# Electron-Labs/starky_bls12_381

Hardware: AMD Instinct MI355X
Metric: starky proofs/sec (FinalExponentiateStark 73527x8192) (higher is better)
Workload: dtype u64 (Goldilocks field)

## Files before the change

bindings/rust/starkhip-sys/src/lib.rs:

```rust
#![allow(non_camel_case_types)]

use std::os::raw::{c_char, c_int, c_long, c_uint, c_void};

#[repr(C)]
#[derive(Clone, Copy, Debug, Default)]
pub struct starkhip_config_t {
    pub security_bits: u32,
    pub num_challenges: u32,
    pub rate_bits: u32,
    pub cap_height: u32,
    pub proof_of_work_bits: u32,
    pub arity_bits: u32,
    pub final_poly_bits: u32,
    pub num_query_rounds: u32,
}

#[repr(C)]
#[derive(Clone, Copy, Debug, PartialEq, Eq)]
pub enum Air {
    Fp12Mul = 0,
    PairingPrecomp = 1,
    MillerLoop = 2,
    FinalExp = 3,
    EccAggregate = 4,
// ... 231 lines not shown
    pub fn starkhip_trace_pairing_precomp(qx: *const u32, qy: *const u32, qz: *const u32, trace: *mut u64, n_rows: usize,
                                          public_inputs: *mut u64) -> c_int;
    pub fn starkhip_trace_ecc_aggregate(points: *const u32, bits: *const u8, trace: *mut u64, n_rows: usize, public_inputs: *mut u64) -> c_int;

    pub fn starkhip_init(device_ordinal: c_int, ctx: *mut *mut c_void) -> c_int;
    pub fn starkhip_shutdown(ctx: *mut c_void);
    pub fn starkhip_set_option(ctx: *mut c_void, name: *const c_char, value: c_long) -> c_int;
    pub fn starkhip_prove(ctx: *mut c_void, air: Air, cfg: *const starkhip_config_t, trace: *const u64, n_rows: usize, n_cols: usize,
                          trace_layout: c_int, trace_on_device: c_int, public_inputs: *const u64, n_pis: usize, pow_witness: u64,
                          proof: *mut *mut u64, proof_words: *mut usize) -> c_int;

    pub fn starkhip_trace_log_begin(log: *mut *mut c_void) -> c_int;
    pub fn starkhip_trace_set_threads(n: c_int) -> c_int;
    pub fn starkhip_trace_log_end(log: *mut c_void) -> c_int;
    pub fn starkhip_trace_log_free(log: *mut c_void);
    pub fn starkhip_trace_log_info(log: *const c_void, n_rows: *mut usize, n_cols: *mut usize, n_records: *mut usize, n_words: *mut usize) -> c_int;
    pub fn starkhip_prove_compact(ctx: *mut c_void, air: Air, cfg: *const starkhip_config_t, log: *const c_void, public_inputs: *const u64,
                                  n_pis: usize, pow_witness: u64, proof: *mut *mut u64, proof_words: *mut usize) -> c_int;

    pub fn starkhip_pool_create(cfg: *const starkhip_pool_config_t, pool: *mut *mut c_void) -> c_int;
    pub fn starkhip_pool_destroy(pool: *mut c_void);
    pub fn starkhip_pool_submit(pool: *mut c_void, air: Air, cfg: *const starkhip_config_t, trace: *const u64, n_rows: usize, n_cols: usize,
                                trace_layout: c_int, trace_on_device: c_int, public_inputs: *const u64, n_pis: usize, pow_witness: u64,
                                ticket: *mut u64) -> c_int;
    pub fn starkhip_prove_columns(ctx: *mut c_void, air: Air, cfg: *const starkhip_config_t, columns: *const *const u64, n_rows: usize, n_cols: usize,
                                  public_inputs: *const u64, n_pis: usize, pow_witness: u64, proof: *mut *mut u64, proof_words: *mut usize) -> c_int;
    pub fn starkhip_pool_submit_columns(pool: *mut c_void, air: Air, cfg: *const starkhip_config_t, columns: *const *const u64, n_rows: usize,
                                        n_cols: usize, public_inputs: *const u64, n_pis: usize, pow_witness: u64, ticket: *mut u64) -> c_int;
    pub fn starkhip_pool_submit_compact(pool: *mut c_void, air: Air, cfg: *const starkhip_config_t, log: *const c_void, public_inputs: *const u64,
                                        n_pis: usize, pow_witness: u64, ticket: *mut u64) -> c_int;
    pub fn starkhip_pool_submit_witness(pool: *mut c_void, air: Air, cfg: *const starkhip_config_t, operands: *const u32, n_limbs: usize,
                                        pow_witness: u64, ticket: *mut u64) -> c_int;
    pub fn starkhip_pool_wait(pool: *mut c_void, ticket: u64, proof: *mut *mut u64, proof_words: *mut usize, info: *mut starkhip_ticket_info_t) -> c_int;

    pub fn starkhip_multipool_create(devices: *const c_int, n_devices: usize, cfg: *const starkhip_pool_config_t, mpool: *mut *mut c_void) -> c_int;
    pub fn starkhip_multipool_destroy(mpool: *mut c_void);
    pub fn starkhip_multipool_size(mpool: *const c_void) -> usize;
    pub fn starkhip_multipool_submit(mpool: *mut c_void, slot: c_int, air: Air, cfg: *const starkhip_config_t, trace: *const u64, n_rows: usize,
                                     n_cols: usize, trace_layout: c_int, trace_on_device: c_int, public_inputs: *const u64, n_pis: usize,
                                     pow_witness: u64, ticket: *mut u64) -> c_int;
    pub fn starkhip_multipool_submit_columns(mpool: *mut c_void, slot: c_int, air: Air, cfg: *const starkhip_config_t, columns: *const *const u64,
                                             n_rows: usize, n_cols: usize, public_inputs: *const u64, n_pis: usize, pow_witness: u64,
                                             ticket: *mut u64) -> c_int;
    pub fn starkhip_multipool_submit_witness(mpool: *mut c_void, slot: c_int, air: Air, cfg: *const starkhip_config_t, operands: *const u32,
                                             n_limbs: usize, pow_witness: u64, ticket: *mut u64) -> c_int;
    pub fn starkhip_multipool_submit_witness_batch(mpool: *mut c_void, n_jobs: usize, airs: *const Air, operands: *const *const u32,
                                                   n_limbs: *const usize, pow_witness: u64, tickets: *mut u64, rcs: *mut c_int) -> c_int;
    pub fn starkhip_multipool_ticket_slot(mpool: *const c_void, ticket: u64) -> c_int;
    pub fn starkhip_multipool_wait(mpool: *mut c_void, ticket: u64, proof: *mut *mut u64, proof_words: *mut usize,
                                   info: *mut starkhip_ticket_info_t) -> c_int;
    pub fn starkhip_hw_queues_status() -> c_int;
    pub fn starkhip_hw_queues_in_effect() -> c_int;
    pub fn starkhip_pool_set_option(pool: *mut c_void, name: *const c_char, value: c_long) -> c_int;
    pub fn starkhip_pool_submit_verify(pool: *mut c_void, air: Air, cfg: *const starkhip_config_t, proof: *const u64, proof_words: usize,
                                       ticket: *mut u64) -> c_int;
    pub fn starkhip_pool_verify_stats(pool: *mut c_void, out: *mut starkhip_pool_verify_stats_t) -> c_int;
    pub fn starkhip_pool_check_stats(pool: *mut c_void, out: *mut u64) -> c_int;
    pub fn starkhip_multipool_set_option(mpool: *mut c_void, name: *const c_char, value: c_long) -> c_int;
    pub fn starkhip_multipool_submit_verify(mpool: *mut c_void, slot: c_int, air: Air, cfg: *const starkhip_config_t, proof: *const u64,
                                            proof_words: usize, ticket: *mut u64) -> c_int;
    pub fn starkhip_multipool_verify_batch(mpool: *mut c_void, n: usize, airs: *const Air, cfgs: *const starkhip_config_t,
                                           proofs: *const *const u64, proof_words: *const usize, results: *mut c_int) -> c_int;
    pub fn starkhip_plan_verify(n: usize, airs: *const Air, n_pools: usize, slots: *mut c_int, order: *mut usize) -> c_int;
    pub fn starkhip_air_verify_cost(air: Air) -> f64;

    pub fn starkhip_last_timings(ctx: *mut c_void, ms: *mut f32) -> c_int;
    pub fn starkhip_host_alloc(ctx: *mut c_void, bytes: usize, out: *mut *mut c_void) -> c_int;
    pub fn starkhip_host_free(p: *mut c_void);

    pub fn starkhip_verify(air: Air, cfg: *const starkhip_config_t, proof: *const u64, proof_words: usize) -> c_int;
    pub fn starkhip_verify_batch(ctx: *mut c_void, n: usize, airs: *const Air, cfgs: *const starkhip_config_t, proofs: *const *const u64,
                                 proof_words: *const usize, results: *mut c_int) -> c_int;
    pub fn starkhip_last_verify_timings(ctx: *mut c_void, out: *mut f64) -> c_int;
    pub fn starkhip_verify_batch_replay(n: usize, airs: *const Air, cfgs: *const starkhip_config_t, proofs: *const *const u64,
                                        proof_words: *const usize, results: *mut c_int) -> c_int;
    pub fn starkhip_proof_layout(proof: *const u64, proof_words: usize, out: *mut starkhip_proof_layout_t) -> c_int;
    pub fn starkhip_proof_hasher(proof: *const u64, proof_words: usize) -> c_int;
    pub fn starkhip_keccak256(bytes: *const u8, len: usize, out32: *mut u8);
    pub fn starkhip_keccak_permute_host(state12: *mut u64);
    pub fn starkhip_keccak_state_from_words(words: *const u64, n: usize, state12: *mut u64) -> c_int;
    pub fn starkhip_keccak_permute_batch(ctx: *mut c_void, states: *mut u64, n: usize) -> c_int;
    pub fn starkhip_merkle_tree_hasher(ctx: *mut c_void, hasher: c_int, lde_colmajor: *const u64, n_cols: usize, log_n: c_uint, cap_height: c_uint,
                                       digests_out: *mut u64, cap_out: *mut u64) -> c_int;
    pub fn starkhip_hash_rows_hasher(ctx: *mut c_void, hasher: c_int, rows: *const u64, width: usize, n_leaves: usize, digests_out: *mut u64) -> c_int;
    pub fn starkhip_fri_geometry(cfg: *const starkhip_config_t, log_n: c_uint, arities_out: *mut c_uint, cap: usize, n_layers: *mut usize,
                                 final_poly_len: *mut usize) -> c_int;
    pub fn starkhip_free(p: *mut c_void);
    pub fn starkhip_proof_blob_stats(out: *mut u64);
    pub fn starkhip_error_string(code: c_int) -> *const c_char;
}

#[derive(Debug, Clone, Copy, PartialEq, Eq)]
pub struct Error(pub c_int);

impl std::fmt::Display for Error {
    fn fmt(&self, f: &mut std::fmt::Formatter<'_>) -> std::fmt::Result {
        let s = unsafe { std::ffi::CStr::from_ptr(starkhip_error_string(self.0)) };
        write!(f, "starkhip: {} ({})", s.to_string_lossy(), self.0)
    }
}
impl std::error::Error for Error {}

fn check(rc: c_int) -> Result<(), Error> {
    if rc == STARKHIP_OK { Ok(()) } else { Err(Error(rc)) }
}

pub type Config = starkhip_config_t;
impl Config {
    pub fn for_air(air: Air) -> Result<Config, Error> {
        let mut cfg = Config::default();
        check(unsafe { starkhip_config_for_air(air, &mut cfg) })?;
        Ok(cfg)
    }
}

pub struct Proof(pub Vec<u64>);
impl Proof {
    pub fn layout(&self) -> Result<starkhip_proof_layout_t, Error> {
        let mut l = std::mem::MaybeUninit::<starkhip_proof_layout_t>::zeroed();
        check(unsafe { starkhip_proof_layout(self.0.as_ptr(), self.0.len(), l.as_mut_ptr()) })?;
        Ok(unsafe { l.assume_init() })
    }
    pub fn hasher(&self) -> Result<c_int, Error> {
        let h = unsafe { starkhip_proof_hasher(self.0.as_ptr(), self.0.len()) };
        if h < 0 { check(h)?; }
        Ok(h)
    }
    pub fn public_inputs(&self) -> Result<&[u64], Error> {
        let l = self.layout()?;
        Ok(&self.0[l.off_public_inputs..l.off_public_inputs + l.n_public_inputs])
    }
}

pub struct RecordedTrace {
    log: *mut c_void,
    pub public_inputs: Vec<u64>,
}
unsafe impl Send for RecordedTrace {}
impl Drop for RecordedTrace {
    fn drop(&mut self) {
        unsafe { starkhip_trace_log_free(self.log) }
    }
}

fn record(air: Air, fill: impl FnOnce(*mut u64) -> c_int) -> Result<RecordedTrace, Error> {
    let n_pis = unsafe { starkhip_air_public_inputs(air) } as usize;
    let mut pis = vec![0u64; n_pis];
    let mut log = std::ptr::null_mut();
    check(unsafe { starkhip_trace_log_begin(&mut log) })?;
    let rc = fill(pis.as_mut_ptr());
    let end = unsafe { starkhip_trace_log_end(log) };
    if rc != STARKHIP_OK || end != STARKHIP_OK {
        unsafe { starkhip_trace_log_free(log) };
        return Err(Error(if rc != STARKHIP_OK { rc } else { end }));
    }
    Ok(RecordedTrace { log, public_inputs: pis })
}

pub fn record_final_exp(x: &[u32; 144]) -> Result<RecordedTrace, Error> {
    record(Air::FinalExp, |pis| unsafe { starkhip_trace_final_exp(x.as_ptr(), std::ptr::null_mut(), 8192, pis) })
}
pub fn record_miller_loop(px: &[u32; 12], py: &[u32; 12], qx: &[u32; 24], qy: &[u32; 24], qz: &[u32; 24]) -> Result<RecordedTrace, Error> {
    record(Air::MillerLoop, |pis| unsafe {
        starkhip_trace_miller_loop(px.as_ptr(), py.as_ptr(), qx.as_ptr(), qy.as_ptr(), qz.as_ptr(), std::ptr::null_mut(), 1024, pis)
    })
}
// ... 316 lines not shown
```

include/starkhip.h:

```cpp
#ifndef STARKHIP_H
#define STARKHIP_H
#include <stddef.h>
#include <stdint.h>

#ifdef __cplusplus
extern "C" {
#endif

typedef struct {
    uint32_t security_bits;
    uint32_t num_challenges;
    uint32_t rate_bits;
    uint32_t cap_height;
    uint32_t proof_of_work_bits;
    uint32_t arity_bits;
    uint32_t final_poly_bits;
    uint32_t num_query_rounds;
} starkhip_config_t;

#define STARKHIP_AIR_CUSTOM_BASE 1024
#define STARKHIP_AIR_CUSTOM_CAPACITY 4096
#define STARKHIP_MAX_LOG_ROWS 20
#define STARKHIP_AIR_MAX_COLUMNS (1u << 20)
#define STARKHIP_AIR_MAX_PUBLIC_INPUTS 65535u
// ... 222 lines not shown
int starkhip_pool_set_option(void* pool, const char* name, long value);
int starkhip_pool_check_stats(void* pool, uint64_t out[2]);
int starkhip_pool_submit_verify(void* pool, starkhip_air_t air, const starkhip_config_t* cfg, const uint64_t* proof, size_t proof_words,
                                uint64_t* ticket);
typedef struct {
    unsigned long proofs_checked, verify_jobs, rejected, device_batches;
    double upload_ms, device_ms, prelude_ms, prelude_cpu_s;
    uint64_t arena_bytes;
} starkhip_pool_verify_stats_t;
int starkhip_pool_verify_stats(void* pool, starkhip_pool_verify_stats_t* out);

int starkhip_multipool_create(const int* devices, size_t n_devices, const starkhip_pool_config_t* cfg, void** mpool);
void starkhip_multipool_destroy(void* mpool);
size_t starkhip_multipool_size(const void* mpool);
void* starkhip_multipool_pool(void* mpool, size_t slot);
int starkhip_multipool_device(const void* mpool, size_t slot);
int starkhip_multipool_submit(void* mpool, int slot, starkhip_air_t air, const starkhip_config_t* cfg, const uint64_t* trace, size_t n_rows,
                              size_t n_cols, int trace_layout, int trace_on_device, const uint64_t* public_inputs, size_t n_pis,
                              uint64_t pow_witness, uint64_t* ticket);
int starkhip_multipool_submit_columns(void* mpool, int slot, starkhip_air_t air, const starkhip_config_t* cfg, const uint64_t* const* columns,
                                      size_t n_rows, size_t n_cols, const uint64_t* public_inputs, size_t n_pis, uint64_t pow_witness,
                                      uint64_t* ticket);
int starkhip_multipool_submit_compact(void* mpool, int slot, starkhip_air_t air, const starkhip_config_t* cfg, const void* log,
                                      const uint64_t* public_inputs, size_t n_pis, uint64_t pow_witness, uint64_t* ticket);
int starkhip_multipool_submit_witness(void* mpool, int slot, starkhip_air_t air, const starkhip_config_t* cfg, const uint32_t* operands,
                                      size_t n_limbs, uint64_t pow_witness, uint64_t* ticket);
int starkhip_multipool_submit_witness_batch(void* mpool, size_t n_jobs, const starkhip_air_t* airs, const uint32_t* const* operands,
                                            const size_t* n_limbs, uint64_t pow_witness, uint64_t* tickets, int* rcs);
int starkhip_multipool_ticket_slot(const void* mpool, uint64_t ticket);
int starkhip_multipool_wait(void* mpool, uint64_t ticket, uint64_t** proof, size_t* proof_words, starkhip_ticket_info_t* info);
int starkhip_multipool_set_option(void* mpool, const char* name, long value);
int starkhip_multipool_submit_verify(void* mpool, int slot, starkhip_air_t air, const starkhip_config_t* cfg, const uint64_t* proof,
                                     size_t proof_words, uint64_t* ticket);
int starkhip_multipool_verify_batch(void* mpool, size_t n, const starkhip_air_t* airs, const starkhip_config_t* cfgs, const uint64_t* const* proofs,
                                    const size_t* proof_words, int* results);
int starkhip_plan_verify(size_t n, const starkhip_air_t* airs, size_t n_pools, int* slots, size_t* order);
double starkhip_air_verify_cost(starkhip_air_t air);
int starkhip_plan_lpt(size_t n_jobs, const starkhip_air_t* airs, size_t n_pools, int* slots);
double starkhip_air_cost(starkhip_air_t air);

#define STARKHIP_N_PHASES 11
int starkhip_last_timings(void* ctx, float ms[STARKHIP_N_PHASES]);
int starkhip_last_kernel_timings(void* ctx, float ms[3]);
int starkhip_last_host_timings(void* ctx, float ms[2]);

int starkhip_host_alloc(void* ctx, size_t bytes, void** out);
void starkhip_host_free(void* p);

int starkhip_permutation_zs(void* ctx, starkhip_air_t air, const uint64_t* trace, size_t n_rows, size_t n_cols, int layout, int on_device,
                            const uint64_t* challenges, uint64_t* zs_out, uint64_t* closing_out);
int starkhip_permutation_zs_replay(starkhip_air_t air, const uint64_t* trace, size_t n_rows, size_t n_cols, int layout, const uint64_t* challenges,
                                   uint64_t* zs_out, uint64_t* closing_out);
int starkhip_air_eval_frame_full(starkhip_air_t air, const uint64_t* local, const uint64_t* next, const uint64_t* public_inputs,
                                 const uint64_t masks[8], const uint64_t* alphas, int n_alpha, const uint64_t* zs, const uint64_t* zs_next,
                                 const uint64_t* challenges, uint64_t* acc_out);
int starkhip_lde_batch(void* ctx, const uint64_t* values, size_t n_cols, unsigned log_n, unsigned rate_bits, uint64_t* coeffs_out,
                       uint64_t* lde_out);
int starkhip_ntt_long(void* ctx, uint64_t* data, size_t n_vecs, unsigned log_len, int inverse);
int starkhip_merkle_cap(void* ctx, const uint64_t* lde_colmajor, size_t n_cols, unsigned log_N, unsigned cap_height, uint64_t* cap_out);
int starkhip_poseidon_permute_batch(void* ctx, uint64_t* states, size_t n_states);
int starkhip_lde_bench(void* ctx, size_t n_cols, unsigned log_n, unsigned rate_bits, unsigned reps, unsigned const_per_64, const uint64_t* device_values,
                       float* ms_per_launch, float* each_ms);
int starkhip_trace_log_expand_device(void* ctx, const void* log, uint64_t* trace_colmajor);
int starkhip_field_ops_batch(void* ctx, int op, const uint64_t* a, const uint64_t* b, uint64_t* out, size_t n);
int starkhip_poseidon_permute_batch_form(void* ctx, int form, int variant, uint64_t* states, size_t n_states);
int starkhip_leaf_hash_lane_group(void* ctx, const uint64_t* mats, size_t n_segments, size_t n_cols, unsigned log_n, unsigned rate_bits, int grouped,
                                  int form, unsigned prefix_mask, uint64_t* digests_out);
int starkhip_leaf_prefix_table(void* ctx, unsigned log_n, unsigned rate_bits, uint64_t* cap_out);
int starkhip_selfcheck_hash_tables(unsigned n_states);
size_t starkhip_hash_table_image(int form, void* out, size_t cap);
size_t starkhip_lde_launch_ranges(size_t n_cols, unsigned rate_bits, uint64_t* triples, size_t cap);
int starkhip_fri_geometry(const starkhip_config_t* cfg, unsigned log_n, unsigned* arities_out, size_t cap, size_t* n_layers,
                          size_t* final_poly_len);
int starkhip_quotient_plan_check(starkhip_air_t air, unsigned want_chunks, uint64_t seed, uint64_t stats[8]);
int starkhip_quotient_classes(starkhip_air_t air, uint8_t* classes, size_t n);
int starkhip_quotient_solve_table(unsigned log_rows, unsigned quotient_degree_bits, uint64_t* out, size_t n);
int starkhip_quotient_class_plan_check(starkhip_air_t air, unsigned want_chunks, uint64_t seed, uint64_t stats[32]);
void starkhip_keccak256(const uint8_t* bytes, size_t len, uint8_t out32[32]);
void starkhip_keccak_permute_host(uint64_t state12[12]);
int starkhip_keccak_state_from_words(const uint64_t* words, size_t n, uint64_t state12[12]);
int starkhip_keccak_permute_batch(void* ctx, uint64_t* states, size_t n);
int starkhip_merkle_tree_hasher(void* ctx, int hasher, const uint64_t* lde_colmajor, size_t n_cols, unsigned log_N, unsigned cap_height,
                                uint64_t* digests_out, uint64_t* cap_out);
int starkhip_hash_rows_hasher(void* ctx, int hasher, const uint64_t* rows, size_t width, size_t n_leaves, uint64_t* digests_out);
void starkhip_poseidon_permute_host(uint64_t state[12]);
void starkhip_poseidon_permute_host_many(uint64_t state[12], size_t n, int which);

int starkhip_verify(starkhip_air_t air, const starkhip_config_t* cfg, const uint64_t* proof, size_t proof_words);

int starkhip_verify_batch(void* ctx, size_t n, const starkhip_air_t* airs, const starkhip_config_t* cfgs, const uint64_t* const* proofs,
                          const size_t* proof_words, int* results);
int starkhip_last_verify_timings(void* ctx, double out[4]);
int starkhip_verify_batch_replay(size_t n, const starkhip_air_t* airs, const starkhip_config_t* cfgs, const uint64_t* const* proofs,
                                 const size_t* proof_words, int* results);

void starkhip_free(void* p);
const char* starkhip_error_string(int code);

#define STARKHIP_PROOF_MAGIC 0x3130304652505353ULL

typedef struct {
    size_t n_columns, n_quotient_polys, degree_bits, rate_bits, cap_height, n_fri_layers, n_query_rounds, final_poly_len,
        n_public_inputs, arity_bits;
    size_t off_trace_cap, off_quotient_cap, off_local_values, off_next_values, off_quotient_openings, off_fri_caps, off_query_rounds,
        query_round_words, off_final_poly, off_pow_witness, off_public_inputs, total_words;
    size_t q_trace_leaf, q_trace_siblings, q_quotient_leaf, q_quotient_siblings, initial_sibling_count;
    size_t q_step_evals[16], q_step_siblings[16], step_sibling_count[16];
    size_t n_permutation_zs, off_permutation_zs_cap, off_permutation_zs, off_permutation_zs_next, q_permutation_zs_leaf, q_permutation_zs_siblings;
} starkhip_proof_layout_t;
int starkhip_proof_layout(const uint64_t* proof, size_t proof_words, starkhip_proof_layout_t* out);
int starkhip_proof_hasher(const uint64_t* proof, size_t proof_words);

#ifdef __cplusplus
}
#endif
#endif
```

starky_bls12_381_amd/api.py:

```python
import ctypes as C
import os
import time
import weakref

import numpy as np

_HERE = os.path.dirname(os.path.abspath(__file__))
LIB_PATH = os.environ.get("STARKHIP_LIBRARY") or os.path.join(_HERE, "libstarkhip.so")

if not os.path.exists(LIB_PATH):
    raise ImportError(
        f"{LIB_PATH} is missing: build it with `make` (or __graft_entry__.build()); "
        "starky_bls12_381_amd has no CPU fallback for the prover")

lib = C.CDLL(LIB_PATH)

P = 0xFFFFFFFF00000001
POW_SEARCH = 0xFFFFFFFFFFFFFFFF
N_PHASES = 11
PHASE_NAMES = ["upload", "ifft_lde", "trace_merkle", "quotient", "quotient_commit", "openings", "fri_combine",
               "fri_commit", "pow", "queries", "total"]

AIR_FP12_MUL, AIR_PAIRING_PRECOMP, AIR_MILLER_LOOP, AIR_FINAL_EXP, AIR_ECC_AGGREGATE, AIR_TEST_FIBONACCI = 0, 1, 2, 3, 4, 100
AIR_NAMES = {AIR_FP12_MUL: "FP12MulStark", AIR_PAIRING_PRECOMP: "PairingPrecompStark", AIR_MILLER_LOOP: "MillerLoopStark",
# ... 24 lines not shown

class StarkhipError(RuntimeError):
    def __init__(self, code):
        self.code = code
        super().__init__(f"starkhip error {code}: {lib.starkhip_error_string(code).decode()}")


def _chk(rc):
    if rc != 0:
        raise StarkhipError(rc)


_u64p = C.POINTER(C.c_uint64)
_u32p = C.POINTER(C.c_uint32)
lib.starkhip_error_string.restype = C.c_char_p
lib.starkhip_error_string.argtypes = [C.c_int]
lib.starkhip_config_standard_fast.argtypes = [C.POINTER(StarkConfig)]
lib.starkhip_config_for_air.argtypes = [C.c_int, C.POINTER(StarkConfig)]
for _f in ("columns", "public_inputs", "constraint_degree", "num_constraints", "default_rows"):
    getattr(lib, "starkhip_air_" + _f).argtypes = [C.c_int]
lib.starkhip_air_program.argtypes = [C.c_int, C.POINTER(_u64p), C.POINTER(C.c_size_t)]
lib.starkhip_init.argtypes = [C.c_int, C.POINTER(C.c_void_p)]
lib.starkhip_shutdown.argtypes = [C.c_void_p]
lib.starkhip_shutdown.restype = None
lib.starkhip_prove.argtypes = [C.c_void_p, C.c_int, C.POINTER(StarkConfig), C.c_void_p, C.c_size_t, C.c_size_t, C.c_int, C.c_int, _u64p, C.c_size_t,
                               C.c_uint64, C.POINTER(_u64p), C.POINTER(C.c_size_t)]
lib.starkhip_prove_columns.argtypes = [C.c_void_p, C.c_int, C.POINTER(StarkConfig), C.POINTER(C.c_void_p), C.c_size_t, C.c_size_t, _u64p, C.c_size_t,
                                       C.c_uint64, C.POINTER(_u64p), C.POINTER(C.c_size_t)]
lib.starkhip_last_timings.argtypes = [C.c_void_p, C.POINTER(C.c_float)]
lib.starkhip_last_kernel_timings.argtypes = [C.c_void_p, C.POINTER(C.c_float)]
lib.starkhip_last_host_timings.argtypes = [C.c_void_p, C.POINTER(C.c_float)]
lib.starkhip_ntt_long.argtypes = [C.c_void_p, _u64p, C.c_size_t, C.c_uint, C.c_int]
lib.starkhip_lde_batch.argtypes = [C.c_void_p, _u64p, C.c_size_t, C.c_uint, C.c_uint, _u64p, _u64p]
lib.starkhip_merkle_cap.argtypes = [C.c_void_p, _u64p, C.c_size_t, C.c_uint, C.c_uint, _u64p]
lib.starkhip_poseidon_permute_batch.argtypes = [C.c_void_p, _u64p, C.c_size_t]
lib.starkhip_poseidon_permute_batch_form.argtypes = [C.c_void_p, C.c_int, C.c_int, _u64p, C.c_size_t]
lib.starkhip_leaf_hash_lane_group.argtypes = [C.c_void_p, _u64p, C.c_size_t, C.c_size_t, C.c_uint, C.c_uint, C.c_int, C.c_int, C.c_uint, _u64p]
lib.starkhip_leaf_prefix_table.argtypes = [C.c_void_p, C.c_uint, C.c_uint, _u64p]
lib.starkhip_field_ops_batch.argtypes = [C.c_void_p, C.c_int, _u64p, _u64p, _u64p, C.c_size_t]
lib.starkhip_poseidon_permute_host.argtypes = [_u64p]
lib.starkhip_poseidon_permute_host.restype = None
lib.starkhip_verify.argtypes = [C.c_int, C.POINTER(StarkConfig), _u64p, C.c_size_t]
_verify_batch_args = [C.c_size_t, C.POINTER(C.c_int), C.POINTER(StarkConfig), C.POINTER(_u64p), C.POINTER(C.c_size_t), C.POINTER(C.c_int)]
lib.starkhip_verify_batch.argtypes = [C.c_void_p] + _verify_batch_args
lib.starkhip_verify_batch_replay.argtypes = _verify_batch_args
lib.starkhip_last_verify_timings.argtypes = [C.c_void_p, C.POINTER(C.c_double)]
lib.starkhip_free.argtypes = [C.c_void_p]
lib.starkhip_free.restype = None
lib.starkhip_host_alloc.argtypes = [C.c_void_p, C.c_size_t, C.POINTER(C.c_void_p)]
lib.starkhip_trace_log_begin.argtypes = [C.POINTER(C.c_void_p)]
lib.starkhip_trace_log_end.argtypes = [C.c_void_p]
lib.starkhip_trace_set_threads.argtypes = [C.c_int]
lib.starkhip_trace_log_free.argtypes = [C.c_void_p]
lib.starkhip_trace_log_free.restype = None
lib.starkhip_trace_log_info.argtypes = [C.c_void_p] + [C.POINTER(C.c_size_t)] * 4
lib.starkhip_trace_log_from_writes.argtypes = [C.c_size_t, C.c_size_t, C.POINTER(C.c_uint64), C.c_size_t, C.POINTER(C.c_void_p)]
lib.starkhip_lde_bench.argtypes = [C.c_void_p, C.c_size_t, C.c_uint, C.c_uint, C.c_uint, C.c_uint, C.c_void_p, C.POINTER(C.c_float), C.POINTER(C.c_float)]
lib.starkhip_trace_log_expand_device.argtypes = [C.c_void_p, C.c_void_p, C.POINTER(C.c_uint64)]
lib.starkhip_trace_log_overwrites.argtypes = [C.c_void_p] + [C.POINTER(C.c_size_t)] * 2
lib.starkhip_trace_log_expand_host.argtypes = [C.c_void_p, C.POINTER(C.c_uint64), C.POINTER(C.c_size_t)]
lib.starkhip_prove_compact.argtypes = [C.c_void_p, C.c_int, C.POINTER(StarkConfig), C.c_void_p, C.POINTER(C.c_uint64), C.c_size_t, C.c_uint64,
                                       C.POINTER(C.POINTER(C.c_uint64)), C.POINTER(C.c_size_t)]
lib.starkhip_host_free.argtypes = [C.c_void_p]
lib.starkhip_host_free.restype = None
lib.starkhip_trace_fibonacci.argtypes = [C.c_uint64, C.c_uint64, _u64p, C.c_size_t, _u64p]
lib.starkhip_trace_fp12_mul.argtypes = [_u32p, _u32p, _u64p, C.c_size_t, _u64p]
lib.starkhip_trace_final_exp.argtypes = [_u32p, _u64p, C.c_size_t, _u64p]
lib.starkhip_trace_miller_loop.argtypes = [_u32p, _u32p, _u32p, _u32p, _u32p, _u64p, C.c_size_t, _u64p]
lib.starkhip_trace_pairing_precomp.argtypes = [_u32p, _u32p, _u32p, _u64p, C.c_size_t, _u64p]
lib.starkhip_native_fp12_mul.argtypes = [_u32p, _u32p, _u32p]
lib.starkhip_native_final_exponentiate.argtypes = [_u32p, _u32p]
lib.starkhip_native_miller_loop.argtypes = [_u32p, _u32p, _u32p, _u32p, _u32p, _u32p]
lib.starkhip_native_pairing_precomp.argtypes = [_u32p, _u32p, _u32p, _u32p]
_u8p = C.POINTER(C.c_uint8)
HASHER_POSEIDON, HASHER_KECCAK = 0, 1
LEAF_HASH_FORM_KECCAK = 6
lib.starkhip_keccak256.argtypes = [C.c_char_p, C.c_size_t, _u8p]
lib.starkhip_keccak256.restype = None
lib.starkhip_keccak_permute_host.argtypes = [_u64p]
lib.starkhip_keccak_permute_host.restype = None
lib.starkhip_keccak_state_from_words.argtypes = [_u64p, C.c_size_t, _u64p]
lib.starkhip_keccak_permute_batch.argtypes = [C.c_void_p, _u64p, C.c_size_t]
lib.starkhip_merkle_tree_hasher.argtypes = [C.c_void_p, C.c_int, _u64p, C.c_size_t, C.c_uint, C.c_uint, _u64p, _u64p]
lib.starkhip_hash_rows_hasher.argtypes = [C.c_void_p, C.c_int, _u64p, C.c_size_t, C.c_size_t, _u64p]
lib.starkhip_proof_hasher.argtypes = [_u64p, C.c_size_t]
lib.starkhip_trace_ecc_aggregate.argtypes = [_u32p, _u8p, _u64p, C.c_size_t, _u64p]
lib.starkhip_native_g1_aggregate.argtypes = [_u32p, _u8p, _u32p]


def _p64(a):
    return a.ctypes.data_as(_u64p)


def _p32(a):
    return a.ctypes.data_as(_u32p)


def _limbs(x, n):
    a = np.ascontiguousarray(x, dtype=np.uint32).reshape(-1)
    assert a.size == n, (a.size, n)
    return a


def air_columns(air):
    r = lib.starkhip_air_columns(air)
    if r < 0:
        raise StarkhipError(r)
    return r


def air_public_inputs(air):
    r = lib.starkhip_air_public_inputs(air)
    if r < 0:
        raise StarkhipError(r)
    return r


def air_constraint_degree(air):
    r = lib.starkhip_air_constraint_degree(air)
    if r < 0:
        raise StarkhipError(r)
    return r


def air_num_constraints(air):
    r = lib.starkhip_air_num_constraints(air)
    if r < 0:
        raise StarkhipError(r)
    return r


def air_default_rows(air):
    r = lib.starkhip_air_default_rows(air)
    if r < 0:
        raise StarkhipError(r)
    return r


def air_permutation_pairs(air):
    r = lib.starkhip_air_permutation_pairs(air)
    if r < 0:
        raise StarkhipError(r)
    return r


def air_permutation_zs(air):
    r = lib.starkhip_air_permutation_zs(air)
    if r < 0:
        raise StarkhipError(r)
    return r


def air_program(air):
    blob = _u64p()
    words = C.c_size_t()
    _chk(lib.starkhip_air_program(air, C.byref(blob), C.byref(words)))
    return np.ctypeslib.as_array(blob, shape=(words.value,)).copy()


lib.starkhip_air_check_program.argtypes = [_u64p, C.c_size_t, C.c_char_p, C.c_size_t]
lib.starkhip_air_register.argtypes = [_u64p, C.c_size_t, C.c_char_p, C.c_uint32, C.POINTER(C.c_int)]
lib.starkhip_check_trace.argtypes = [C.c_void_p, C.c_int, C.c_void_p, C.c_size_t, C.c_size_t, C.c_int, C.c_int, _u64p, _u64p, _u64p]
CHECK_LIST_MAX = 1 << 20


class _CheckReportStruct(C.Structure):
# ... 900 lines not shown
    def lde_bench(self, n_cols, log_n, rate_bits, reps=5, const_per_64=0, device_ptr=None, each=False):
        ms = C.c_float()
        per = (C.c_float * 16)()
        _chk(lib.starkhip_lde_bench(self._ctx, n_cols, log_n, rate_bits, reps, const_per_64, C.c_void_p(device_ptr) if device_ptr else None, C.byref(ms), per))
        return [round(float(x), 2) for x in per[:max(1, min(reps, 16))]] if each else float(ms.value)

    def expand_trace(self, compact):
        n, c = compact.shape
        out = np.empty((c, n), dtype=np.uint64)
        _chk(lib.starkhip_trace_log_expand_device(self._ctx, compact._h, _p64(out)))
        return np.ascontiguousarray(out.T)

    def set_option(self, name, value):
        _chk(lib.starkhip_set_option(self._ctx, name.encode(), int(value)))

    def check_stats(self):
        out = np.zeros(2, dtype=np.uint64)
        _chk(lib.starkhip_check_stats(self._ctx, _p64(out)))
        return {"checked": int(out[0]), "rejected": int(out[1])}

    def prove_device(self, air, config, trace_ptr, n_rows, public_inputs, pow_witness=POW_SEARCH, layout=1, keep=True):
        pis = np.ascontiguousarray(public_inputs, dtype=np.uint64)
        out = _u64p()
        words = C.c_size_t()
        t0 = time.perf_counter()
        rc = lib.starkhip_prove(self._ctx, air, C.byref(config), C.c_void_p(trace_ptr), n_rows, air_columns(air), layout, 1, _p64(pis), pis.size, pow_witness,
                                C.byref(out), C.byref(words))
        self.last_call_s = time.perf_counter() - t0
        return _take_blob(rc, out, words, keep)

    def host_array(self, shape, dtype=np.uint64):
        shape = tuple(int(s) for s in np.atleast_1d(shape))
        nbytes = int(np.prod(shape)) * np.dtype(dtype).itemsize
        p = C.c_void_p()
        _chk(lib.starkhip_host_alloc(self._ctx, nbytes, C.byref(p)))
        raw = (C.c_ubyte * nbytes).from_address(p.value)
        weakref.finalize(raw, lib.starkhip_host_free, p.value)
        return np.frombuffer(raw, dtype=dtype).reshape(shape)

    def last_timings(self):
        ms = (C.c_float * N_PHASES)()
        _chk(lib.starkhip_last_timings(self._ctx, ms))
        return dict(zip(PHASE_NAMES, [float(x) for x in ms]))

    def last_host_timings(self):
        ms = (C.c_float * 2)()
        _chk(lib.starkhip_last_host_timings(self._ctx, ms))
        return {"fiat_shamir": float(ms[0]), "other": float(ms[1])}

    def last_kernel_timings(self):
        ms = (C.c_float * 3)()
        _chk(lib.starkhip_last_kernel_timings(self._ctx, ms))
        return {"lde_columns": float(ms[0]), "leaf_hash": float(ms[1]), "quotient_eval": float(ms[2])}

    def ntt_long(self, vectors, inverse=False):
        v = np.ascontiguousarray(vectors, dtype=np.uint64).copy()
        n_vecs, n = v.shape
        _chk(lib.starkhip_ntt_long(self._ctx, _p64(v), n_vecs, n.bit_length() - 1, 1 if inverse else 0))
        return v

    def lde_batch(self, values_colmajor, rate_bits):
        v = np.ascontiguousarray(values_colmajor, dtype=np.uint64)
        ncols, n = v.shape
        log_n = n.bit_length() - 1
        coeffs = np.zeros_like(v)
        lde = np.zeros((ncols, n << rate_bits), dtype=np.uint64)
        _chk(lib.starkhip_lde_batch(self._ctx, _p64(v), ncols, log_n, rate_bits, _p64(coeffs), _p64(lde)))
        return coeffs, lde

    def merkle_cap(self, lde_colmajor, cap_height):
        v = np.ascontiguousarray(lde_colmajor, dtype=np.uint64)
        ncols, N = v.shape
        cap = np.zeros((1 << cap_height, 4), dtype=np.uint64)
        _chk(lib.starkhip_merkle_cap(self._ctx, _p64(v), ncols, N.bit_length() - 1, cap_height, _p64(cap)))
        return cap

    def merkle_tree(self, lde_colmajor, cap_height, hasher=HASHER_POSEIDON):
        v = np.ascontiguousarray(lde_colmajor, dtype=np.uint64)
        ncols, N = v.shape
        digests = np.zeros((N, 4), dtype=np.uint64)
        cap = np.zeros((1 << cap_height, 4), dtype=np.uint64)
        _chk(lib.starkhip_merkle_tree_hasher(self._ctx, hasher, _p64(v), ncols, N.bit_length() - 1, cap_height, _p64(digests), _p64(cap)))
        return digests, cap

    def hash_rows(self, rows, hasher=HASHER_POSEIDON):
        r = np.ascontiguousarray(rows, dtype=np.uint64)
        assert r.ndim == 2
        out = np.zeros((r.shape[0], 4), dtype=np.uint64)
        _chk(lib.starkhip_hash_rows_hasher(self._ctx, hasher, _p64(r), r.shape[1], r.shape[0], _p64(out)))
        return out

    def keccak_permute_batch(self, states):
        s = np.ascontiguousarray(states, dtype=np.uint64).copy()
        assert s.ndim == 2 and s.shape[1] == 12
        _chk(lib.starkhip_keccak_permute_batch(self._ctx, _p64(s), s.shape[0]))
        return s

    def field_ops(self, op, a, b):
        a = np.ascontiguousarray(a, dtype=np.uint64)
        b = np.ascontiguousarray(b, dtype=np.uint64)
        assert a.shape == b.shape and a.ndim == 1
        out = np.zeros_like(a)
        _chk(lib.starkhip_field_ops_batch(self._ctx, op, _p64(a), _p64(b), _p64(out), a.size))
        return out

    def leaf_hash_lane_group(self, mats, log_n, rate_bits=0, grouped=True, form=3, prefix_mask=0):
        m = np.ascontiguousarray(mats, dtype=np.uint64)
        assert m.ndim == 3
        out = np.zeros((m.shape[0], m.shape[2], 4), dtype=np.uint64)
        if m.shape[2] != 1 << (log_n + rate_bits):
            raise StarkhipError(ERR_BAD_SHAPE)
        _chk(lib.starkhip_leaf_hash_lane_group(self._ctx, _p64(m), m.shape[0], m.shape[1], log_n, rate_bits, 1 if grouped else 0, form, prefix_mask, _p64(out)))
        return out

    def leaf_prefix_table(self, log_n, rate_bits):
        out = np.zeros((4, 1 << (log_n + rate_bits)), dtype=np.uint64)
        _chk(lib.starkhip_leaf_prefix_table(self._ctx, log_n, rate_bits, _p64(out)))
        return out

    def poseidon_permute_batch(self, states, form=0, variant=0):
        s = np.ascontiguousarray(states, dtype=np.uint64).copy()
        assert s.ndim == 2 and s.shape[1] == 12
        if form == 0 and variant == 0:
            _chk(lib.starkhip_poseidon_permute_batch(self._ctx, _p64(s), s.shape[0]))
        else:
            _chk(lib.starkhip_poseidon_permute_batch_form(self._ctx, form, variant, _p64(s), s.shape[0]))
        return s

    def verify_batch(self, items):
        return _verify_batch(items, self._ctx)

    def verify_stark_proof_device(self, air, config, proof):
        _chk(self.verify_batch([(air, config, proof)])[0])

    def last_verify_timings(self):
        out = (C.c_double * 4)()
        _chk(lib.starkhip_last_verify_timings(self._ctx, out))
        return dict(zip(("prelude_ms", "upload_ms", "device_ms", "cpu_s"), list(out)))


class PoolConfig(C.Structure):
    _fields_ = [("device", C.c_int), ("big_contexts", C.c_uint), ("small_contexts", C.c_uint), ("generator_threads", C.c_uint),
                ("trace_threads", C.c_uint), ("commit_policy", C.c_uint), ("stream_priority", C.c_uint), ("warm_up", C.c_uint), ("gather_ms", C.c_float)]


class TicketInfo(C.Structure):
    _fields_ = [("phase_ms", C.c_float * N_PHASES), ("kernel_ms", C.c_float * 3), ("host_ms", C.c_float * 2), ("t_submit", C.c_double), ("t_generate_start", C.c_double),
                ("t_generate_end", C.c_double), ("t_prove_start", C.c_double), ("t_done", C.c_double), ("leaf_hash_form", C.c_int),
                ("leaf_hash_group", C.c_uint)]


class PoolStats(C.Structure):
    _fields_ = [(n, C.c_ulong) for n in ("big_commit_launches", "small_commit_launches", "small_commit_requests", "max_merged_commitments", "big_commit_grids")]


lib.starkhip_pool_create.argtypes = [C.POINTER(PoolConfig), C.POINTER(C.c_void_p)]
lib.starkhip_pool_destroy.argtypes = [C.c_void_p]
lib.starkhip_pool_destroy.restype = None
lib.starkhip_pool_submit.argtypes = [C.c_void_p, C.c_int, C.POINTER(StarkConfig), C.c_void_p, C.c_size_t, C.c_size_t, C.c_int, C.c_int, _u64p,
                                     C.c_size_t, C.c_uint64, C.POINTER(C.c_uint64)]
lib.starkhip_pool_submit_compact.argtypes = [C.c_void_p, C.c_int, C.POINTER(StarkConfig), C.c_void_p, _u64p, C.c_size_t, C.c_uint64,
                                             C.POINTER(C.c_uint64)]
lib.starkhip_pool_submit_witness.argtypes = [C.c_void_p, C.c_int, C.POINTER(StarkConfig), _u32p, C.c_size_t, C.c_uint64, C.POINTER(C.c_uint64)]
lib.starkhip_pool_wait.argtypes = [C.c_void_p, C.c_uint64, C.POINTER(_u64p), C.POINTER(C.c_size_t), C.POINTER(TicketInfo)]
lib.starkhip_pool_stats.argtypes = [C.c_void_p, C.POINTER(PoolStats)]
lib.starkhip_pool_submit_columns.argtypes = [C.c_void_p, C.c_int, C.POINTER(StarkConfig), C.POINTER(C.c_void_p), C.c_size_t, C.c_size_t, _u64p, C.c_size_t,
# ... 387 lines not shown
```

starky_bls12_381_amd/csrc/capi.cpp:

```cpp
#include <dirent.h>
#include <mutex>
#include <stdio.h>
#include <stdlib.h>
#include <string.h>
#include <unistd.h>

#include <new>

#include "air_eval.h"
#include "air_validate.h"
#include "airs.h"
#include "blob_arena.h"
#include "check_report.h"
#include "free_cells.h"
#include "kernels.h"
#include "lde_ranges.h"
#include "lookup_columns.h"
#include "permutation.h"
#include "permutation_check.h"
#include "trace_log.h"

#include <atomic>
#include "poseidon.h"
#include "prover.h"
// ... 966 lines not shown
    try {
        return expand_log((Ctx*)ctx, (const TraceLog*)log, trace_colmajor);
    } catch (const std::bad_alloc&) {
        return STARKHIP_ERR_OOM;
    }
}
int starkhip_poseidon_permute_batch(void* ctx, uint64_t* states, size_t n_states) {
    if (!ctx) return STARKHIP_ERR_NO_DEVICE;
    return permute_batch((Ctx*)ctx, states, n_states);
}
int starkhip_poseidon_permute_batch_form(void* ctx, int form, int variant, uint64_t* states, size_t n_states) {
    if (!ctx) return STARKHIP_ERR_NO_DEVICE;
    return permute_batch_form((Ctx*)ctx, form, variant, states, n_states);
}
int starkhip_leaf_hash_lane_group(void* ctx, const uint64_t* mats, size_t n_segments, size_t n_cols, unsigned log_n, unsigned rate_bits, int grouped,
                                  int form, unsigned prefix_mask, uint64_t* digests_out) {
    if (!ctx) return STARKHIP_ERR_NO_DEVICE;
    return leaf_hash_lane_group((Ctx*)ctx, mats, n_segments, n_cols, log_n, rate_bits, grouped, form, prefix_mask, digests_out);
}
int starkhip_leaf_prefix_table(void* ctx, unsigned log_n, unsigned rate_bits, uint64_t* cap_out) {
    if (!ctx) return STARKHIP_ERR_NO_DEVICE;
    return leaf_prefix_table((Ctx*)ctx, log_n, rate_bits, cap_out);
}
int starkhip_field_ops_batch(void* ctx, int op, const uint64_t* a, const uint64_t* b, uint64_t* out, size_t n) {
    if (!ctx) return STARKHIP_ERR_NO_DEVICE;
    return field_ops((Ctx*)ctx, op, a, b, out, n);
}
int starkhip_selfcheck_hash_tables(unsigned n_states) {
    const int fours = merged_fours_selfcheck(n_states);
    if (fours < 0) return -1;
    return quad_merged_tables_selfcheck(n_states) + fours;
}
size_t starkhip_hash_table_image(int form, void* out, size_t cap) {
    const void* image = nullptr;
    size_t bytes = 0;
    switch (form) {
        case FORM_QUAD: image = quad_merged_tables_host(); bytes = sizeof(QuadMergedTables); break;
        case FORM_ROW: image = row_merged_tables_host(); bytes = sizeof(RowMergedTables); break;
        case FORM_LANE: image = lane_tables_host(); bytes = sizeof(LaneTables); break;
        case FORM_PAIR: image = pair_tables_host(); bytes = sizeof(PairTables); break;
    }
    if (!image) return 0;
    if (out && cap >= bytes) memcpy(out, image, bytes);
    return bytes;
}
int starkhip_fri_geometry(const starkhip_config_t* cfg, unsigned log_n, unsigned* arities_out, size_t cap, size_t* n_layers, size_t* final_poly_len) {
    if (!cfg) return STARKHIP_ERR_BAD_SHAPE;
    FriGeometry g;
    if (!FriGeometry::make(*cfg, log_n, &g)) return STARKHIP_ERR_BAD_SHAPE;
    for (size_t l = 0; l < g.arities.size() && l < cap; l++) arities_out[l] = g.arities[l];
    if (n_layers) *n_layers = g.arities.size();
    if (final_poly_len) *final_poly_len = g.final_poly_len;
    return STARKHIP_OK;
}

size_t starkhip_lde_launch_ranges(size_t n_cols, unsigned rate_bits, uint64_t* triples, size_t cap) {
    const std::vector<LdeLaunch> plan = lde_launch_plan(n_cols, rate_bits);
    for (size_t i = 0; i < plan.size() && i < cap; i++) {
        triples[3 * i] = plan[i].a;
        triples[3 * i + 1] = plan[i].b;
        triples[3 * i + 2] = plan[i].from_copy ? 1 : 0;
    }
    return plan.size();
}
void starkhip_poseidon_permute_host(uint64_t state[12]) { poseidon_permute_host(state); }

void starkhip_keccak256(const uint8_t* bytes, size_t len, uint8_t out32[32]) { keccak256_host(bytes, len, out32); }
void starkhip_keccak_permute_host(uint64_t state12[12]) { keccak_permute_host(state12); }
int starkhip_keccak_state_from_words(const uint64_t* words, size_t n, uint64_t state12[12]) {
    if (!words || !state12) return -1;
    int used = 0;
    const int have = keccak_take_words(words, (int)std::min<size_t>(n, 1u << 20), state12, 0, &used);
    return have == 12 ? used : -1;
}
int starkhip_keccak_permute_batch(void* ctx, uint64_t* states, size_t n) {
    if (!ctx) return STARKHIP_ERR_NO_DEVICE;
    return keccak_permute_batch((Ctx*)ctx, states, n);
}
int starkhip_merkle_tree_hasher(void* ctx, int hasher, const uint64_t* lde_colmajor, size_t n_cols, unsigned log_N, unsigned cap_height,
                                uint64_t* digests_out, uint64_t* cap_out) {
    if (!ctx) return STARKHIP_ERR_NO_DEVICE;
    return merkle_tree_hasher((Ctx*)ctx, hasher, lde_colmajor, n_cols, log_N, cap_height, digests_out, cap_out);
}
int starkhip_hash_rows_hasher(void* ctx, int hasher, const uint64_t* rows, size_t width, size_t n_leaves, uint64_t* digests_out) {
    if (!ctx) return STARKHIP_ERR_NO_DEVICE;
    return hash_rows_hasher((Ctx*)ctx, hasher, rows, width, n_leaves, digests_out);
}
int starkhip_proof_hasher(const uint64_t* proof, size_t proof_words) {
    ProofLayout pl;
    if (!proof || !pl.read_header(proof, proof_words)) return STARKHIP_ERR_BAD_SHAPE;
    return (int)pl.hasher;
}
void starkhip_poseidon_permute_host_many(uint64_t state[12], size_t n, int which) {
    for (size_t i = 0; i < n; i++) {
        if (which == 0) poseidon_permute_host(state);
        else poseidon_permute(state);
    }
}

int starkhip_verify(starkhip_air_t air, const starkhip_config_t* cfg, const uint64_t* proof, size_t proof_words) {
    const AirInfo* a = air_get(air);
    if (!a) return STARKHIP_ERR_BAD_AIR;
    return verify_proof(*a, *cfg, proof, proof_words);
}

int starkhip_verify_batch(void* ctx, size_t n, const starkhip_air_t* airs, const starkhip_config_t* cfgs, const uint64_t* const* proofs,
                          const size_t* proof_words, int* results) {
    if (!ctx) return STARKHIP_ERR_NO_DEVICE;
    try {
        return verify_batch_device((Ctx*)ctx, n, airs, cfgs, proofs, proof_words, results);
    } catch (const std::bad_alloc&) {
        return STARKHIP_ERR_OOM;
    }
}

int starkhip_last_verify_timings(void* ctx, double out[4]) {
    if (!ctx) return STARKHIP_ERR_NO_DEVICE;
    if (!out) return STARKHIP_ERR_BAD_SHAPE;
    memcpy(out, ctx_verify_timings((Ctx*)ctx), 4 * sizeof(double));
    return STARKHIP_OK;
}

int starkhip_verify_batch_replay(size_t n, const starkhip_air_t* airs, const starkhip_config_t* cfgs, const uint64_t* const* proofs,
                                 const size_t* proof_words, int* results) {
    try {
        return verify_batch_replay(n, airs, cfgs, proofs, proof_words, results);
    } catch (const std::bad_alloc&) {
        return STARKHIP_ERR_OOM;
    }
}

void starkhip_proof_blob_stats(uint64_t out[5]) {
    const starkhip::BlobArenaStats st = starkhip::blob_arena_stats();
    out[0] = st.blobs; out[1] = st.busy; out[2] = st.bytes; out[3] = st.taken; out[4] = st.missed;
}
void starkhip_free(void* p) { starkhip::blob_free(p); }

const char* starkhip_error_string(int code) {
    switch (code) {
        case STARKHIP_OK: return "ok";
        case STARKHIP_ERR_QUOTIENT_NOT_DIVISIBLE: return "Quotient has failed, the vanishing polynomial is not divisible by Z_H";
        case STARKHIP_ERR_ZETA_IN_SUBGROUP: return "Opening point is in the subgroup";
        case STARKHIP_ERR_BAD_SHAPE: return "bad shape (columns / public inputs / rows / config do not match the AIR)";
        case STARKHIP_ERR_HIP: return "HIP runtime error";
        case STARKHIP_ERR_OOM: return "out of device memory";
        case STARKHIP_ERR_NO_DEVICE: return "no such HIP device / context";
        case STARKHIP_ERR_VERIFY: return "proof rejected";
        case STARKHIP_ERR_BAD_AIR: return "unknown or unbuildable AIR id";
        case STARKHIP_ERR_TRACE: return "the trace violates the AIR (\"check_trace\"): a check blob is returned instead of a proof";
        default: return "unknown error";
    }
}

}
```

starky_bls12_381_amd/csrc/ctx.h:

```cpp
#pragma once
#include <hip/hip_runtime.h>

#include <stdio.h>

#include <atomic>
#include <memory>
#include <set>
#include <system_error>
#include <thread>
#include <vector>

#include "airs.h"
#include "kernels.h"
#include "prover.h"
#include "scheduler.h"
#include "trace_log.h"

namespace starkhip {

#define HIPCHK(expr)                                                                                       \
    do {                                                                                                   \
        hipError_t _e = (expr);                                                                            \
        if (_e != hipSuccess) {                                                                            \
            fprintf(stderr, "starkhip: HIP error %s at %s:%d (%s)\n", hipGetErrorString(_e), __FILE__, __LINE__, #expr); \
// ... 8 lines not shown
    ~DevBuf() { release(); }
    void release() {
        if (p) (void)hipFree(p);
        p = nullptr;
        cap = 0;
    }
    hipError_t ensure(size_t bytes) {
        if (bytes <= cap) return hipSuccess;
        release();
        hipError_t e = hipMalloc(&p, bytes);
        if (e == hipSuccess) cap = bytes;
        return e;
    }
    template <class T>
    T* as() const { return (T*)p; }
};

struct Ctx {
    int device = 0;
    hipStream_t st = nullptr;
    hipStream_t st_normal = nullptr, st_high = nullptr;
    hipEvent_t ev[STARKHIP_N_PHASES + 1] = {};
    float timings[STARKHIP_N_PHASES] = {0};
    hipEvent_t kev[6] = {};
    float ktimings[3] = {0};
    float htimings[2] = {0};
    HashService* hs = nullptr;
    hipEvent_t hash_ready = nullptr, hash_done = nullptr;
    HashService::Timing hash_timing;
    hipEvent_t wait_ev = nullptr;
    void* rb = nullptr;
    size_t rb_cap = 0, rb_used = 0;
    struct Pending { void* dst; const void* src; size_t bytes; };
    std::vector<Pending> rb_pending;
    void* host_staging = nullptr;
    size_t host_staging_cap = 0;
    hipEvent_t col_ev[2] = {nullptr, nullptr};
    std::set<int> blob_airs;
    bool hash_requested = false;
    bool urgent = false;
    long opt_quotient_impl = 0;
    long opt_quotient_cosets = 0;
    long opt_quotient_waves = 65536, opt_quotient_slots = 0, opt_quotient_chunks = 0, opt_quotient_debug = 0, opt_zeta_on_coset = 0;
    struct Tables {
        int log_n = -1, rate = -1, qdb = -1;
        DevBuf tw_fwd, tw_inv, coset_scale, qtab, qshift_inv;
        DevBuf qsolve;
        DevBuf lde2_fwd, lde2_inv, lde2_cs, lde2_oh;
        DevBuf lde_wave;
        DevBuf leaf_prefix;
        bool leaf_prefix_built = false;
        DevBuf long_cs, long_sub;
        struct LongTw { unsigned log_len; DevBuf fwd, inv; };
        std::vector<std::unique_ptr<LongTw>> long_tw;
        std::vector<DevBuf*> bufs() {
            std::vector<DevBuf*> v = {&tw_fwd, &tw_inv, &coset_scale, &qtab, &qshift_inv, &qsolve, &lde2_fwd, &lde2_inv, &lde2_cs, &lde2_oh, &lde_wave, &leaf_prefix, &long_cs, &long_sub};
            for (auto& t : long_tw) {
                v.push_back(&t->fwd);
                v.push_back(&t->inv);
            }
            return v;
        }
    };
    struct PlanDev {
        int air = -1;
        unsigned chunks = 0, want = 0;
        uint32_t recs = 0;
        bool by_class = false;
        unsigned n_work = 0, n_vecs = 0, n_classes = 0;
        DevBuf q_recs, q_streams, q_chunk_tile_off, q_tile_list, q_contrib_off, q_contribs, q_consts, q_apow, q_work, q_sum_off, q_vec_slot, q_vec_of;
        std::vector<DevBuf*> bufs() {
            return {&q_recs, &q_streams, &q_chunk_tile_off, &q_tile_list, &q_contrib_off, &q_contribs, &q_consts, &q_apow, &q_work, &q_sum_off, &q_vec_slot, &q_vec_of};
        }
    };
    std::vector<std::unique_ptr<Tables>> table_cache;
    std::vector<std::unique_ptr<PlanDev>> plan_cache;
    Tables* tab = nullptr;
    PlanDev* plan = nullptr;
    long opt_leaf_hash_form = FORM_AUTO;
    long opt_hasher = 0;
    long opt_lde_impl = 0;
    long opt_lde_closed_forms = 1;
    long opt_leaf_hash_prefix = 1;
    long opt_host_commit_leaves = 64;
    long opt_verify_chunk_mb = 1024;
    double verify_timings[4] = {0};
    long opt_check_trace = 0, opt_check_trace_list = 16;
    std::atomic<uint64_t> traces_checked{0}, traces_rejected{0};
    std::vector<gl_t> host_lde;
    struct OpProgram {
        int air = -1;
        unsigned chunks = 0, slots = 0;
        DevBuf ops, loads, chunk_off;
        std::vector<uint32_t> chunk_k_after;
        std::vector<DevBuf*> bufs() { return {&ops, &loads, &chunk_off}; }
    } prog;
    struct CheckProgram {
        int air = -1;
        unsigned want = 0, chunks = 0;
        std::vector<uint32_t> k0;
        DevBuf ops, meta, out, rep, list;
        std::vector<DevBuf*> bufs() { return {&ops, &meta, &out, &rep, &list}; }
    } chk;
    DevBuf staging, values, lde, digests, pis, apow, chunk_scale, partial, qclass, qvals, qcoef, qlde, qdigests, zpow, gzpow, open_local,
        open_next, open_q, ext_apow, comb_partial, comb_out, fri_coef, fri_vals, fri_rows[16], fri_digests[16], scale_tab, pow_state,
        pow_best, qidx, gather_t;
    std::vector<DevBuf*> dev_bufs() {
        std::vector<DevBuf*> v = {&staging, &values, &lde, &digests, &pis,
                                  &apow, &chunk_scale, &partial, &qclass, &qvals, &qcoef, &qlde, &qdigests, &zpow, &gzpow, &open_local, &open_next, &open_q,
                                  &ext_apow, &comb_partial, &comb_out, &fri_coef, &fri_vals, &scale_tab, &pow_state, &pow_best, &qidx, &gather_t};
        for (DevBuf& b : fri_rows) v.push_back(&b);
        for (DevBuf& b : fri_digests) v.push_back(&b);
        for (DevBuf* b : prog.bufs()) v.push_back(b);
        for (DevBuf* b : chk.bufs()) v.push_back(b);
        for (DevBuf* b : free_chk.bufs()) v.push_back(b);
        for (DevBuf* b : perm.bufs()) v.push_back(b);
        for (DevBuf* b : mset.bufs()) v.push_back(b);
        for (DevBuf* b : lookup.bufs()) v.push_back(b);
        for (auto& t : table_cache)
            for (DevBuf* b : t->bufs()) v.push_back(b);
        for (auto& d : plan_cache)
            for (DevBuf* b : d->bufs()) v.push_back(b);
        return v;
    }
    struct FreeCellsProgram {
        int air = -1;
        unsigned want = 0;
        DevBuf cons, pivots, planes, class_counts;
        std::vector<DevBuf*> bufs() { return {&cons, &pivots, &planes, &class_counts}; }
    } free_chk;
    struct PermBufs {
        DevBuf cols, desc, chal, zvals, zcoef, zlde, zdigests, scan, open_z, open_zn;
        std::vector<DevBuf*> bufs() { return {&cols, &desc, &chal, &zvals, &zcoef, &zlde, &zdigests, &scan, &open_z, &open_zn}; }
    } perm;
    struct MultisetBufs {
        DevBuf desc, keys, idx, table, masks;
        float ms[4] = {0, 0, 0, 0};
        std::vector<DevBuf*> bufs() { return {&desc, &keys, &idx, &table, &masks}; }
    } mset;
    struct LookupBufs {
        DevBuf desc, cols, flags, sums, slot, mask;
        float ms[4] = {0, 0, 0, 0};
        std::vector<DevBuf*> bufs() { return {&desc, &cols, &flags, &sums, &slot, &mask}; }
    } lookup;
};

hipError_t stream_wait(Ctx* c);
hipError_t read_back(Ctx* c, void* dst, const void* src, size_t bytes, hipStream_t st);
hipError_t ensure_host_staging(Ctx* c, size_t need, size_t grow_to);
int ensure_tables(Ctx* c, unsigned log_n, unsigned rate, unsigned qdb);
bool long_vector(unsigned log_len);
int ensure_long_tw(Ctx* c, unsigned log_len, LdeLongTables* out);
int ensure_plan(Ctx* c, const AirInfo& air, size_t quotient_points, bool by_class = false);
int ensure_program(Ctx* c, const AirInfo& air, size_t quotient_points);
hipError_t run_lde(Ctx* c, const gl_t* values, gl_t* coeffs, gl_t* lde, size_t cols, unsigned log_n, unsigned rate, int from_coeffs, unsigned col_base = 0,
                   unsigned* unit_count = nullptr);
bool leaf_prefix_wanted(const Ctx* c, size_t n_cols, unsigned log_n, unsigned rate);
size_t leaf_prefix_bytes(const Ctx* c, size_t n_cols, unsigned log_n, unsigned rate);
int ensure_leaf_prefix(Ctx* c, unsigned log_n, unsigned rate);
unsigned* leaf_prefix_counter(const Ctx* c);
hipError_t leaf_prefix_reset(Ctx* c);
LeafPrefix leaf_prefix(const Ctx* c);
int run_ntt(Ctx* c, gl_t* data, gl_t* mid, size_t n_vecs, size_t vec_stride, unsigned log_len, bool inverse, const gl_t* pre_scale,
            const gl_t* post_scale);
int upload_dense(Ctx* c, const TraceInput& in, gl_t* dst, const gl_t** d_values);
int check_trace_in_prove(Ctx* c, const AirInfo& air, const gl_t* d_trace, size_t n_rows, const uint64_t* pis, uint64_t** blob, size_t* words);
// ... 25 lines not shown
```

starky_bls12_381_amd/csrc/ctx.hip:

```cpp
#include <hip/hip_runtime.h>

#include <atomic>
#include <time.h>
#include <string.h>

#include <algorithm>
#include <memory>
#include <string>
#include <vector>

#include "blob_arena.h"
#include "ctx.h"
#include "quotient_ops.h"
#include "quotient_plan.h"
#include "verifier.h"

namespace starkhip {

hipError_t event_wait_sleeping(hipEvent_t ev) {
    for (int spin = 0; spin < 8; spin++) {
        const hipError_t q = hipEventQuery(ev);
        if (q != hipErrorNotReady) return q;
    }
    (void)hipGetLastError();
// ... 261 lines not shown
static void ctx_release(Ctx* c) {
    for (DevBuf* b : c->dev_bufs()) b->release();
    for (hipEvent_t e : c->ev)
        if (e) (void)hipEventDestroy(e);
    for (hipEvent_t e : c->kev)
        if (e) (void)hipEventDestroy(e);
    if (c->rb) (void)hipHostFree(c->rb);
    for (hipEvent_t e : {c->hash_ready, c->hash_done, c->wait_ev, c->hash_timing.t0, c->hash_timing.t1, c->col_ev[0], c->col_ev[1]})
        if (e) (void)hipEventDestroy(e);
    if (c->host_staging) (void)hipHostFree(c->host_staging);
    blob_arena_drop(c);
    if (c->st_normal) (void)hipStreamDestroy(c->st_normal);
    if (c->st_high) (void)hipStreamDestroy(c->st_high);
    delete c;
}

int ctx_create(int device, Ctx** out, int priority) {
    int count = 0;
    if (hipGetDeviceCount(&count) != hipSuccess || count <= 0) return STARKHIP_ERR_NO_DEVICE;
    if (device < 0 || device >= count) return STARKHIP_ERR_NO_DEVICE;
    HIPCHK(hipSetDevice(device));
    Ctx* c = new Ctx();
    c->device = device;
    bool ok;
    if (priority) {
        int least = 0, greatest = 0;
        ok = hipDeviceGetStreamPriorityRange(&least, &greatest) == hipSuccess &&
             hipStreamCreateWithPriority(&c->st_normal, hipStreamDefault, priority > 0 ? greatest : least) == hipSuccess;
    } else {
        ok = hipStreamCreate(&c->st_normal) == hipSuccess;
    }
    c->st = c->st_normal;
    for (auto& e : c->ev) ok = ok && hipEventCreate(&e) == hipSuccess;
    for (auto& e : c->kev) ok = ok && hipEventCreate(&e) == hipSuccess;
    ok = ok && hipEventCreateWithFlags(&c->hash_ready, hipEventDisableTiming) == hipSuccess;
    ok = ok && hipEventCreateWithFlags(&c->hash_done, hipEventDisableTiming | hipEventBlockingSync) == hipSuccess;
    ok = ok && hipEventCreateWithFlags(&c->wait_ev, hipEventDisableTiming | hipEventBlockingSync) == hipSuccess;
    ok = ok && hipEventCreate(&c->hash_timing.t0) == hipSuccess && hipEventCreate(&c->hash_timing.t1) == hipSuccess;
    if (ok && hipHostMalloc(&c->rb, (size_t)8 << 20, hipHostMallocDefault) == hipSuccess) c->rb_cap = (size_t)8 << 20;
    else c->rb = nullptr;
    if (!ok) {
        ctx_release(c);
        return STARKHIP_ERR_HIP;
    }
    *out = c;
    return 0;
}

void ctx_destroy(Ctx* c) {
    if (!c) return;
    (void)hipSetDevice(c->device);
    (void)hipStreamSynchronize(c->st);
    ctx_release(c);
}
void ctx_attach_hash_service(Ctx* c, HashService* hs) { c->hs = hs; }
int ctx_set_urgent(Ctx* c, bool urgent) {
    if (urgent && !c->st_high) {
        HIPCHK(hipSetDevice(c->device));
        int least = 0, greatest = 0;
        HIPCHK(hipDeviceGetStreamPriorityRange(&least, &greatest));
        HIPCHK(hipStreamCreateWithPriority(&c->st_high, hipStreamDefault, greatest));
    }
    c->st = urgent ? c->st_high : c->st_normal;
    c->urgent = urgent;
    return STARKHIP_OK;
}
bool ctx_has_hash_service(Ctx* c) { return c->hs != nullptr; }
void ctx_hash_request_reset(Ctx* c) { c->hash_requested = false; }
bool ctx_hash_requested(Ctx* c) { return c->hash_requested; }

int ctx_set_option(Ctx* c, const char* name, long value) {
    if (!c || !name) return STARKHIP_ERR_BAD_SHAPE;
    const std::string k(name);
    if (k == "quotient_impl" && (value == 0 || value == 1)) c->opt_quotient_impl = value;
    else if (k == "quotient_waves" && value >= 64) { c->opt_quotient_waves = value; c->prog.air = -1; }
    else if (k == "quotient_slots" && value >= 0 && value <= 64) { c->opt_quotient_slots = value; c->prog.air = -1; }
#ifdef STARKHIP_DEBUG
    else if (k == "quotient_debug" && value >= 0 && value <= 9) c->opt_quotient_debug = value;
#endif
    else if (k == "zeta_on_coset" && value >= 0) c->opt_zeta_on_coset = value;
    else if (k == "lde_closed_forms" && (value == 0 || value == 1)) c->opt_lde_closed_forms = value;
    else if (k == "lde_impl" && (value == 0 || value == 1)) c->opt_lde_impl = value;
    else if (k == "leaf_hash_prefix" && (value == 0 || value == 1)) c->opt_leaf_hash_prefix = value;
    else if (k == "host_commit_leaves" && value >= 0 && value <= 4096) c->opt_host_commit_leaves = value;
    else if (k == "leaf_hash_form" && value >= FORM_AUTO && value <= FORM_PAIR) c->opt_leaf_hash_form = value;
    else if (k == "quotient_cosets" && (value == 0 || value == 1)) c->opt_quotient_cosets = value;
    else if (k == "quotient_chunks" && value >= 0 && value <= 4096) c->opt_quotient_chunks = value;
    else if (k == "verify_chunk_mb" && value >= 1) c->opt_verify_chunk_mb = value;
    else if (k == "hasher" && value >= STARKHIP_HASHER_POSEIDON && value <= STARKHIP_HASHER_KECCAK) c->opt_hasher = value;
    else if (k == "check_trace" && (value == 0 || value == 1)) c->opt_check_trace = value;
    else if (k == "check_trace_list" && value >= 0 && value <= (long)STARKHIP_CHECK_LIST_MAX) c->opt_check_trace_list = value;
    else return STARKHIP_ERR_BAD_SHAPE;
    return STARKHIP_OK;
}
void ctx_set_check_trace(Ctx* c, bool on, size_t list_cap) {
    c->opt_check_trace = on;
    c->opt_check_trace_list = (long)std::min<size_t>(list_cap, STARKHIP_CHECK_LIST_MAX);
}
void ctx_set_hasher(Ctx* c, int hasher) { c->opt_hasher = hasher; }
void ctx_check_stats(Ctx* c, uint64_t out[2]) {
    out[0] = c->traces_checked.load();
    out[1] = c->traces_rejected.load();
}
size_t ctx_device_bytes(Ctx* c) {
    size_t total = 0;
    for (DevBuf* b : c->dev_bufs()) total += b->cap;
    return total;
}
size_t ctx_pinned_bytes(Ctx* c) { return c->host_staging_cap + c->rb_cap; }
const float* ctx_timings(Ctx* c) { return c->timings; }
long ctx_verify_chunk_mb(Ctx* c) { return c->opt_verify_chunk_mb; }
double* ctx_verify_timings(Ctx* c) { return c->verify_timings; }
int ctx_device(Ctx* c) { return c->device; }
const float* ctx_kernel_timings(Ctx* c) { return c->ktimings; }
const float* ctx_host_timings(Ctx* c) { return c->htimings; }
void ctx_commit_info(Ctx* c, int* form, unsigned* group) {
    *form = c->hash_timing.form;
    *group = c->hash_timing.group;
}

hipError_t ensure_host_staging(Ctx* c, size_t need, size_t grow_to) {
    if (c->host_staging_cap >= need) return hipSuccess;
    if (c->host_staging) (void)hipHostFree(c->host_staging);
    c->host_staging = nullptr;
    c->host_staging_cap = 0;
    const hipError_t e = hipHostMalloc(&c->host_staging, grow_to, hipHostMallocDefault);
    if (e == hipSuccess) c->host_staging_cap = grow_to;
    return e;
}

std::vector<LogPiece> recording_pieces(const TraceLog& log) {
    const size_t nw = log.total_words(), nr = log.total_records();
    std::vector<LogPiece> pieces;
    size_t at_r = 0, at_z = 0;
    log.for_each_part([&](const TraceLog& part) {
        if (!part.words.empty()) pieces.push_back({part.base, part.words.data(), part.words.size()});
        if (!part.offsets.empty()) pieces.push_back({nw + at_r, part.offsets.data(), part.offsets.size()});
        if (!part.late_zeros.empty()) pieces.push_back({nw + nr + at_z, part.late_zeros.data(), part.late_zeros.size()});
        at_r += part.offsets.size();
        at_z += part.late_zeros.size();
    });
    return pieces;
}

int upload_dense(Ctx* c, const TraceInput& in, gl_t* dst, const gl_t** d_values) {
    const size_t n = in.n_rows, C = in.n_cols;
    *d_values = dst;
    if (in.callers_columns()) *d_values = in.words;
    else if (in.on_device) HIPCHK(launch_transpose(in.words, dst, n, C, c->st));
    else if (in.form == TraceForm::ColMajor) HIPCHK(hipMemcpyAsync(dst, in.words, C * n * 8, hipMemcpyHostToDevice, c->st));
    else {
        HIPCHK(hipMemcpyAsync(c->lde.p, in.words, C * n * 8, hipMemcpyHostToDevice, c->st));
        HIPCHK(launch_transpose(c->lde.as<gl_t>(), dst, n, C, c->st));
    }
    return 0;
}

hipError_t launch_leaf_hash_lone(const Ctx* c, const gl_t* lde, size_t n_cols, unsigned log_n, unsigned rate, gl_t* digests, hipStream_t st, int* form,
                                 LeafPrefix prefix) {
    const LeafHashForm f = c->opt_leaf_hash_form == FORM_LANE ? FORM_LANE : use_pair_form(c, n_cols, log_n + rate) ? FORM_PAIR : use_row_form(c, n_cols, log_n + rate) ? FORM_ROW : FORM_QUAD;
    *form = leaf_hash_sent(f);
    return launch_leaf_hash_form(f, lde, n_cols, log_n, rate, digests, st, prefix);
}

int run_ntt(Ctx* c, gl_t* data, gl_t* mid, size_t n_vecs, size_t vec_stride, unsigned log_len, bool inverse, const gl_t* pre_scale,
                   const gl_t* post_scale) {
// ... 13 lines not shown
```

starky_bls12_381_amd/csrc/host_only_stubs.cc:

```cpp
#include <hip/hip_runtime.h>
#include <stdlib.h>
#include <string.h>

#include <atomic>
#include <chrono>
#include <set>
#include <thread>

#include "blob_arena.h"
#include "kernels.h"
#include "prover.h"
#include "scheduler.h"
#include "verifier.h"
#include "verify_chunk.h"
#include "verify_query.h"

namespace starkhip {
std::atomic<uint64_t> g_wait_cpu_ns(0);

static bool fake_device() {
    const char* e = getenv("STARKHIP_FAKE_DEVICE");
    return e && *e == '1';
}

// ... 5 lines not shown
    float timings[STARKHIP_N_PHASES] = {0}, ktimings[3] = {0}, htimings[2] = {0};
    double verify_timings[4] = {0};
    std::set<int> blob_airs;
    HashService::Timing hash_timing;
    char done_tag = 0;
};
static char g_failing_ready_tag = 0;
static hipEvent_t failing_ready() { return (hipEvent_t)&g_failing_ready_tag; }
int ctx_create(int device, Ctx** out, int) {
    if (!fake_device() || device < 0 || device >= 8) {
        *out = nullptr;
        return STARKHIP_ERR_NO_DEVICE;
    }
    *out = new Ctx();
    (*out)->device = device;
    return STARKHIP_OK;
}
void ctx_destroy(Ctx* c) {
    if (c) blob_arena_drop(c);
    delete c;
}
size_t ctx_device_bytes(Ctx*) { return 0; }
size_t ctx_pinned_bytes(Ctx*) { return 0; }
const float* ctx_timings(Ctx* c) { return c->timings; }
long ctx_verify_chunk_mb(Ctx*) { return 1024; }
double* ctx_verify_timings(Ctx* c) { return c->verify_timings; }
int ctx_device(Ctx* c) { return c->device; }
const float* ctx_kernel_timings(Ctx* c) { return c->ktimings; }
const float* ctx_host_timings(Ctx* c) { return c->htimings; }
void ctx_commit_info(Ctx* c, int* form, unsigned* group) { *form = c->hash_timing.form; *group = c->hash_timing.group; }
int ctx_set_option(Ctx*, const char*, long) { return STARKHIP_ERR_NO_DEVICE; }
void ctx_attach_hash_service(Ctx* c, HashService* hs) { c->hs = hs; }
bool ctx_has_hash_service(Ctx* c) { return c->hs != nullptr; }
void ctx_hash_request_reset(Ctx* c) { c->hash_requested = false; }
bool ctx_hash_requested(Ctx* c) { return c->hash_requested; }
int ctx_set_urgent(Ctx* c, bool urgent) { c->urgent = urgent; return STARKHIP_OK; }
void ctx_set_check_trace(Ctx* c, bool on, size_t) { c->check_trace = on; }
void ctx_set_hasher(Ctx*, int) {}
void ctx_check_stats(Ctx* c, uint64_t out[2]) { out[0] = c->traces_checked.load(); out[1] = 0; }
int ctx_reserve(Ctx* c, const AirInfo& air, const starkhip_config_t&, size_t, unsigned proof_blobs, bool) {
    if (proof_blobs && !c->blob_airs.count(air.id)) {
        if (blob_arena_add(c, 64 + air.prog.n_pis * 8, proof_blobs) != 0) return STARKHIP_ERR_OOM;
        c->blob_airs.insert(air.id);
    }
    return STARKHIP_OK;
}

int prove(Ctx* c, const AirInfo& air, const starkhip_config_t& cfg, const TraceInput& in, const uint64_t* pis, size_t n_pis, uint64_t pow_witness,
          uint64_t** proof_out, size_t* proof_words) {
    if (!fake_device()) return STARKHIP_ERR_NO_DEVICE;
    if (n_pis != air.prog.n_pis) return STARKHIP_ERR_BAD_SHAPE;
    if (pow_witness == 0xBAD) return STARKHIP_ERR_BAD_SHAPE;
    const size_t n_rows = in.n_rows;
    std::this_thread::sleep_for(std::chrono::milliseconds(air.cols > 50000 ? 3 : 1));
    if (c->check_trace) c->traces_checked++;
    unsigned log_n = 0;
    while (((size_t)1 << log_n) < n_rows) log_n++;
    if (c->hs) {
        c->hash_requested = true;
        static gl_t dummy[8];
        c->hash_timing = HashService::Timing();
        if (c->hs->hash(dummy, air.cols, log_n, cfg.rate_bits, dummy, nullptr, pow_witness == 0xBAD3 ? failing_ready() : nullptr, (hipEvent_t)&c->done_tag,
                        !HashService::is_big(log_n, cfg.rate_bits), c->urgent, &c->hash_timing) != hipSuccess)
            return STARKHIP_ERR_HIP;
    }
    std::this_thread::sleep_for(std::chrono::milliseconds(2));
    if (pow_witness == 0xBAD2) return STARKHIP_ERR_QUOTIENT_NOT_DIVISIBLE;
    uint64_t* out = blob_alloc((4 + n_pis) * 8);
    if (!out) return STARKHIP_ERR_OOM;
    out[0] = 0xFA4EULL; out[1] = (uint64_t)air.id; out[2] = n_rows; out[3] = (uint64_t)c->urgent | ((uint64_t)c->device << 8);
    if (n_pis) memcpy(out + 4, pis, n_pis * 8);
    *proof_out = out;
    *proof_words = 4 + n_pis;
    c->timings[STARKHIP_N_PHASES - 1] = 3.0f;
    return STARKHIP_OK;
}
int lde_batch(Ctx*, const uint64_t*, size_t, unsigned, unsigned, uint64_t*, uint64_t*) { return STARKHIP_ERR_NO_DEVICE; }
int ntt_long(Ctx*, uint64_t*, size_t, unsigned, int) { return STARKHIP_ERR_NO_DEVICE; }
int merkle_cap(Ctx*, const uint64_t*, size_t, unsigned, unsigned, uint64_t*) { return STARKHIP_ERR_NO_DEVICE; }
int permute_batch(Ctx*, uint64_t*, size_t) { return STARKHIP_ERR_NO_DEVICE; }
int permute_batch_form(Ctx*, int, int, uint64_t*, size_t) { return STARKHIP_ERR_NO_DEVICE; }
int keccak_permute_batch(Ctx*, uint64_t*, size_t) { return STARKHIP_ERR_NO_DEVICE; }
int merkle_tree_hasher(Ctx*, int, const uint64_t*, size_t, unsigned, unsigned, uint64_t*, uint64_t*) { return STARKHIP_ERR_NO_DEVICE; }
int hash_rows_hasher(Ctx*, int, const uint64_t*, size_t, size_t, uint64_t*) { return STARKHIP_ERR_NO_DEVICE; }
int leaf_hash_lane_group(Ctx*, const uint64_t*, size_t, size_t, unsigned, unsigned, int, int, unsigned, uint64_t*) { return STARKHIP_ERR_NO_DEVICE; }
int leaf_prefix_table(Ctx*, unsigned, unsigned, uint64_t*) { return STARKHIP_ERR_NO_DEVICE; }
int expand_log(Ctx*, const TraceLog*, uint64_t*) { return STARKHIP_ERR_NO_DEVICE; }
int check_trace(Ctx*, const AirInfo&, const TraceInput&, const uint64_t*, uint64_t*, uint64_t*) { return STARKHIP_ERR_NO_DEVICE; }
int check_trace_report(Ctx*, const AirInfo&, const TraceInput&, const uint64_t*, uint32_t*, uint64_t*, uint64_t*, size_t, starkhip_check_report_t*) {
    return STARKHIP_ERR_NO_DEVICE;
}
int check_trace_free_cells(Ctx*, const AirInfo&, const TraceInput&, const uint64_t*, uint64_t, uint32_t*, uint64_t*, starkhip_free_cells_t*) {
    return STARKHIP_ERR_NO_DEVICE;
}
int check_trace_free_cell_classes(Ctx*, const AirInfo&, const TraceInput&, const uint64_t*, uint64_t, uint32_t*, uint64_t*, uint32_t*,
                                  starkhip_free_cell_classes_t*) {
    return STARKHIP_ERR_NO_DEVICE;
}
int check_trace_permutations(Ctx*, const AirInfo&, const TraceInput&, uint64_t, uint32_t*, uint64_t*, uint64_t*, size_t, starkhip_perm_check_t*) {
    return STARKHIP_ERR_NO_DEVICE;
}
void perm_check_timings(Ctx*, float ms[4]) { ms[0] = ms[1] = ms[2] = ms[3] = 0; }
int lookup_columns(Ctx*, const LookupTrace&, const starkhip_lookup_t*, size_t, uint32_t*, uint64_t*, uint64_t*, size_t, starkhip_lookup_report_t*) {
    return STARKHIP_ERR_NO_DEVICE;
}
void lookup_timings(Ctx*, float ms[4]) { ms[0] = ms[1] = ms[2] = ms[3] = 0; }
int lde_bench(Ctx*, size_t, unsigned, unsigned, unsigned, unsigned, const uint64_t*, float*, float*) { return STARKHIP_ERR_NO_DEVICE; }
int field_ops(Ctx*, int, const uint64_t*, const uint64_t*, uint64_t*, size_t) { return STARKHIP_ERR_NO_DEVICE; }
int permutation_zs(Ctx*, const AirInfo&, const TraceInput&, const uint64_t*, uint64_t*, uint64_t*) { return STARKHIP_ERR_NO_DEVICE; }
int host_alloc(Ctx*, size_t, void**) { return STARKHIP_ERR_NO_DEVICE; }
void host_free(void*) {}

hipError_t event_wait_sleeping(hipEvent_t ev) { return ev == failing_ready() ? hipErrorUnknown : hipSuccess; }

static std::atomic<unsigned long> g_fake_launches(0), g_fake_merged(0), g_fake_lane_grids(0), g_fake_lane_members(0), g_service_records(0);
hipError_t launch_leaf_hash_form(LeafHashForm, const gl_t*, size_t, unsigned, unsigned, gl_t*, hipStream_t, LeafPrefix) { g_fake_launches++; return hipSuccess; }
hipError_t launch_leaf_hash_multi(const LeafHashBatch&, unsigned count, size_t, unsigned, unsigned, hipStream_t) {
    g_fake_launches++;
    g_fake_merged += count;
    return hipSuccess;
}
hipError_t launch_leaf_hash_lane_group(const LeafHashBatch& B, unsigned count, size_t, unsigned, unsigned, hipStream_t) {
    if (count == 0 || count > LEAF_HASH_MAX_BATCH) return hipErrorInvalidValue;
    for (unsigned i = 0; i < count; i++)
        if (!B.mat[i] || !B.digests[i]) return hipErrorInvalidValue;
    g_fake_launches++;
    g_fake_lane_grids++;
    g_fake_lane_members += count;
    return hipSuccess;
}
hipError_t launch_leaf_hash_keccak(const gl_t*, size_t, unsigned, unsigned, gl_t*, hipStream_t) { return hipErrorNoDevice; }
hipError_t launch_leaf_hash_rows_keccak(const gl_t*, size_t, size_t, gl_t*, hipStream_t) { return hipErrorNoDevice; }
hipError_t launch_merkle_levels_keccak(gl_t*, unsigned, unsigned, hipStream_t) { return hipErrorNoDevice; }
hipError_t launch_permute_batch_keccak(gl_t*, size_t, hipStream_t) { return hipErrorNoDevice; }
hipError_t launch_pow_grind_keccak(const gl_t*, int, unsigned, uint64_t, uint64_t, unsigned long long*, hipStream_t) { return hipErrorNoDevice; }
hipError_t launch_verify_leaf_digests_keccak(const gl_t* words, const VQLeaf* leaves, size_t n, gl_t* digests, hipStream_t) {
    if (!fake_device()) return hipErrorNoDevice;
    verify_host_leaf_digests(words, leaves, n, digests);
    return hipSuccess;
}
hipError_t launch_ext_powers(gl2_t* out, gl2_t alpha, size_t n, hipStream_t) {
    if (!fake_device()) return hipErrorNoDevice;
    verify_host_ext_powers(out, alpha, n);
    return hipSuccess;
}
hipError_t launch_verify_leaf_digests(const gl_t* words, const VQLeaf* leaves, size_t n, gl_t* digests, unsigned, hipStream_t) {
    if (!fake_device()) return hipErrorNoDevice;
    verify_host_leaf_digests(words, leaves, n, digests);
    return hipSuccess;
}
hipError_t launch_verify_range(const gl_t* words, const VQProof* proofs, size_t n, uint32_t* bad, hipStream_t) {
    if (!fake_device()) return hipErrorNoDevice;
    verify_host_range(words, proofs, n, bad);
    return hipSuccess;
}
hipError_t launch_verify_combine(const gl_t* words, const VQProof* proofs, const uint32_t* qp, size_t nq, const gl2_t* apow, gl2_t* sums, hipStream_t) {
    if (!fake_device()) return hipErrorNoDevice;
    verify_host_combine(words, proofs, qp, nq, apow, sums);
    return hipSuccess;
}
hipError_t launch_verify_queries(const gl_t* words, const VQProof* proofs, const uint32_t* qp, const uint64_t* xi, size_t nq, const gl_t* dig,
                                 const gl2_t* sums, uint32_t* status, hipStream_t) {
    if (!fake_device()) return hipErrorNoDevice;
    verify_host_queries(words, proofs, qp, xi, nq, dig, sums, status);
    return hipSuccess;
}
}

static std::atomic<unsigned long> g_stub_allocs(0);
extern "C" unsigned long starkhip_stub_allocations(void) { return g_stub_allocs.load(); }
extern "C" void starkhip_stub_commit_counters(unsigned long out[4]) {
    out[0] = starkhip::g_fake_launches.load(); out[1] = starkhip::g_fake_lane_grids.load(); out[2] = starkhip::g_fake_lane_members.load();
    out[3] = starkhip::g_service_records.load();
}
extern "C" {
hipError_t hipSetDevice(int) { return hipSuccess; }
hipError_t hipGetDevice(int* d) { *d = 0; return hipSuccess; }
hipError_t hipGetLastError(void) { return hipSuccess; }
hipError_t hipStreamCreateWithFlags(hipStream_t* s, unsigned) { g_stub_allocs++; *s = (hipStream_t)malloc(1); return hipSuccess; }
hipError_t hipStreamCreateWithPriority(hipStream_t* s, unsigned, int) { g_stub_allocs++; *s = (hipStream_t)malloc(1); return hipSuccess; }
hipError_t hipDeviceGetStreamPriorityRange(int* least, int* greatest) { *least = 1; *greatest = -1; return hipSuccess; }
hipError_t hipStreamDestroy(hipStream_t s) { free((void*)s); return hipSuccess; }
hipError_t hipStreamSynchronize(hipStream_t) { return hipSuccess; }
hipError_t hipStreamQuery(hipStream_t) { return hipSuccess; }
hipError_t hipStreamWaitEvent(hipStream_t, hipEvent_t, unsigned) { return hipSuccess; }
hipError_t hipEventRecord(hipEvent_t, hipStream_t s) { if (s) starkhip::g_service_records++; return hipSuccess; }
hipError_t hipEventSynchronize(hipEvent_t) { return hipSuccess; }
hipError_t hipEventQuery(hipEvent_t) { return hipSuccess; }
hipError_t hipHostMalloc(void** p, size_t bytes, unsigned) { g_stub_allocs++; *p = malloc(bytes ? bytes : 1); return *p ? hipSuccess : hipErrorOutOfMemory; }
hipError_t hipHostFree(void* p) { free(p); return hipSuccess; }
hipError_t hipMalloc(void** p, size_t bytes) { g_stub_allocs++; *p = malloc(bytes ? bytes : 1); return *p ? hipSuccess : hipErrorOutOfMemory; }
hipError_t hipFree(void* p) { free(p); return hipSuccess; }
hipError_t hipMemcpy(void* d, const void* s, size_t n, hipMemcpyKind) { if (n) memcpy(d, s, n); return hipSuccess; }
hipError_t hipMemcpyAsync(void* d, const void* s, size_t n, hipMemcpyKind, hipStream_t) { if (n) memcpy(d, s, n); return hipSuccess; }
hipError_t hipMemsetAsync(void* d, int v, size_t n, hipStream_t) { if (n) memset(d, v, n); return hipSuccess; }
hipError_t hipEventCreate(hipEvent_t* e) { g_stub_allocs++; *e = (hipEvent_t)malloc(1); return hipSuccess; }
hipError_t hipEventCreateWithFlags(hipEvent_t* e, unsigned) { g_stub_allocs++; *e = (hipEvent_t)malloc(1); return hipSuccess; }
hipError_t hipEventDestroy(hipEvent_t e) { free((void*)e); return hipSuccess; }
hipError_t hipEventElapsedTime(float* ms, hipEvent_t, hipEvent_t) { *ms = 0; return hipSuccess; }
}
```

starky_bls12_381_amd/csrc/kernel_entries.hip:

```cpp
#include <hip/hip_runtime.h>

#include <algorithm>
#include <vector>

#include "ctx.h"
#include "kernels_permutation.h"
#include "permutation.h"

namespace starkhip {

int permutation_zs(Ctx* c, const AirInfo& air, const TraceInput& in, const uint64_t* challenges, uint64_t* zs_out, uint64_t* closing_out) {
    const AirProgram& P = air.prog;
    const size_t n = in.n_rows, C = in.n_cols, nZ = P.perm_zs(), B = P.perm_batch_size();
    HIPCHK(hipSetDevice(c->device));
    const std::vector<uint32_t> cols = perm_columns(P), desc = perm_descriptor(P, true);
    Ctx::PermBufs& pb = c->perm;
    HIPCHK(c->values.ensure(C * n * 8));
    HIPCHK(c->lde.ensure(C * n * 8));
    HIPCHK(pb.cols.ensure(cols.size() * n * 8));
    HIPCHK(pb.desc.ensure(desc.size() * 4));
    HIPCHK(pb.chal.ensure(B * 4 * 8));
    HIPCHK(pb.zvals.ensure(nZ * n * 8));
    HIPCHK(pb.scan.ensure((perm_scratch_words(n, (unsigned)nZ) + nZ) * 8));
    const gl_t* d_values = nullptr;
// ... 60 lines not shown
    HIPCHK(c->values.ensure(words * 8));
    HIPCHK(c->lde.ensure(words * 8));
    HIPCHK(hipMemcpyAsync(c->values.p, data, words * 8, hipMemcpyHostToDevice, c->st));
    if (int rc = run_ntt(c, c->values.as<gl_t>(), c->lde.as<gl_t>(), n_vecs, (size_t)1 << log_len, log_len, inverse != 0, nullptr, nullptr)) return rc;
    HIPCHK(hipMemcpyAsync(data, c->values.p, words * 8, hipMemcpyDeviceToHost, c->st));
    HIPCHK(stream_wait(c));
    return STARKHIP_OK;
}

int lde_bench(Ctx* c, size_t n_cols, unsigned log_n, unsigned rate_bits, unsigned reps, unsigned const_per_64, const uint64_t* device_values, float* ms_out, float* each_ms) {
    if (log_n < 1 || log_n > STARKHIP_MAX_LOG_ROWS || rate_bits > 8 || !n_cols) return STARKHIP_ERR_BAD_SHAPE;
    HIPCHK(hipSetDevice(c->device));
    int rc;
    if ((rc = ensure_tables(c, log_n, rate_bits, 0))) return rc;
    const size_t n = (size_t)1 << log_n, N = n << rate_bits;
    const bool long_cols = lde_long_supported(log_n);
    HIPCHK(c->values.ensure(n_cols * n * 8 * (long_cols ? 2 : 1)));
    HIPCHK(c->lde.ensure(n_cols * N * 8));
    const gl_t* in = device_values ? (const gl_t*)device_values : c->values.as<gl_t>();
    gl_t* const cf = long_cols ? c->values.as<gl_t>() + n_cols * n : nullptr;
    if (device_values) const_per_64 = 0;
    else HIPCHK(launch_fill_powers(c->values.as<gl_t>(), 3, GL_GENERATOR, n_cols * n, c->st));
    const bool unit = (const_per_64 & 256u) != 0, prewarm = (const_per_64 & 1024u) != 0, touch = (const_per_64 & 2048u) != 0;
    const_per_64 &= 255u;
    for (size_t c0 = 0; const_per_64 && c0 < n_cols; c0 += 64) {
        const size_t cnt = std::min<size_t>(const_per_64, n_cols - c0);
        HIPCHK(hipMemsetAsync(c->values.as<gl_t>() + c0 * n, unit ? 0 : 1, cnt * n * 8, c->st));
        for (size_t k = 0; unit && k < cnt; k++) HIPCHK(hipMemsetAsync(c->values.as<gl_t>() + (c0 + k) * n + ((c0 + k) * 37) % n, 1, 1, c->st));
    }
    const bool cold = reps == 0;
    if (cold) reps = 1;
    reps = std::min(reps, 16u);
    std::vector<hipEvent_t> ev(reps + 1, nullptr);
    hipError_t err = hipSuccess;
    for (hipEvent_t& e : ev)
        if (err == hipSuccess) err = hipEventCreate(&e);
    if (err == hipSuccess && cold && touch) err = hipMemsetAsync(c->lde.p, 0, n_cols * N * 8, c->st);
    if (err == hipSuccess && cold && prewarm)
        for (int k = 0; k < 4 && err == hipSuccess; k++) err = run_lde(c, in, cf, c->lde.as<gl_t>(), std::min<size_t>(n_cols, 4096), log_n, rate_bits, 0);
    if (err == hipSuccess) err = cold ? hipStreamSynchronize(c->st) : run_lde(c, in, cf, c->lde.as<gl_t>(), n_cols, log_n, rate_bits, 0);
    if (err == hipSuccess) err = hipEventRecord(ev[0], c->st);
    for (unsigned r = 0; r < reps && err == hipSuccess; r++) {
        err = run_lde(c, in, cf, c->lde.as<gl_t>(), n_cols, log_n, rate_bits, 0);
        if (err == hipSuccess) err = hipEventRecord(ev[r + 1], c->st);
    }
    if (err == hipSuccess) err = hipEventSynchronize(ev[reps]);
    float ms = 0;
    if (err == hipSuccess) err = hipEventElapsedTime(&ms, ev[0], ev[reps]);
    for (unsigned r = 0; r < reps && err == hipSuccess && each_ms; r++) err = hipEventElapsedTime(&each_ms[r], ev[r], ev[r + 1]);
    for (hipEvent_t e : ev)
        if (e) (void)hipEventDestroy(e);
    HIPCHK(err);
    *ms_out = ms / reps;
    return STARKHIP_OK;
}

int expand_log(Ctx* c, const TraceLog* log, uint64_t* out_colmajor) {
    HIPCHK(hipSetDevice(c->device));
    const size_t nw = log->total_words(), nr = log->total_records(), nz = log->total_late_zeros();
    std::vector<uint32_t> h(nw + nr + nz);
    for (const LogPiece& pc : recording_pieces(*log)) std::copy(pc.src, pc.src + pc.words, h.begin() + pc.at);
    const size_t cells = log->rows * log->cols;
    HIPCHK(c->values.ensure(cells * 8));
    HIPCHK(c->staging.ensure(std::max<size_t>(h.size(), 1) * 4));
    uint32_t* d = c->staging.as<uint32_t>();
    if (!h.empty()) HIPCHK(hipMemcpyAsync(d, h.data(), h.size() * 4, hipMemcpyHostToDevice, c->st));
    HIPCHK(hipMemsetAsync(c->values.p, 0, cells * 8, c->st));
    if (nr) HIPCHK(launch_expand_trace(d, d + nw, nr, c->values.as<gl_t>(), log->rows, c->st));
    if (nz) HIPCHK(launch_zero_cells(d + nw + nr, nz / 2, c->values.as<gl_t>(), log->rows, c->st));
    HIPCHK(hipMemcpyAsync(out_colmajor, c->values.p, cells * 8, hipMemcpyDeviceToHost, c->st));
    HIPCHK(stream_wait(c));
    return STARKHIP_OK;
}

int merkle_cap(Ctx* c, const uint64_t* lde_natural, size_t n_cols, unsigned log_N, unsigned cap_h, uint64_t* cap_out) {
    if (log_N < cap_h) return STARKHIP_ERR_BAD_SHAPE;
    HIPCHK(hipSetDevice(c->device));
    const size_t N = (size_t)1 << log_N;
    HIPCHK(c->lde.ensure(n_cols * N * 8));
    HIPCHK(c->digests.ensure(digest_words(N) * 8));
    HIPCHK(hipMemcpyAsync(c->lde.p, lde_natural, n_cols * N * 8, hipMemcpyHostToDevice, c->st));
    int form;
    HIPCHK(launch_leaf_hash_lone(c, c->lde.as<gl_t>(), n_cols, log_N, 0, c->digests.as<gl_t>(), c->st, &form));
    HIPCHK(launch_merkle_levels(c->digests.as<gl_t>(), log_N, cap_h, c->st));
    HIPCHK(hipMemcpyAsync(cap_out, c->digests.as<gl_t>() + 4 * level_off(N, log_N - cap_h), ((size_t)4 << cap_h) * 8, hipMemcpyDeviceToHost, c->st));
    HIPCHK(stream_wait(c));
    return STARKHIP_OK;
}

int permute_batch(Ctx* c, uint64_t* states, size_t n) {
    HIPCHK(hipSetDevice(c->device));
    HIPCHK(c->staging.ensure(n * 12 * 8));
    HIPCHK(hipMemcpyAsync(c->staging.p, states, n * 96, hipMemcpyHostToDevice, c->st));
    HIPCHK(launch_permute_batch(c->staging.as<gl_t>(), n, c->st));
    HIPCHK(hipMemcpyAsync(states, c->staging.p, n * 96, hipMemcpyDeviceToHost, c->st));
    HIPCHK(stream_wait(c));
    return STARKHIP_OK;
}

int keccak_permute_batch(Ctx* c, uint64_t* states, size_t n) {
    if (n == 0) return STARKHIP_OK;
    if (!states) return STARKHIP_ERR_BAD_SHAPE;
    HIPCHK(hipSetDevice(c->device));
    HIPCHK(c->staging.ensure(n * 96));
    HIPCHK(hipMemcpyAsync(c->staging.p, states, n * 96, hipMemcpyHostToDevice, c->st));
    HIPCHK(launch_permute_batch_keccak(c->staging.as<gl_t>(), n, c->st));
    HIPCHK(hipMemcpyAsync(states, c->staging.p, n * 96, hipMemcpyDeviceToHost, c->st));
    HIPCHK(stream_wait(c));
    return STARKHIP_OK;
}

int merkle_tree_hasher(Ctx* c, int hasher, const uint64_t* lde_natural, size_t n_cols, unsigned log_N, unsigned cap_h, uint64_t* digests_out, uint64_t* cap_out) {
    if (hasher < STARKHIP_HASHER_POSEIDON || hasher > STARKHIP_HASHER_KECCAK || !lde_natural || !cap_out || !n_cols || log_N < cap_h || log_N > 28)
        return STARKHIP_ERR_BAD_SHAPE;
    HIPCHK(hipSetDevice(c->device));
    const size_t N = (size_t)1 << log_N;
    HIPCHK(c->lde.ensure(n_cols * N * 8));
    HIPCHK(c->digests.ensure(digest_words(N) * 8));
    HIPCHK(hipMemcpyAsync(c->lde.p, lde_natural, n_cols * N * 8, hipMemcpyHostToDevice, c->st));
    int form;
    if (hasher == STARKHIP_HASHER_KECCAK) HIPCHK(launch_leaf_hash_keccak(c->lde.as<gl_t>(), n_cols, log_N, 0, c->digests.as<gl_t>(), c->st));
    else HIPCHK(launch_leaf_hash_lone(c, c->lde.as<gl_t>(), n_cols, log_N, 0, c->digests.as<gl_t>(), c->st, &form));
    HIPCHK(launch_merkle_levels_by(hasher, c->digests.as<gl_t>(), log_N, cap_h, c->st));
    if (digests_out) HIPCHK(hipMemcpyAsync(digests_out, c->digests.p, 4 * N * 8, hipMemcpyDeviceToHost, c->st));
    HIPCHK(hipMemcpyAsync(cap_out, c->digests.as<gl_t>() + 4 * level_off(N, log_N - cap_h), ((size_t)4 << cap_h) * 8, hipMemcpyDeviceToHost, c->st));
    HIPCHK(stream_wait(c));
    return STARKHIP_OK;
}

int hash_rows_hasher(Ctx* c, int hasher, const uint64_t* rows, size_t width, size_t n_leaves, uint64_t* digests_out) {
    if (hasher < STARKHIP_HASHER_POSEIDON || hasher > STARKHIP_HASHER_KECCAK || !rows || !digests_out || !width || !n_leaves || width > ((size_t)1 << 24) ||
        n_leaves > ((size_t)1 << 28))
        return STARKHIP_ERR_BAD_SHAPE;
    HIPCHK(hipSetDevice(c->device));
    HIPCHK(c->staging.ensure((width + 4) * n_leaves * 8));
    gl_t* d_rows = c->staging.as<gl_t>();
    gl_t* d_dig = d_rows + width * n_leaves;
    HIPCHK(hipMemcpyAsync(d_rows, rows, width * n_leaves * 8, hipMemcpyHostToDevice, c->st));
    HIPCHK(launch_leaf_hash_rows_by(hasher, d_rows, width, n_leaves, d_dig, c->st));
    HIPCHK(hipMemcpyAsync(digests_out, d_dig, 4 * n_leaves * 8, hipMemcpyDeviceToHost, c->st));
    HIPCHK(stream_wait(c));
    return STARKHIP_OK;
}

int permute_batch_form(Ctx* c, int form, int variant, uint64_t* states, size_t n) {
    if (variant < 0 || (unsigned)variant >= permute_form_variants(form)) return STARKHIP_ERR_BAD_SHAPE;
    if (n == 0) return STARKHIP_OK;
    if (!states) return STARKHIP_ERR_BAD_SHAPE;
    HIPCHK(hipSetDevice(c->device));
    HIPCHK(c->staging.ensure(2 * n * 96));
    gl_t* in = c->staging.as<gl_t>();
    HIPCHK(hipMemcpyAsync(in, states, n * 96, hipMemcpyHostToDevice, c->st));
    HIPCHK(launch_permute_batch_form(form, variant, in, in + 12 * n, n, c->st));
    HIPCHK(hipMemcpyAsync(states, in + 12 * n, n * 96, hipMemcpyDeviceToHost, c->st));
    HIPCHK(stream_wait(c));
    return STARKHIP_OK;
}

int leaf_hash_lane_group(Ctx* c, const uint64_t* mats, size_t n_segments, size_t n_cols, unsigned log_n, unsigned rate_bits, int grouped, int form,
                         unsigned prefix_mask, uint64_t* digests_out) {
    if (!mats || !digests_out || n_segments == 0 || n_segments > 4 || n_cols == 0 || log_n + rate_bits > 20 || n_cols > ((size_t)1 << 20)) return STARKHIP_ERR_BAD_SHAPE;
    if ((form != FORM_LANE && form != FORM_PAIR) || (grouped && form != FORM_LANE) || (prefix_mask >> n_segments) != 0) return STARKHIP_ERR_BAD_SHAPE;
    HIPCHK(hipSetDevice(c->device));
    LeafPrefix pf;
    if (prefix_mask && leaf_prefix_wanted(c, ((size_t)1 << log_n) + 8, log_n, rate_bits)) {
        if (int rc = ensure_tables(c, log_n, rate_bits, 0)) return rc;
        if (int rc = ensure_leaf_prefix(c, log_n, rate_bits)) return rc;
        pf = leaf_prefix(c);
    }
    const size_t N = (size_t)1 << (log_n + rate_bits), mat_words = n_cols * N, dig_words = 4 * N;
    HIPCHK(c->staging.ensure(n_segments * (mat_words + dig_words) * 8));
    gl_t* d_mats = c->staging.as<gl_t>();
    gl_t* d_dig = d_mats + n_segments * mat_words;
    HIPCHK(hipMemcpyAsync(d_mats, mats, n_segments * mat_words * 8, hipMemcpyHostToDevice, c->st));
    HIPCHK(hipMemsetAsync(d_dig, 0xEE, n_segments * dig_words * 8, c->st));
    LeafHashBatch B = {};
    for (size_t s = 0; s < n_segments; s++) {
        B.mat[s] = d_mats + s * mat_words;
        B.digests[s] = d_dig + s * dig_words;
        if (prefix_mask >> s & 1u) {
            B.prefix_count[s] = pf.count;
            B.prefix_cap[s] = pf.cap;
        }
    }
    if (grouped) {
        HIPCHK(launch_leaf_hash_lane_group(B, (unsigned)n_segments, n_cols, log_n, rate_bits, c->st));
    } else {
        for (size_t s = 0; s < n_segments; s++) HIPCHK(launch_leaf_hash_form((LeafHashForm)form, B.mat[s], n_cols, log_n, rate_bits, B.digests[s], c->st, LeafPrefix{B.prefix_count[s], B.prefix_cap[s]}));
    }
    HIPCHK(hipMemcpyAsync(digests_out, d_dig, n_segments * dig_words * 8, hipMemcpyDeviceToHost, c->st));
    HIPCHK(stream_wait(c));
    return STARKHIP_OK;
}

int leaf_prefix_table(Ctx* c, unsigned log_n, unsigned rate_bits, uint64_t* cap_out) {
    if (!cap_out || log_n > STARKHIP_MAX_LOG_ROWS || rate_bits > 8 || !leaf_prefix_wanted(c, ((size_t)1 << log_n) + 8, log_n, rate_bits)) return STARKHIP_ERR_BAD_SHAPE;
    HIPCHK(hipSetDevice(c->device));
    if (int rc = ensure_tables(c, log_n, rate_bits, 0)) return rc;
    if (int rc = ensure_leaf_prefix(c, log_n, rate_bits)) return rc;
    HIPCHK(hipMemcpyAsync(cap_out, c->tab->leaf_prefix.p, leaf_prefix_words(log_n, rate_bits) * 8, hipMemcpyDeviceToHost, c->st));
    HIPCHK(stream_wait(c));
    return STARKHIP_OK;
}

int field_ops(Ctx* c, int op, const uint64_t* a, const uint64_t* b, uint64_t* out, size_t n) {
    HIPCHK(hipSetDevice(c->device));
    HIPCHK(c->staging.ensure(3 * n * 8));
    gl_t* d = c->staging.as<gl_t>();
// ... 28 lines not shown
```

starky_bls12_381_amd/csrc/kernels.h:

```cpp
#pragma once
#include <hip/hip_runtime.h>
#include <stdint.h>

#include "gl.h"
#include "poseidon_tables.h"

#ifndef STARKHIP_NO_PRIO
#define STARKHIP_PRIO_ENTRY __builtin_amdgcn_s_setprio(2);
#else
#define STARKHIP_PRIO_ENTRY
#endif

namespace starkhip {
struct QOp;
struct QTRec;
struct QTStream;
struct QTContrib;
struct VQProof;
struct VQLeaf;
}

namespace starkhip {

hipError_t launch_fill_powers(gl_t* out, gl_t base, gl_t mult, size_t count, hipStream_t st);
hipError_t launch_fill_coset_scale(gl_t* out, unsigned log_n, unsigned rate_bits, hipStream_t st);
hipError_t launch_transpose(const gl_t* in, gl_t* out, size_t rows, size_t cols, hipStream_t st);
hipError_t launch_expand_trace(const uint32_t* words, const uint32_t* offsets, size_t n_records, gl_t* values, size_t n_rows, hipStream_t st);
hipError_t launch_zero_cells(const uint32_t* col_row, size_t n_cells, gl_t* values, size_t n_rows, hipStream_t st);
hipError_t launch_lde_columns(const gl_t* values, gl_t* coeffs, gl_t* lde, size_t n_cols, unsigned log_n, unsigned rate_bits,
                              const gl_t* tw_fwd, const gl_t* tw_inv, unsigned tw_log, const gl_t* coset_scale, int from_coeffs,
                              hipStream_t st);
bool lde_v2_supported(unsigned log_n);
size_t lde_v2_tw_words(unsigned log_n);
size_t lde_v2_oh_words(unsigned log_n, unsigned rate_bits);
hipError_t lde_v2_upload_tables(unsigned log_n, unsigned rate_bits, gl_t* d_tw_fwd, gl_t* d_tw_inv, gl_t* d_cs, gl_t* d_oh, hipStream_t st);
hipError_t launch_lde_columns_v2(const gl_t* values, gl_t* coeffs, gl_t* lde, size_t n_cols, unsigned log_n, unsigned rate_bits,
                                 const gl_t* tw_fwd, const gl_t* tw_inv, const gl_t* cs, const gl_t* oh, int from_coeffs, hipStream_t st,
                                 unsigned col_base = 0, unsigned* unit_count = nullptr);
bool lde_wave_supported(unsigned log_n);
size_t lde_wave_table_words(unsigned rate_bits);
hipError_t lde_wave_upload_tables(unsigned rate_bits, gl_t* d_tab, hipStream_t st);
hipError_t launch_lde_columns_wave(const gl_t* values, gl_t* lde, size_t n_cols, unsigned rate_bits, const gl_t* d_tab, const gl_t* oh, unsigned* next,
                                   hipStream_t st, unsigned col_base = 0, unsigned* unit_count = nullptr);
bool lde_long_supported(unsigned log_n);
size_t lde_long_sub_words();
hipError_t lde_long_upload_sub_tables(gl_t* d_sub, hipStream_t st);
hipError_t lde_long_fill_twiddles(gl_t* d_fwd, gl_t* d_inv, unsigned log_n, hipStream_t st);
struct LdeLongTables {
    const gl_t *sub, *tw_fwd, *tw_inv;
};
hipError_t launch_lde_columns_long(const gl_t* values, gl_t* coeffs, gl_t* lde, size_t n_cols, unsigned log_n, unsigned rate_bits, const LdeLongTables& tb,
                                   const gl_t* cs, int from_coeffs, hipStream_t st);
hipError_t launch_ntt_long(const gl_t* src, gl_t* mid, gl_t* dst, size_t n_vecs, size_t vec_stride, unsigned log_n, bool inverse, const gl_t* pre_scale,
                           const gl_t* post_scale, const LdeLongTables& tb, hipStream_t st);
hipError_t launch_ntt_global(gl_t* data, size_t n_vecs, size_t vec_stride, unsigned log_n, const gl_t* tw, unsigned tw_log,
                             const gl_t* pre_scale, const gl_t* post_scale, gl_t final_mul, hipStream_t st);

static const unsigned LEAF_HASH_MAX_BATCH = 64;
struct LeafPrefix {
    const unsigned* count = nullptr;
    const gl_t* cap = nullptr;
};
size_t leaf_prefix_words(unsigned log_n, unsigned rate_bits);
hipError_t launch_leaf_prefix_build(const gl_t* oh, unsigned log_n, unsigned rate_bits, gl_t* cap, hipStream_t st);
struct LeafHashBatch {
    const gl_t* mat[LEAF_HASH_MAX_BATCH];
    gl_t* digests[LEAF_HASH_MAX_BATCH];
    const unsigned* prefix_count[LEAF_HASH_MAX_BATCH];
    const gl_t* prefix_cap[LEAF_HASH_MAX_BATCH];
};
hipError_t launch_leaf_hash_multi(const LeafHashBatch& B, unsigned count, size_t n_cols, unsigned log_n, unsigned rate_bits, hipStream_t st);
hipError_t launch_leaf_hash_lane_group(const LeafHashBatch& B, unsigned count, size_t n_cols, unsigned log_n, unsigned rate_bits, hipStream_t st);
enum LeafHashForm : int {
    FORM_AUTO = 0,
    FORM_QUAD = 1,
    FORM_ROW = 2,
    FORM_LANE = 3,
    FORM_PAIR = 4,
};
enum LeafHashSent : int {
    SENT_QUAD = 0,
    SENT_ROW = 1,
    SENT_MERGED = 2,
    SENT_LANE = 3,
    SENT_HOST = 4,
    SENT_PAIR = 5,
    SENT_KECCAK = 6,
};
inline LeafHashSent leaf_hash_sent(LeafHashForm form) {
    return form == FORM_ROW ? SENT_ROW : form == FORM_LANE ? SENT_LANE : form == FORM_PAIR ? SENT_PAIR : SENT_QUAD;
}
hipError_t launch_leaf_hash_form(LeafHashForm form, const gl_t* mat, size_t n_cols, unsigned log_n, unsigned rate_bits, gl_t* digests, hipStream_t st,
                                 LeafPrefix prefix = LeafPrefix());
hipError_t upload_table_once(const void* symbol, const void* image, size_t bytes, bool (&done)[64]);
hipError_t launch_leaf_hash_rows(const gl_t* rows, size_t width, size_t n_leaves, gl_t* digests, hipStream_t st);
hipError_t launch_merkle_levels(gl_t* digests, unsigned log_leaves, unsigned cap_h, hipStream_t st);
hipError_t launch_permute_batch(gl_t* states, size_t n, hipStream_t st);
inline unsigned permute_form_variants(int form) {
    switch (form) {
        case FORM_AUTO: case FORM_ROW: return 1u;
        case FORM_QUAD: case FORM_LANE: case FORM_PAIR: return 2u;
    }
    return 0u;
}
hipError_t launch_permute_quad_form(bool cap_only, const gl_t* in, gl_t* out, size_t n, hipStream_t st);
hipError_t launch_permute_batch_form(int form, int variant, const gl_t* in, gl_t* out, size_t n, hipStream_t st);
hipError_t launch_pow_grind(const gl_t* base_state, int pos, unsigned pow_bits, uint64_t start, uint64_t count, unsigned long long* best,
                            hipStream_t st);
hipError_t launch_leaf_hash_keccak(const gl_t* mat, size_t n_cols, unsigned log_n, unsigned rate_bits, gl_t* digests, hipStream_t st);
hipError_t launch_leaf_hash_rows_keccak(const gl_t* rows, size_t width, size_t n_leaves, gl_t* digests, hipStream_t st);
hipError_t launch_merkle_levels_keccak(gl_t* digests, unsigned log_leaves, unsigned cap_h, hipStream_t st);
hipError_t launch_permute_batch_keccak(gl_t* states, size_t n, hipStream_t st);
hipError_t launch_pow_grind_keccak(const gl_t* base_state, int pos, unsigned pow_bits, uint64_t start, uint64_t count, unsigned long long* best,
                                   hipStream_t st);
inline hipError_t launch_leaf_hash_rows_by(int hasher, const gl_t* rows, size_t width, size_t n_leaves, gl_t* digests, hipStream_t st) {
    return hasher ? launch_leaf_hash_rows_keccak(rows, width, n_leaves, digests, st) : launch_leaf_hash_rows(rows, width, n_leaves, digests, st);
}
inline hipError_t launch_merkle_levels_by(int hasher, gl_t* digests, unsigned log_leaves, unsigned cap_h, hipStream_t st) {
    return hasher ? launch_merkle_levels_keccak(digests, log_leaves, cap_h, st) : launch_merkle_levels(digests, log_leaves, cap_h, st);
}
hipError_t launch_field_ops(int op, const gl_t* a, const gl_t* b, gl_t* out, size_t n, hipStream_t st);

hipError_t launch_quotient_tables(gl_t* tab, unsigned log_n, unsigned qdb, hipStream_t st);
hipError_t launch_quotient_eval(const QOp* ops, const uint32_t* loads, unsigned n_slots, const uint32_t* chunk_batch, unsigned n_chunks,
                                const gl_t* pis, const gl_t* lde, const gl_t* tab, const gl_t* apow, gl_t alpha0, gl_t alpha1, gl_t* partial,
                                unsigned log_n, unsigned rate_bits, unsigned qdb, hipStream_t st);
hipError_t launch_quotient_combine(const gl_t* partial, const gl_t* chunk_scale, unsigned n_chunks, const gl_t* tab, unsigned log_n,
                                   unsigned qdb, gl_t* out, hipStream_t st);

hipError_t launch_quotient_weights(QTRec* recs, const uint32_t* contrib_off, const QTContrib* contribs, uint32_t n_recs, gl_t* apow, uint32_t K,
                                   const gl_t* consts, const gl_t* pis, gl_t alpha0, gl_t alpha1, hipStream_t st);
hipError_t launch_quotient_tiles(const QTRec* recs, const QTStream* streams, const uint32_t* chunk_tile_off,
                                 const uint32_t* tile_list, unsigned n_chunks, const gl_t* lde, const gl_t* tab, gl_t* partial, unsigned log_n,
                                 unsigned rate_bits, unsigned qdb, unsigned n_cols, unsigned dbg, hipStream_t st, const uint32_t* work = nullptr,
                                 unsigned n_work = 0, unsigned n_accs = 1);
hipError_t launch_quotient_class_sums(const gl_t* partial, const uint32_t* sum_off, const uint32_t* vec_slot, unsigned n_vecs, unsigned n_slots,
                                      const gl_t* tab, unsigned log_n, unsigned qdb, gl_t* out, hipStream_t st);
hipError_t launch_quotient_class_solve(const gl_t* a, const uint32_t* vec_of, unsigned n_classes, const gl_t* solve, unsigned log_n, unsigned qdb,
                                       gl_t* out, hipStream_t st);
hipError_t launch_quotient_tiles_combine(const gl_t* partial, unsigned n_chunks, const gl_t* tab, unsigned log_n, unsigned qdb, gl_t* out,
                                         hipStream_t st);

struct CheckView {
    const QOp* ops;
    const uint32_t* chunk_op;
    const gl_t* trace;
    const gl_t* pis;
    const uint32_t* chunk_k0;
    unsigned n_chunks, log_n;
};
hipError_t launch_check_trace(const CheckView& v, unsigned long long* out, hipStream_t st);
hipError_t launch_check_report_count(const CheckView& v, uint32_t* counts, unsigned long long* row_mask, hipStream_t st);
hipError_t launch_check_report_list(const CheckView& v, const uint32_t* chunks, unsigned n_launched, uint32_t* cursors, const unsigned long long* row_mask,
                                    const uint32_t* base, unsigned long long* list, uint32_t list_len, hipStream_t st);

struct FreeCon;
hipError_t launch_free_cell_classes(const CheckView& v, const FreeCon* cons, const uint32_t* pivots, uint32_t n_constraints, gl_t delta,
                                    unsigned long long* planes, size_t plane_words, uint32_t* open_rows, hipStream_t st);
hipError_t launch_free_cell_classes_count(const unsigned long long* planes, size_t plane_words, uint32_t n_cols, unsigned log_n,
                                          uint32_t* per_column, hipStream_t st);

hipError_t launch_ext_powers(gl2_t* out, gl2_t base, size_t count, hipStream_t st);
hipError_t launch_coset_weights(gl2_t* wz, gl2_t* wgz, gl2_t z, gl2_t scale, unsigned log_n, hipStream_t st);
hipError_t launch_openings(const gl_t* coeffs, size_t stride, size_t n_polys, size_t n, const gl2_t* zpow, const gl2_t* gzpow, gl2_t* out_z,
                           gl2_t* out_gz, hipStream_t st);
hipError_t launch_fri_combine(const gl_t* coeffs, size_t stride, size_t n_polys, size_t n, const gl2_t* apow, size_t polys_per_chunk,
                              size_t n_chunks, gl2_t* partial, hipStream_t st);
hipError_t launch_ext_reduce(const gl2_t* partial, size_t n_chunks, size_t n, gl_t* out, hipStream_t st);
hipError_t launch_fri_leaves(const gl_t* vals, unsigned log_len, unsigned arity_bits, gl_t* rows, hipStream_t st);
hipError_t launch_fri_fold(const gl_t* in, size_t len, unsigned arity_bits, gl2_t beta, gl_t* out, hipStream_t st);

hipError_t launch_query_leaf_colmajor(const gl_t* mat, size_t n_cols, unsigned log_n, unsigned rate_bits, const uint32_t* xs, size_t n_queries,
                                      gl_t* out, size_t stride, size_t off, hipStream_t st);
hipError_t launch_query_leaf_rows(const gl_t* rows, size_t width, const uint32_t* xs, unsigned shift, size_t n_queries, gl_t* out, size_t stride,
                                  size_t off, hipStream_t st);
hipError_t launch_query_path(const gl_t* digests, size_t n_leaves, unsigned depth, const uint32_t* xs, unsigned shift, size_t n_queries, gl_t* out,
                             size_t stride, size_t off, hipStream_t st);

hipError_t launch_verify_leaf_digests(const gl_t* words, const VQLeaf* leaves, size_t n_leaves, gl_t* digests, unsigned hashers, hipStream_t st);
hipError_t launch_verify_leaf_digests_keccak(const gl_t* words, const VQLeaf* leaves, size_t n_leaves, gl_t* digests, hipStream_t st);
hipError_t launch_verify_range(const gl_t* words, const VQProof* proofs, size_t n_proofs, uint32_t* bad, hipStream_t st);
hipError_t launch_verify_combine(const gl_t* words, const VQProof* proofs, const uint32_t* query_proof, size_t n_queries, const gl2_t* apow,
                                 gl2_t* sums, hipStream_t st);
hipError_t launch_verify_queries(const gl_t* words, const VQProof* proofs, const uint32_t* query_proof, const uint64_t* x_index, size_t n_queries,
                                 const gl_t* digests, const gl2_t* sums, uint32_t* status, hipStream_t st);

}
```

starky_bls12_381_amd/csrc/kernels_hash.hip:

```cpp
#include <hip/hip_runtime.h>

#include <mutex>

#include "kernels.h"
#include "poseidon_dev.h"
#include "verify_query.h"

namespace starkhip {

__constant__ QuadMergedTables QUAD_MERGED;
__constant__ RowMergedTables ROW_MERGED;
static bool quad_uploaded[64], row_uploaded[64], lane_uploaded[64], pair_uploaded[64];

__device__ __forceinline__ void leaf_hash_body(const gl_t* __restrict__ mat, size_t n_cols, unsigned log_n, unsigned rate_bits,
                                               gl_t* __restrict__ digests) {
    __shared__ RcPair rcs[4][96];
    for (unsigned idx = threadIdx.x; idx < 4 * 96; idx += blockDim.x) {
        const unsigned ll = idx / 96, w = idx % 96;
        const gl_t c = w < 90 ? POSEIDON_RC_DEV[12 * (w / 3) + ll + 4 * (w % 3)] : 0;
        rcs[ll][w].lo = c & 0xFFFFFFFFull;
        rcs[ll][w].hi = c >> 32;
    }
    __shared__ RcPair tks[2 * QUAD_MERGED_TRIPLES];
    __shared__ RcPair tk3s[4][3 * QUAD_MERGED_TRIPLES];
    for (unsigned idx = threadIdx.x; idx < 2 * QUAD_MERGED_TRIPLES; idx += blockDim.x) tks[idx] = QUAD_MERGED.tk[idx];
    for (unsigned idx = threadIdx.x; idx < 4 * 3 * QUAD_MERGED_TRIPLES; idx += blockDim.x)
        tk3s[idx / (3 * QUAD_MERGED_TRIPLES)][idx % (3 * QUAD_MERGED_TRIPLES)] = QUAD_MERGED.tk3[idx / (3 * QUAD_MERGED_TRIPLES)][idx % (3 * QUAD_MERGED_TRIPLES)];
    __syncthreads();
    const unsigned log_N = log_n + rate_bits;
    const size_t N = (size_t)1 << log_N;
    const size_t tid = blockIdx.x * (size_t)blockDim.x + threadIdx.x;
    const unsigned l = (unsigned)tid & 3u;
    const size_t q = tid >> 2;
    if (q >= N) return;
    const size_t s = q >> log_n, k = q & (((size_t)1 << log_n) - 1);
    const size_t i = (k << rate_bits) + s;
    const size_t j = gl_bitrev((uint32_t)i, log_N);
    const gl_t* col = mat + q;
    if (n_cols <= 4) {
        digests[4 * j + l] = l < n_cols ? col[(size_t)l * N] : 0;
        return;
    }
    const uint32_t diag0 = l == 0 ? 8u : 0u;
    const RcPair* rc = rcs[l];
    QuadMergedCoef mc;
    {
        const uint32_t* c = QUAD_MERGED.coef[l];
#pragma unroll
        for (int e = 0; e < 36; e++) mc.n3[e / 12][e % 12] = c[e];
#pragma unroll
        for (int e = 0; e < 3; e++) {
            mc.n1[e] = c[36 + e];
            mc.n2[e] = c[39 + e];
            mc.b2[e] = c[43 + e];
            mc.b3[e] = c[46 + e];
        }
        mc.m00 = c[42];
#pragma unroll
        for (int e = 0; e < 12; e++) mc.cf[e] = c[50 + e];
    }
    const RcPair* tk3 = tk3s[l];
    const bool even_lane = (l & 1u) == 0;
    gl_t s0 = 0, s1 = 0, s2 = 0;
    const gl_t* mine = col + (size_t)l * N;
    const size_t n_full = n_cols / 8, rem = n_cols % 8;
    gl_t n0 = 0, n1 = 0;
    if (n_full) {
        n0 = mine[0];
        n1 = mine[4 * N];
    }
    for (size_t b = 0; b < n_full; b++) {
        s0 = n0;
        s1 = n1;
        if (b + 1 < n_full) {
            n0 = mine[(8 * (b + 1)) * N];
            n1 = mine[(8 * (b + 1) + 4) * N];
            poseidon_permute_quad_merged<true>(s0, s1, s2, diag0, rc, mc, tks, tk3, l == 0, even_lane);
        } else {
            poseidon_permute_quad_merged<false>(s0, s1, s2, diag0, rc, mc, tks, tk3, l == 0, even_lane);
        }
    }
    if (rem) {
        const size_t off = 8 * n_full;
        if (l < rem) s0 = mine[off * N];
        if (l + 4 < rem) s1 = mine[(off + 4) * N];
        poseidon_permute_quad_merged<false>(s0, s1, s2, diag0, rc, mc, tks, tk3, l == 0, even_lane);
    }
// ... 448 lines not shown
    const size_t N = (size_t)1 << (log_n + rate_bits);
    hipLaunchKernelGGL(leaf_prefix_build_kernel, dim3(nblocks(N, 64)), dim3(64), 0, st, oh, log_n, rate_bits, cap);
    return hipGetLastError();
}

hipError_t upload_table_once(const void* symbol, const void* image, size_t bytes, bool (&done)[64]) {
    static std::mutex mu;
    int dev = 0;
    hipError_t e = hipGetDevice(&dev);
    if (e != hipSuccess) return e;
    std::lock_guard<std::mutex> g(mu);
    if (dev < 0 || dev >= 64) return hipErrorInvalidDevice;
    if (done[dev]) return hipSuccess;
    if (!image) return hipErrorInvalidValue;
    e = hipMemcpyToSymbol(symbol, image, bytes);
    if (e == hipSuccess) done[dev] = true;
    return e;
}
static hipError_t ensure_quad_merged_tables() { return upload_table_once(&QUAD_MERGED, quad_merged_tables_host(), sizeof QUAD_MERGED, quad_uploaded); }
static hipError_t ensure_row_merged_tables() { return upload_table_once(&ROW_MERGED, row_merged_tables_host(), sizeof ROW_MERGED, row_uploaded); }
static hipError_t ensure_lane_tables() { return upload_table_once(&LANE_TABLES, lane_tables_host(), sizeof LANE_TABLES, lane_uploaded); }
static hipError_t ensure_pair_tables() { return upload_table_once(&PAIR_TABLES, pair_tables_host(), sizeof PAIR_TABLES, pair_uploaded); }

hipError_t launch_leaf_hash_form(LeafHashForm form, const gl_t* mat, size_t n_cols, unsigned log_n, unsigned rate_bits, gl_t* digests, hipStream_t st,
                                 LeafPrefix prefix) {
    const size_t N = (size_t)1 << (log_n + rate_bits);
    switch (form) {
        case FORM_QUAD:
            if (hipError_t e = ensure_quad_merged_tables(); e != hipSuccess) return e;
            hipLaunchKernelGGL(leaf_hash_kernel, dim3(nblocks(4 * N, 256)), dim3(256), 0, st, mat, n_cols, log_n, rate_bits, digests);
            break;
        case FORM_ROW:
            if (hipError_t e = ensure_row_merged_tables(); e != hipSuccess) return e;
            hipLaunchKernelGGL(leaf_hash_row_kernel, dim3(nblocks(16 * N, 256)), dim3(256), 0, st, mat, n_cols, log_n, rate_bits, digests);
            break;
        case FORM_LANE:
            if (hipError_t e = ensure_lane_tables(); e != hipSuccess) return e;
            {
                LeafHashBatch B = {};
                B.mat[0] = mat;
                B.digests[0] = digests;
                B.prefix_count[0] = prefix.count;
                B.prefix_cap[0] = prefix.cap;
                hipLaunchKernelGGL(leaf_hash_lane_kernel, dim3(nblocks(N, 256)), dim3(256), 0, st, B, n_cols, log_n, rate_bits);
            }
            break;
        case FORM_PAIR:
            if (hipError_t e = ensure_pair_tables(); e != hipSuccess) return e;
            hipLaunchKernelGGL(leaf_hash_pair_kernel, dim3(nblocks(N, 128)), dim3(256), 0, st, mat, n_cols, log_n, rate_bits, digests, prefix.count, prefix.cap);
            break;
        default: return hipErrorInvalidValue;
    }
    return hipGetLastError();
}
hipError_t launch_verify_leaf_digests(const gl_t* words, const VQLeaf* leaves, size_t n_leaves, gl_t* digests, unsigned hashers, hipStream_t st) {
    if (!n_leaves) return hipSuccess;
    if (hashers & (1u << STARKHIP_HASHER_POSEIDON)) {
        if (hipError_t e = ensure_row_merged_tables(); e != hipSuccess) return e;
        hipLaunchKernelGGL(verify_leaf_digest_kernel, dim3(nblocks(16 * n_leaves, 256)), dim3(256), 0, st, words, leaves, n_leaves, digests);
        if (hipError_t e = hipGetLastError(); e != hipSuccess) return e;
    }
    if (hashers & (1u << STARKHIP_HASHER_KECCAK)) return launch_verify_leaf_digests_keccak(words, leaves, n_leaves, digests, st);
    return hipSuccess;
}
hipError_t launch_leaf_hash_multi(const LeafHashBatch& B, unsigned count, size_t n_cols, unsigned log_n, unsigned rate_bits, hipStream_t st) {
    if (count == 0 || count > LEAF_HASH_MAX_BATCH) return hipErrorInvalidValue;
    size_t N = (size_t)1 << (log_n + rate_bits);
    if (hipError_t e = ensure_quad_merged_tables(); e != hipSuccess) return e;
    if (count == 1) hipLaunchKernelGGL(leaf_hash_kernel, dim3(nblocks(4 * N, 256)), dim3(256), 0, st, B.mat[0], n_cols, log_n, rate_bits, B.digests[0]);
    else hipLaunchKernelGGL(leaf_hash_multi_kernel, dim3(nblocks(4 * N, 256), count), dim3(256), 0, st, B, n_cols, log_n, rate_bits);
    return hipGetLastError();
}
hipError_t launch_leaf_hash_lane_group(const LeafHashBatch& B, unsigned count, size_t n_cols, unsigned log_n, unsigned rate_bits, hipStream_t st) {
    if (count == 0 || count > LEAF_HASH_MAX_BATCH) return hipErrorInvalidValue;
    const size_t N = (size_t)1 << (log_n + rate_bits);
    if (hipError_t e = ensure_lane_tables(); e != hipSuccess) return e;
    hipLaunchKernelGGL(leaf_hash_lane_kernel, dim3(nblocks(N, 256), count), dim3(256), 0, st, B, n_cols, log_n, rate_bits);
    return hipGetLastError();
}
hipError_t launch_leaf_hash_rows(const gl_t* rows, size_t width, size_t n_leaves, gl_t* digests, hipStream_t st) {
    hipLaunchKernelGGL(leaf_hash_rows_kernel, dim3(nblocks(n_leaves, 64)), dim3(64), 0, st, rows, width, n_leaves, digests);
    return hipGetLastError();
}
hipError_t launch_merkle_levels(gl_t* digests, unsigned log_leaves, unsigned cap_h, hipStream_t st) {
    gl_t* child = digests;
    for (unsigned lv = log_leaves; lv > cap_h; lv--) {
        size_t n_parent = (size_t)1 << (lv - 1);
        gl_t* parent = child + ((size_t)4 << lv);
        hipLaunchKernelGGL(merkle_level_kernel, dim3(nblocks(n_parent, 64)), dim3(64), 0, st, child, parent, n_parent);
        hipError_t e = hipGetLastError();
        if (e != hipSuccess) return e;
        child = parent;
    }
    return hipSuccess;
}
hipError_t launch_permute_batch(gl_t* states, size_t n, hipStream_t st) {
    hipLaunchKernelGGL(permute_batch_kernel, dim3(nblocks(n, 64)), dim3(64), 0, st, states, n);
    return hipGetLastError();
}
hipError_t launch_permute_batch_form(int form, int variant, const gl_t* in, gl_t* out, size_t n, hipStream_t st) {
    if (variant < 0 || (unsigned)variant >= permute_form_variants(form) || n == 0) return hipErrorInvalidValue;
    switch (form) {
        case FORM_AUTO:
            if (hipError_t e = hipMemcpyAsync(out, in, n * 96, hipMemcpyDeviceToDevice, st); e != hipSuccess) return e;
            return launch_permute_batch(out, n, st);
        case FORM_QUAD: return launch_permute_quad_form(variant != 0, in, out, n, st);
        case FORM_ROW:
            if (hipError_t e = ensure_row_merged_tables(); e != hipSuccess) return e;
            hipLaunchKernelGGL(permute_row_form_kernel, dim3(nblocks(16 * n, 256)), dim3(256), 0, st, in, out, n);
            break;
        case FORM_LANE:
            if (hipError_t e = ensure_lane_tables(); e != hipSuccess) return e;
            if (variant) hipLaunchKernelGGL(permute_lane_form_kernel<true>, dim3(nblocks(n, 256)), dim3(256), 0, st, in, out, n);
            else hipLaunchKernelGGL(permute_lane_form_kernel<false>, dim3(nblocks(n, 256)), dim3(256), 0, st, in, out, n);
            break;
        default:
            if (hipError_t e = ensure_pair_tables(); e != hipSuccess) return e;
            if (variant) hipLaunchKernelGGL(permute_pair_form_kernel<true>, dim3(nblocks(n, 128)), dim3(256), 0, st, in, out, n);
            else hipLaunchKernelGGL(permute_pair_form_kernel<false>, dim3(nblocks(n, 128)), dim3(256), 0, st, in, out, n);
    }
    return hipGetLastError();
}
hipError_t launch_pow_grind(const gl_t* base_state, int pos, unsigned pow_bits, uint64_t start, uint64_t count, unsigned long long* best,
                            hipStream_t st) {
    hipLaunchKernelGGL(pow_grind_kernel, dim3(nblocks(count, 256)), dim3(256), 0, st, base_state, pos, pow_bits, start, count, best);
    return hipGetLastError();
}

}
```

starky_bls12_381_amd/csrc/kernels_keccak.hip:

```cpp
#include <hip/hip_runtime.h>

#include "keccak.h"
#include "kernels.h"
#include "verify_query.h"

namespace starkhip {

__global__ __launch_bounds__(64) void leaf_hash_keccak_kernel(const gl_t* __restrict__ mat, size_t n_cols, unsigned log_n, unsigned rate_bits,
                                                              gl_t* __restrict__ digests) { STARKHIP_PRIO_ENTRY
    const unsigned log_N = log_n + rate_bits;
    const size_t N = (size_t)1 << log_N;
    const size_t q = blockIdx.x * (size_t)blockDim.x + threadIdx.x;
    if (q >= N) return;
    const size_t s = q >> log_n, k = q & (((size_t)1 << log_n) - 1);
    const size_t i = (k << rate_bits) + s;
    const size_t j = gl_bitrev((uint32_t)i, log_N);
    const gl_t* col = mat + q;
    gl_t w[4];
    if (n_cols <= 3) {
        keccak_digest_words(col[0], n_cols > 1 ? col[N] : 0, n_cols > 2 ? col[2 * N] : 0, 0, w);
    } else {
        uint64_t a[25], nx[KECCAK_RATE_WORDS];
#pragma unroll
        for (int e = 0; e < 25; e++) a[e] = 0;
        const size_t n_blocks = n_cols / KECCAK_RATE_WORDS + 1;
        size_t rem = n_cols < KECCAK_RATE_WORDS ? n_cols : KECCAK_RATE_WORDS;
#pragma unroll
        for (int e = 0; e < KECCAK_RATE_WORDS; e++) nx[e] = (size_t)e < rem ? col[(size_t)e * N] : 0;
        for (size_t b = 0; b < n_blocks; b++) {
#pragma unroll
            for (int e = 0; e < KECCAK_RATE_WORDS; e++) a[e] ^= nx[e];
            if (b + 1 == n_blocks) {
#pragma unroll
                for (int e = 0; e < KECCAK_RATE_WORDS; e++) {
                    if ((size_t)e == rem) a[e] ^= 0x01ULL;
                }
                a[16] ^= KECCAK_PAD_LAST;
            } else {
                const size_t off = (b + 1) * KECCAK_RATE_WORDS;
                rem = n_cols - off < KECCAK_RATE_WORDS ? n_cols - off : KECCAK_RATE_WORDS;
#pragma unroll
                for (int e = 0; e < KECCAK_RATE_WORDS; e++) nx[e] = (size_t)e < rem ? col[(off + e) * N] : 0;
            }
            keccak_f1600(a);
        }
        keccak_digest_words(a[0], a[1], a[2], a[3], w);
    }
#pragma unroll
    for (int e = 0; e < 4; e++) digests[4 * j + e] = w[e];
}

__global__ __launch_bounds__(64) void leaf_hash_rows_keccak_kernel(const gl_t* __restrict__ rows, size_t width, size_t n_leaves,
                                                                   gl_t* __restrict__ digests) { STARKHIP_PRIO_ENTRY
    const size_t j = blockIdx.x * (size_t)blockDim.x + threadIdx.x;
    if (j >= n_leaves) return;
    gl_t w[4];
    keccak_hash_or_noop(rows + j * width, width, 1, w);
#pragma unroll
    for (int e = 0; e < 4; e++) digests[4 * j + e] = w[e];
}

__global__ __launch_bounds__(64) void merkle_level_keccak_kernel(const gl_t* __restrict__ child, gl_t* __restrict__ parent, size_t n_parent) { STARKHIP_PRIO_ENTRY
    const size_t j = blockIdx.x * (size_t)blockDim.x + threadIdx.x;
    if (j >= n_parent) return;
    gl_t w[4];
    keccak_two_to_one(child + 8 * j, child + 8 * j + 4, w);
#pragma unroll
    for (int e = 0; e < 4; e++) parent[4 * j + e] = w[e];
}

__global__ __launch_bounds__(64) void keccak_permute_batch_kernel(gl_t* states, size_t n) { STARKHIP_PRIO_ENTRY
    const size_t i = blockIdx.x * (size_t)blockDim.x + threadIdx.x;
    if (i >= n) return;
    gl_t s[12];
#pragma unroll
    for (int e = 0; e < 12; e++) s[e] = states[12 * i + e];
    keccak_permute(s);
#pragma unroll
    for (int e = 0; e < 12; e++) states[12 * i + e] = s[e];
}

__global__ __launch_bounds__(256) void pow_grind_keccak_kernel(const gl_t* __restrict__ base_state, int pos, unsigned pow_bits, uint64_t start,
                                                               uint64_t count, unsigned long long* best) { STARKHIP_PRIO_ENTRY
    const uint64_t t = blockIdx.x * (uint64_t)blockDim.x + threadIdx.x;
    if (t >= count) return;
    const uint64_t w = start + t;
    gl_t s[12];
#pragma unroll
    for (int e = 0; e < 12; e++) s[e] = e == pos ? w : base_state[e];
    keccak_permute(s);
    if ((s[7] >> (64 - pow_bits)) == 0) atomicMin(best, (unsigned long long)w);
}

__global__ __launch_bounds__(64) void verify_leaf_digest_keccak_kernel(const gl_t* __restrict__ words, const VQLeaf* __restrict__ leaves,
                                                                       size_t n_leaves, gl_t* __restrict__ digests) { STARKHIP_PRIO_ENTRY
    const size_t q = blockIdx.x * (size_t)blockDim.x + threadIdx.x;
    if (q >= n_leaves) return;
    const VQLeaf lf = leaves[q];
    if (lf.hasher != STARKHIP_HASHER_KECCAK) return;
    gl_t w[4];
    keccak_hash_or_noop(words + lf.off, lf.len, 1, w);
    gl_t* out = digests + 4 * (size_t)lf.slot;
#pragma unroll
    for (int e = 0; e < 4; e++) out[e] = w[e];
}

static inline unsigned nblocks(size_t n, unsigned bs) { return (unsigned)((n + bs - 1) / bs); }

hipError_t launch_leaf_hash_keccak(const gl_t* mat, size_t n_cols, unsigned log_n, unsigned rate_bits, gl_t* digests, hipStream_t st) {
    const size_t N = (size_t)1 << (log_n + rate_bits);
    hipLaunchKernelGGL(leaf_hash_keccak_kernel, dim3(nblocks(N, 64)), dim3(64), 0, st, mat, n_cols, log_n, rate_bits, digests);
    return hipGetLastError();
}
hipError_t launch_leaf_hash_rows_keccak(const gl_t* rows, size_t width, size_t n_leaves, gl_t* digests, hipStream_t st) {
    hipLaunchKernelGGL(leaf_hash_rows_keccak_kernel, dim3(nblocks(n_leaves, 64)), dim3(64), 0, st, rows, width, n_leaves, digests);
    return hipGetLastError();
}
hipError_t launch_merkle_levels_keccak(gl_t* digests, unsigned log_leaves, unsigned cap_h, hipStream_t st) {
    gl_t* child = digests;
    for (unsigned lv = log_leaves; lv > cap_h; lv--) {
        const size_t n_parent = (size_t)1 << (lv - 1);
        gl_t* parent = child + ((size_t)4 << lv);
        hipLaunchKernelGGL(merkle_level_keccak_kernel, dim3(nblocks(n_parent, 64)), dim3(64), 0, st, child, parent, n_parent);
        if (hipError_t e = hipGetLastError(); e != hipSuccess) return e;
        child = parent;
    }
    return hipSuccess;
}
hipError_t launch_permute_batch_keccak(gl_t* states, size_t n, hipStream_t st) {
    if (!n) return hipSuccess;
    hipLaunchKernelGGL(keccak_permute_batch_kernel, dim3(nblocks(n, 64)), dim3(64), 0, st, states, n);
    return hipGetLastError();
}
hipError_t launch_pow_grind_keccak(const gl_t* base_state, int pos, unsigned pow_bits, uint64_t start, uint64_t count, unsigned long long* best,
                                   hipStream_t st) {
    hipLaunchKernelGGL(pow_grind_keccak_kernel, dim3(nblocks(count, 256)), dim3(256), 0, st, base_state, pos, pow_bits, start, count, best);
    return hipGetLastError();
}
hipError_t launch_verify_leaf_digests_keccak(const gl_t* words, const VQLeaf* leaves, size_t n_leaves, gl_t* digests, hipStream_t st) {
    if (!n_leaves) return hipSuccess;
    hipLaunchKernelGGL(verify_leaf_digest_keccak_kernel, dim3(nblocks(n_leaves, 64)), dim3(64), 0, st, words, leaves, n_leaves, digests);
    return hipGetLastError();
}

}
```

starky_bls12_381_amd/csrc/prover.h:

```cpp
#pragma once
#include <stddef.h>
#include <stdint.h>

#include "airs.h"
#include "lookup_columns.h"
#include "trace_input.h"

namespace starkhip {

struct Ctx;
int ctx_create(int device, Ctx** out, int priority = 0);
void ctx_destroy(Ctx* c);
const float* ctx_timings(Ctx* c);
const float* ctx_kernel_timings(Ctx* c);
const float* ctx_host_timings(Ctx* c);
void ctx_commit_info(Ctx* c, int* form, unsigned* group);
int ctx_set_option(Ctx* c, const char* name, long value);
class HashService;
void ctx_attach_hash_service(Ctx* c, HashService* hs);
bool ctx_has_hash_service(Ctx* c);
int ctx_set_urgent(Ctx* c, bool urgent);
void ctx_set_check_trace(Ctx* c, bool on, size_t list_cap);
void ctx_set_hasher(Ctx* c, int hasher);
void ctx_check_stats(Ctx* c, uint64_t out[2]);
int ctx_reserve(Ctx* c, const AirInfo& air, const starkhip_config_t& cfg, size_t log_bytes, unsigned proof_blobs = 0, bool device_traces = false);
void ctx_hash_request_reset(Ctx* c);
bool ctx_hash_requested(Ctx* c);

struct Pool;
int pool_create(const starkhip_pool_config_t& cfg, Pool** out, unsigned cpu_share = 1);
void pool_destroy(Pool* p);
int pool_submit(Pool* p, int air, const starkhip_config_t* cfg, const TraceInput& in, const uint64_t* pis, size_t n_pis, uint64_t pow, uint64_t* ticket);
int pool_submit_witness(Pool* p, int air, const starkhip_config_t* cfg, const uint32_t* operands, size_t n_limbs, uint64_t pow, uint64_t* ticket);
int pool_wait(Pool* p, uint64_t ticket, uint64_t** proof, size_t* words, starkhip_ticket_info_t* info);
int pool_stats(Pool* p, starkhip_pool_stats_t* out);
int pool_reservation(Pool* p, starkhip_pool_reservation_t* out);
int pool_host_info(Pool* p, starkhip_pool_host_info_t* out);
int pool_set_option(Pool* p, const char* name, long value);
int pool_submit_verify(Pool* p, int air, const starkhip_config_t* cfg, const uint64_t* proof, size_t words, uint64_t* ticket);
int pool_verify_stats(Pool* p, starkhip_pool_verify_stats_t* out);
int pool_check_stats(Pool* p, uint64_t out[2]);
double air_verify_cost(int air);
unsigned cpu_budget();
void host_cpu_seconds(double out[3]);
struct MultiPool;
double air_cost(int air);
int multipool_create(const int* devices, size_t n, const starkhip_pool_config_t& cfg, MultiPool** out);
void multipool_destroy(MultiPool* mp);
size_t multipool_size(const MultiPool* mp);
Pool* multipool_pool(MultiPool* mp, size_t slot);
int multipool_device(const MultiPool* mp, size_t slot);
int multipool_submit(MultiPool* mp, int slot, int air, const starkhip_config_t* cfg, const TraceInput& in, const uint64_t* pis, size_t n_pis, uint64_t pow,
                     uint64_t* ticket);
int multipool_submit_witness(MultiPool* mp, int slot, int air, const starkhip_config_t* cfg, const uint32_t* operands, size_t n_limbs, uint64_t pow,
                             uint64_t* ticket);
int multipool_submit_witness_batch(MultiPool* mp, size_t n, const int* airs, const uint32_t* const* operands, const size_t* n_limbs, uint64_t pow,
                                   uint64_t* tickets, int* rcs);
int multipool_ticket_slot(const MultiPool* mp, uint64_t ticket);
int multipool_wait(MultiPool* mp, uint64_t ticket, uint64_t** proof, size_t* words, starkhip_ticket_info_t* info);
int multipool_set_option(MultiPool* mp, const char* name, long value);
int multipool_submit_verify(MultiPool* mp, int slot, int air, const starkhip_config_t* cfg, const uint64_t* proof, size_t words, uint64_t* ticket);
int multipool_verify_batch(MultiPool* mp, size_t n, const int* airs, const starkhip_config_t* cfgs, const uint64_t* const* proofs, const size_t* words,
                           int* results);
void plan_verify(size_t n, const int* airs, size_t n_pools, int* slots, size_t* order);
void plan_lpt(size_t n, const int* airs, size_t n_pools, int* slots);
size_t ctx_device_bytes(Ctx* c);
size_t ctx_pinned_bytes(Ctx* c);

int prove(Ctx* c, const AirInfo& air, const starkhip_config_t& cfg, const TraceInput& in, const uint64_t* pis, size_t n_pis, uint64_t pow_witness,
          uint64_t** proof_out, size_t* proof_words);
int check_trace(Ctx* c, const AirInfo& air, const TraceInput& in, const uint64_t* pis, uint64_t* violations, uint64_t first[3]);
int check_trace_report(Ctx* c, const AirInfo& air, const TraceInput& in, const uint64_t* pis, uint32_t* per_constraint, uint64_t* row_mask,
                       uint64_t* list, size_t cap, starkhip_check_report_t* out);
int check_trace_free_cells(Ctx* c, const AirInfo& air, const TraceInput& in, const uint64_t* pis, uint64_t delta, uint32_t* per_column,
                           uint64_t* free_mask, starkhip_free_cells_t* out);
int check_trace_free_cell_classes(Ctx* c, const AirInfo& air, const TraceInput& in, const uint64_t* pis, uint64_t delta, uint32_t* per_column,
                                  uint64_t* planes, uint32_t* open_rows, starkhip_free_cell_classes_t* out);
int check_trace_permutations(Ctx* c, const AirInfo& air, const TraceInput& in, uint64_t seed, uint32_t* per_pair, uint64_t* masks, uint64_t* list,
                             size_t cap, starkhip_perm_check_t* out);
void perm_check_timings(Ctx* c, float ms[4]);
int lookup_columns(Ctx* c, const LookupTrace& tr, const starkhip_lookup_t* lookups, size_t n_lookups, uint32_t* per_lookup, uint64_t* masks,
                   uint64_t* list, size_t cap, starkhip_lookup_report_t* out);
void lookup_timings(Ctx* c, float ms[4]);
int ntt_long(Ctx* c, uint64_t* data, size_t n_vecs, unsigned log_len, int inverse);
int lde_batch(Ctx* c, const uint64_t* values, size_t n_cols, unsigned log_n, unsigned rate_bits, uint64_t* coeffs_out, uint64_t* lde_out);
int merkle_cap(Ctx* c, const uint64_t* lde_natural, size_t n_cols, unsigned log_N, unsigned cap_h, uint64_t* cap_out);
int permute_batch(Ctx* c, uint64_t* states, size_t n);
int keccak_permute_batch(Ctx* c, uint64_t* states, size_t n);
int merkle_tree_hasher(Ctx* c, int hasher, const uint64_t* lde_natural, size_t n_cols, unsigned log_N, unsigned cap_h, uint64_t* digests_out, uint64_t* cap_out);
int hash_rows_hasher(Ctx* c, int hasher, const uint64_t* rows, size_t width, size_t n_leaves, uint64_t* digests_out);
int permute_batch_form(Ctx* c, int form, int variant, uint64_t* states, size_t n);
int leaf_hash_lane_group(Ctx* c, const uint64_t* mats, size_t n_segments, size_t n_cols, unsigned log_n, unsigned rate_bits, int grouped, int form,
                         unsigned prefix_mask, uint64_t* digests_out);
int leaf_prefix_table(Ctx* c, unsigned log_n, unsigned rate_bits, uint64_t* cap_out);
int expand_log(Ctx* c, const TraceLog* log, uint64_t* out_colmajor);
int lde_bench(Ctx* c, size_t n_cols, unsigned log_n, unsigned rate_bits, unsigned reps, unsigned const_per_64, const uint64_t* device_values, float* ms_out, float* each_ms = nullptr);
int field_ops(Ctx* c, int op, const uint64_t* a, const uint64_t* b, uint64_t* out, size_t n);
int permutation_zs(Ctx* c, const AirInfo& air, const TraceInput& in, const uint64_t* challenges, uint64_t* zs_out, uint64_t* closing_out);
int host_alloc(Ctx* c, size_t bytes, void** out);
void host_free(void* p);

int verify_proof(const AirInfo& air, const starkhip_config_t& cfg, const uint64_t* proof, size_t words);

}
```

starky_bls12_381_amd/csrc/prover.hip:

```cpp
#include <hip/hip_runtime.h>

#include <stdio.h>
#include <stdlib.h>
#include <string.h>

#include <algorithm>
#include <chrono>
#include <vector>

#include "airs.h"
#include "blob_arena.h"
#include "check_report.h"
#include "ctx.h"
#include "kernels.h"
#include "kernels_permutation.h"
#include "lde_ranges.h"
#include "permutation.h"
#include "trace_log.h"
#include "poseidon.h"
#include "proof.h"
#include "quotient_ops.h"
#include "quotient_plan.h"
#include "prover.h"
#include "scheduler.h"
// ... 208 lines not shown
    return 0;
}

int ProveCall::upload() {
    int rc;
    switch (in.form) {
        case TraceForm::Recording: rc = upload_recording(in.log); break;
        case TraceForm::ColumnTable: rc = upload_column_table(in.columns); break;
        default: rc = upload_dense(c, in, d_trace, &d_values);
    }
    if (rc == 0 && c->opt_check_trace) rc = check_trace_in_prove(c, air, d_values, s.n, pis_host, &out, &check_words);
    if (rc == 0 && s.nZ) {
        const std::vector<uint32_t> cols = perm_columns(air.prog);
        for (size_t k = 0; k < cols.size(); k++)
            HIPCHK(hipMemcpyAsync(c->perm.cols.as<gl_t>() + k * s.n, d_values + (size_t)cols[k] * s.n, s.n * 8, hipMemcpyDeviceToDevice, st));
    }
    return rc;
}

int ProveCall::ifft_lde() {
    HIPCHK(hipEventRecord(c->kev[4], st));
    if (lde_long_supported(s.log_n)) HIPCHK(run_lde(c, d_values, c->values.as<gl_t>(), c->lde.as<gl_t>(), s.C, s.log_n, s.r, 0));
    else {
        HIPCHK(leaf_prefix_reset(c));
        HIPCHK(run_lde_trace(c, d_values, c->lde.as<gl_t>(), c->values.as<gl_t>(), s.C, s.log_n, s.r, trace_in_lde, prefix ? leaf_prefix_counter(c) : nullptr));
    }
    HIPCHK(hipEventRecord(c->kev[5], st));
    return 0;
}

int ProveCall::leaf_hash_on_host() {
    const size_t n = s.n, N = s.N, C = s.C;
    const unsigned r = s.r, log_N = s.log_N;
    if (c->hs && !HashService::is_big(s.log_n, r)) {
        c->hs->abandon_small();
        c->hash_requested = true;
    }
    c->hash_timing.form = SENT_HOST;
    c->hash_timing.group = 1;
    c->host_lde.resize(C * N);
    HIPCHK(hipMemcpyAsync(c->host_lde.data(), c->lde.p, C * N * 8, hipMemcpyDeviceToHost, st));
    HIPCHK(stream_wait(c));
    std::vector<gl_t> leaf_digests(4 * N);
    const gl_t* lde_h = c->host_lde.data();
    const unsigned n_thr = (unsigned)std::min<size_t>(N, std::max(1u, cpu_budget()));
    run_on_helpers(n_thr, [&](unsigned w) {
        for (size_t j = w; j < N; j += n_thr) {
            size_t i = 0;
            for (unsigned b = 0; b < log_N; b++) i |= ((j >> b) & 1) << (log_N - 1 - b);
            const size_t s_ = i & (((size_t)1 << r) - 1), k_ = i >> r;
            gl_t state[12] = {0};
            const gl_t* col = lde_h + s_ * n + k_;
            for (size_t off = 0; off < C; off += 8) {
                const size_t cnt = std::min<size_t>(8, C - off);
                for (size_t e = 0; e < cnt; e++) state[e] = col[(off + e) * N];
                poseidon_permute_host(state);
            }
            for (int e = 0; e < 4; e++) leaf_digests[4 * j + e] = state[e];
        }
    });
    HIPCHK(hipMemcpyAsync(c->digests.p, leaf_digests.data(), 4 * N * 8, hipMemcpyHostToDevice, st));
    HIPCHK(stream_wait(c));
    return 0;
}

int ProveCall::trace_merkle() {
    const LeafPrefix pf = prefix ? leaf_prefix(c) : LeafPrefix();
    HIPCHK(hipEventRecord(c->kev[0], st));
    if (c->opt_hasher == STARKHIP_HASHER_KECCAK) {
        c->hash_timing.form = SENT_KECCAK;
        c->hash_timing.group = 1;
        HIPCHK(launch_leaf_hash_keccak(c->lde.as<gl_t>(), s.C, s.log_n, s.r, c->digests.as<gl_t>(), st));
    } else if (s.N <= (size_t)c->opt_host_commit_leaves && s.C >= 64 && c->opt_leaf_hash_form == FORM_AUTO) {
        if (int rc = leaf_hash_on_host()) return rc;
    } else if (c->hs) {
        c->hash_requested = true;
        HIPCHK(c->hs->hash(c->lde.as<gl_t>(), s.C, s.log_n, s.r, c->digests.as<gl_t>(), st, c->hash_ready, c->hash_done, !HashService::is_big(s.log_n, s.r), c->urgent,
                           &c->hash_timing, pf));
    } else {
        c->hash_timing.group = 1;
        HIPCHK(launch_leaf_hash_lone(c, c->lde.as<gl_t>(), s.C, s.log_n, s.r, c->digests.as<gl_t>(), st, &c->hash_timing.form, pf));
    }
    HIPCHK(hipEventRecord(c->kev[1], st));
    HIPCHK(launch_merkle_levels_by((int)c->opt_hasher, c->digests.as<gl_t>(), s.log_N, s.cap_h, st));
    trace_cap.resize(4 * s.ncap);
    HIPCHK(read_back(c, trace_cap.data(), c->digests.as<gl_t>() + 4 * level_off(s.N, s.log_N - s.cap_h), 4 * s.ncap * 8, st));
    return 0;
}

int ProveCall::run_quotient_tiles(unsigned debug_mode, gl_t* qvals_out, bool timed) {
    const Ctx::PlanDev& D = *c->plan;
    HIPCHK(launch_quotient_weights(D.q_recs.as<QTRec>(), D.q_contrib_off.as<uint32_t>(), D.q_contribs.as<QTContrib>(), D.recs, D.q_apow.as<gl_t>(),
                                   air.prog.n_constraints, D.q_consts.as<gl_t>(), c->pis.as<gl_t>(), alphas[0], alphas[1], st));
    if (timed) HIPCHK(hipEventRecord(c->kev[2], st));
    HIPCHK(launch_quotient_tiles(D.q_recs.as<QTRec>(), D.q_streams.as<QTStream>(), D.q_chunk_tile_off.as<uint32_t>(), D.q_tile_list.as<uint32_t>(), D.chunks,
                                 c->lde.as<gl_t>(), c->tab->qtab.as<gl_t>(), c->partial.as<gl_t>(), s.log_n, s.r, s.qdb, (unsigned)s.C, debug_mode, st));
    if (timed) HIPCHK(hipEventRecord(c->kev[3], st));
    HIPCHK(launch_quotient_tiles_combine(c->partial.as<gl_t>(), D.chunks, c->tab->qtab.as<gl_t>(), s.log_n, s.qdb, qvals_out, st));
    return 0;
}

int ProveCall::run_quotient_classes() {
    const Ctx::PlanDev& D = *c->plan;
    HIPCHK(launch_quotient_weights(D.q_recs.as<QTRec>(), D.q_contrib_off.as<uint32_t>(), D.q_contribs.as<QTContrib>(), D.recs, D.q_apow.as<gl_t>(),
                                   air.prog.n_constraints, D.q_consts.as<gl_t>(), c->pis.as<gl_t>(), alphas[0], alphas[1], st));
    HIPCHK(hipEventRecord(c->kev[2], st));
    HIPCHK(launch_quotient_tiles(D.q_recs.as<QTRec>(), D.q_streams.as<QTStream>(), D.q_chunk_tile_off.as<uint32_t>(), D.q_tile_list.as<uint32_t>(), D.chunks,
                                 c->lde.as<gl_t>(), c->tab->qtab.as<gl_t>(), c->partial.as<gl_t>(), s.log_n, s.r, s.qdb, (unsigned)s.C, 0, st,
                                 D.q_work.as<uint32_t>(), D.n_work, D.n_classes));
    HIPCHK(hipEventRecord(c->kev[3], st));
    gl_t* const vecs = c->qclass.as<gl_t>();
    HIPCHK(launch_quotient_class_sums(c->partial.as<gl_t>(), D.q_sum_off.as<uint32_t>(), D.q_vec_slot.as<uint32_t>(), D.n_vecs, D.n_classes + 1,
                                      c->tab->qtab.as<gl_t>(), s.log_n, s.qdb, vecs, st));
    if (int rc = run_ntt(c, vecs, vecs + (size_t)2 * D.n_vecs * s.n, 2 * D.n_vecs, s.n, s.log_n, true, nullptr, nullptr)) return rc;
    HIPCHK(launch_quotient_class_solve(vecs, D.q_vec_of.as<uint32_t>(), D.n_classes, c->tab->qsolve.as<gl_t>(), s.log_n, s.qdb, c->qvals.as<gl_t>(), st));
    return 0;
}

int ProveCall::run_quotient_ops() {
    std::vector<gl_t> apow(2 * (AIR_MAX_GROUP + 1)), cscale(2 * n_chunks);
    for (int j = 0; j < 2; j++) {
        apow[j * (AIR_MAX_GROUP + 1)] = 1;
        for (unsigned m = 1; m <= AIR_MAX_GROUP; m++) apow[j * (AIR_MAX_GROUP + 1) + m] = gl_mul(apow[j * (AIR_MAX_GROUP + 1) + m - 1], alphas[j]);
        for (unsigned k = 0; k < n_chunks; k++) cscale[k * 2 + j] = gl_pow(alphas[j], c->prog.chunk_k_after[k]);
    }
    HIPCHK(hipMemcpyAsync(c->apow.p, apow.data(), apow.size() * 8, hipMemcpyHostToDevice, st));
    HIPCHK(hipMemcpyAsync(c->chunk_scale.p, cscale.data(), cscale.size() * 8, hipMemcpyHostToDevice, st));
    HIPCHK(hipEventRecord(c->kev[2], st));
    HIPCHK(launch_quotient_eval(c->prog.ops.as<QOp>(), c->prog.loads.as<uint32_t>(), c->prog.slots, c->prog.chunk_off.as<uint32_t>(), n_chunks,
                                c->pis.as<gl_t>(), c->lde.as<gl_t>(), c->tab->qtab.as<gl_t>(), c->apow.as<gl_t>(), alphas[0], alphas[1],
                                c->partial.as<gl_t>(), s.log_n, s.r, s.qdb, st));
    HIPCHK(hipEventRecord(c->kev[3], st));
    HIPCHK(launch_quotient_combine(c->partial.as<gl_t>(), c->chunk_scale.as<gl_t>(), n_chunks, c->tab->qtab.as<gl_t>(), s.log_n, s.qdb,
                                   c->qvals.as<gl_t>(), st));
    HIPCHK(stream_wait(c));
    return 0;
}

int ProveCall::compare_quotient_evaluators() {
    const size_t n = s.n, size = s.size, qdb = s.qdb;
    if (int rc = ensure_plan(c, air, size)) return rc;
    std::vector<gl_t> ref(2 * size), got(2 * size);
    HIPCHK(read_back(c, ref.data(), c->qvals.p, 2 * size * 8, st));
    HIPCHK(c->partial.ensure((size_t)std::max(n_chunks, c->plan->chunks) * 2 * size * 8));
    if (int rc = run_quotient_tiles(0, c->comb_partial.as<gl_t>(), false)) return rc;
    HIPCHK(read_back(c, got.data(), c->comb_partial.p, 2 * size * 8, st));
    HIPCHK(stream_wait(c));
    size_t bad = 0, last_blk = (size_t)-1;
    for (size_t i = 0; i < 2 * size; i++)
        if (ref[i] != got[i]) {
            const size_t ii = i % size, k = ii >> qdb, spp = ii & (((size_t)1 << qdb) - 1), tt = spp * n + k, blk = tt / 64;
            if (blk != last_blk && bad < 4096) fprintf(stderr, "quotient mismatch alpha %zu point-block %zu (sp %zu, k %zu..)\n", i / size, blk, spp, k & ~(size_t)63);
            last_blk = blk;
            bad++;
        }
    fprintf(stderr, "quotient compare: %zu of %zu values differ\n", bad, 2 * size);
    return 0;
}

int ProveCall::permutation() {
    const AirProgram& P = air.prog;
    const size_t n = s.n, nZ = s.nZ;
    fs.start();
    perm_chal.resize((size_t)P.perm_batch_size() * 4);
    for (gl_t& x : perm_chal) x = ch.get();
    fs.stop();
    perm_desc = perm_descriptor(P, true);
    const std::vector<uint32_t> by_col = perm_descriptor(P, false);
    perm_desc.insert(perm_desc.end(), by_col.begin(), by_col.end());
    Ctx::PermBufs& pb = c->perm;
    HIPCHK(hipMemcpyAsync(pb.desc.p, perm_desc.data(), perm_desc.size() * 4, hipMemcpyHostToDevice, st));
    HIPCHK(hipMemcpyAsync(pb.chal.p, perm_chal.data(), perm_chal.size() * 8, hipMemcpyHostToDevice, st));
    gl_t* const d_closing = pb.scan.as<gl_t>() + perm_scratch_words(n, (unsigned)nZ);
    HIPCHK(launch_perm_zs(pb.desc.as<uint32_t>(), pb.cols.as<gl_t>(), n, pb.chal.as<gl_t>(), n, (unsigned)nZ, pb.zvals.as<gl_t>(), pb.scan.as<gl_t>(), d_closing, st));
    std::vector<gl_t> closing(nZ);
    HIPCHK(read_back(c, closing.data(), d_closing, nZ * 8, st));
    HIPCHK(stream_wait(c));
    for (gl_t v : closing)
        if (v != 1) return STARKHIP_ERR_QUOTIENT_NOT_DIVISIBLE;
    HIPCHK(run_lde(c, pb.zvals.as<gl_t>(), lde_long_supported(s.log_n) ? pb.zcoef.as<gl_t>() : nullptr, pb.zlde.as<gl_t>(), nZ, s.log_n, s.r, 0));
    if (c->opt_hasher == STARKHIP_HASHER_KECCAK) HIPCHK(launch_leaf_hash_keccak(pb.zlde.as<gl_t>(), nZ, s.log_n, s.r, pb.zdigests.as<gl_t>(), st));
    else HIPCHK(launch_leaf_hash_form(FORM_QUAD, pb.zlde.as<gl_t>(), nZ, s.log_n, s.r, pb.zdigests.as<gl_t>(), st));
    HIPCHK(launch_merkle_levels_by((int)c->opt_hasher, pb.zdigests.as<gl_t>(), s.log_N, s.cap_h, st));
    zs_cap.resize(4 * s.ncap);
    HIPCHK(read_back(c, zs_cap.data(), pb.zdigests.as<gl_t>() + 4 * level_off(s.N, s.log_N - s.cap_h), 4 * s.ncap * 8, st));
    HIPCHK(stream_wait(c));
    fs.start();
    ch.observe_many(zs_cap.data(), zs_cap.size());
    fs.stop();
    return 0;
}

int ProveCall::quotient() {
    const size_t n = s.n, size = s.size, factor = s.factor;
    HIPCHK(stream_wait(c));
    fs.start();
    ch.observe_many(trace_cap.data(), trace_cap.size());
    fs.stop();
    if (s.nZ)
        if (int rc = permutation()) return rc;
    fs.start();
    alphas[0] = ch.get();
    alphas[1] = ch.get();
    fs.stop();
    if (s.pl.n_pis) HIPCHK(hipMemcpyAsync(c->pis.p, pis_host, s.pl.n_pis * 8, hipMemcpyHostToDevice, st));
    const unsigned debug = (unsigned)((c->opt_quotient_debug <= 4 || c->opt_quotient_debug == 8) ? c->opt_quotient_debug : 0);
    if (tiled && c->plan->by_class) {
        if (int rc = run_quotient_classes()) return rc;
    } else {
        if (int rc = tiled ? run_quotient_tiles(debug, c->qvals.as<gl_t>(), true) : run_quotient_ops()) return rc;
        if (c->opt_quotient_debug == 9 && !tiled)
            if (int rc = compare_quotient_evaluators()) return rc;
        if (s.nZ)
            HIPCHK(launch_perm_quotient(c->perm.desc.as<uint32_t>() + s.perm_desc_words, c->lde.as<gl_t>(), c->perm.zlde.as<gl_t>(), c->perm.chal.as<gl_t>(),
                                        c->tab->qtab.as<gl_t>(), c->qvals.as<gl_t>(), alphas[0], alphas[1], gl_pow(alphas[0], 2 * s.nZ), gl_pow(alphas[1], 2 * s.nZ),
                                        s.log_n, s.r, s.qdb, st));
        if (int rc = run_ntt(c, c->qvals.as<gl_t>(), c->partial.as<gl_t>(), 2, size, s.log_n + s.qdb, true, nullptr, c->tab->qshift_inv.as<gl_t>()))
            return rc;
    }
    if (size > factor * n) {
        quot_tail.resize(2 * (size - factor * n));
        for (int j = 0; j < 2; j++)
            HIPCHK(read_back(c, quot_tail.data() + j * (size - factor * n), c->qvals.as<gl_t>() + j * size + factor * n, (size - factor * n) * 8, st));
    }
    for (int j = 0; j < 2; j++)
        HIPCHK(hipMemcpyAsync(c->qcoef.as<gl_t>() + (size_t)j * factor * n, c->qvals.as<gl_t>() + j * size, factor * n * 8, hipMemcpyDeviceToDevice, st));
    return 0;
}

int ProveCall::quotient_commit() {
    HIPCHK(stream_wait(c));
    for (gl_t v : quot_tail)
        if (v != 0) return STARKHIP_ERR_QUOTIENT_NOT_DIVISIBLE;
    HIPCHK(run_lde(c, c->qcoef.as<gl_t>(), nullptr, c->qlde.as<gl_t>(), s.Q, s.log_n, s.r, 1));
    if (c->opt_hasher == STARKHIP_HASHER_KECCAK) HIPCHK(launch_leaf_hash_keccak(c->qlde.as<gl_t>(), s.Q, s.log_n, s.r, c->qdigests.as<gl_t>(), st));
    else HIPCHK(launch_leaf_hash_form(FORM_QUAD, c->qlde.as<gl_t>(), s.Q, s.log_n, s.r, c->qdigests.as<gl_t>(), st));
    HIPCHK(launch_merkle_levels_by((int)c->opt_hasher, c->qdigests.as<gl_t>(), s.log_N, s.cap_h, st));
    quot_cap.resize(4 * s.ncap);
    HIPCHK(read_back(c, quot_cap.data(), c->qdigests.as<gl_t>() + 4 * level_off(s.N, s.log_N - s.cap_h), 4 * s.ncap * 8, st));
    return 0;
}

int ProveCall::openings() {
    const size_t n = s.n, C = s.C, Q = s.Q, nZ = s.nZ;
    HIPCHK(stream_wait(c));
    fs.start();
    ch.observe_many(quot_cap.data(), quot_cap.size());
    zeta = ch.get_ext();
    fs.stop();
    if (c->opt_zeta_on_coset > 0)
        zeta = gl2_make(gl_mul(GL_GENERATOR, gl_pow(gl_root_of_unity(s.log_n), (uint64_t)(c->opt_zeta_on_coset - 1) & (n - 1))), 0);
    if (gl2_eq(gl2_pow(zeta, n), gl2_one())) return STARKHIP_ERR_ZETA_IN_SUBGROUP;
    const gl_t shift_n = gl_pow(GL_GENERATOR, n);
    const gl2_t zh = gl2_sub(gl2_pow(zeta, n), gl2_make(shift_n, 0));
    const gl2_t w_scale = gl2_mul_base(zh, gl_inv(gl_mul((gl_t)n, shift_n)));
    HIPCHK(launch_ext_powers(c->zpow.as<gl2_t>(), zeta, n, st));
    HIPCHK(launch_coset_weights(c->zpow.as<gl2_t>() + n, c->gzpow.as<gl2_t>(), zeta, w_scale, s.log_n, st));
    HIPCHK(launch_openings(c->lde.as<gl_t>(), s.N, C, n, c->zpow.as<gl2_t>() + n, c->gzpow.as<gl2_t>(), c->open_local.as<gl2_t>(),
                           c->open_next.as<gl2_t>(), st));
    HIPCHK(launch_openings(c->qcoef.as<gl_t>(), n, Q, n, c->zpow.as<gl2_t>(), nullptr, c->open_q.as<gl2_t>(), nullptr, st));
    if (nZ) {
        HIPCHK(launch_openings(c->perm.zlde.as<gl_t>(), s.N, nZ, n, c->zpow.as<gl2_t>() + n, c->gzpow.as<gl2_t>(), c->perm.open_z.as<gl2_t>(),
                               c->perm.open_zn.as<gl2_t>(), st));
        op_z.resize(nZ);
        op_zn.resize(nZ);
        HIPCHK(read_back(c, op_z.data(), c->perm.open_z.p, nZ * 16, st));
        HIPCHK(read_back(c, op_zn.data(), c->perm.open_zn.p, nZ * 16, st));
    }
    op_local.resize(C);
    op_next.resize(C);
    op_q.resize(Q);
    HIPCHK(read_back(c, op_local.data(), c->open_local.p, C * 16, st));
    HIPCHK(read_back(c, op_next.data(), c->open_next.p, C * 16, st));
    HIPCHK(read_back(c, op_q.data(), c->open_q.p, Q * 16, st));
    return 0;
}

int ProveCall::fri_combine() {
    const size_t n = s.n, N = s.N, C = s.C, Q = s.Q, nZ = s.nZ;
    HIPCHK(stream_wait(c));
    fs.start();
    for (size_t i = 0; i < C; i++) ch.observe_ext(op_local[i]);
    for (size_t i = 0; i < nZ; i++) ch.observe_ext(op_z[i]);
    for (size_t i = 0; i < Q; i++) ch.observe_ext(op_q[i]);
    for (size_t i = 0; i < C; i++) ch.observe_ext(op_next[i]);
    for (size_t i = 0; i < nZ; i++) ch.observe_ext(op_zn[i]);
    const gl2_t fri_alpha = ch.get_ext();
    fs.stop();
    const gl2_t gzeta = gl2_mul_base(zeta, gl_root_of_unity(s.log_n));
    HIPCHK(launch_ext_powers(c->ext_apow.as<gl2_t>(), fri_alpha, C + nZ + Q, st));
    gl_t* comb_t = c->comb_out.as<gl_t>();
    gl2_t* comb_q = c->comb_out.as<gl2_t>() + n;
    HIPCHK(launch_fri_combine(c->lde.as<gl_t>(), N, C, n, c->ext_apow.as<gl2_t>(), COMB_PPC, comb_chunks(C), c->comb_partial.as<gl2_t>(), st));
    if (nZ)
        HIPCHK(launch_fri_combine(c->perm.zlde.as<gl_t>(), N, nZ, n, c->ext_apow.as<gl2_t>() + C, nZ, 1, c->comb_partial.as<gl2_t>() + comb_chunks(C) * n, st));
    HIPCHK(launch_ext_reduce(c->comb_partial.as<gl2_t>(), comb_chunks(C) + (nZ ? 1 : 0), n, comb_t, st));
    if (int rc = run_ntt(c, comb_t, c->fri_vals.as<gl_t>(), 2, n, s.log_n, true, nullptr, c->tab->qshift_inv.as<gl_t>())) return rc;
    HIPCHK(launch_fri_combine(c->qcoef.as<gl_t>(), n, Q, n, c->ext_apow.as<gl2_t>() + C + nZ, Q, 1, comb_q, st));
    std::vector<gl_t> F1w(2 * n);
    std::vector<gl2_t> F1(n), tailq(n), F0(n), q0(n), q1(n), fin(n);
    HIPCHK(read_back(c, F1w.data(), comb_t, n * 16, st));
    HIPCHK(read_back(c, tailq.data(), comb_q, n * 16, st));
    HIPCHK(stream_wait(c));
    host_other.start();
    for (size_t k = 0; k < n; k++) F1[k] = gl2_make(F1w[k], F1w[n + k]);
    for (size_t k = 0; k < n; k++) F0[k] = gl2_add(F1[k], tailq[k]);
    divide_by_linear(F0.data(), n, zeta, q0.data());
    divide_by_linear(F1.data(), n, gzeta, q1.data());
    const gl2_t shift = gl2_pow(fri_alpha, C + nZ);
    for (size_t k = 0; k < n; k++) fin[k] = gl2_add(gl2_mul(q0[k], shift), q1[k]);
    std::vector<gl_t> soa(2 * N, 0);
    for (size_t k = 0; k < n; k++) {
        soa[k] = fin[k].a0;
        soa[N + k] = fin[k].a1;
    }
    host_other.stop();
    HIPCHK(hipMemcpyAsync(c->fri_coef.p, soa.data(), 2 * N * 8, hipMemcpyHostToDevice, st));
    HIPCHK(stream_wait(c));
    return 0;
}

int ProveCall::fri_commit() {
    const size_t ncap = s.ncap;
    fri_caps.resize(s.L * 4 * ncap);
    final_poly.resize(s.geo.final_poly_len);
    size_t len = s.N;
    unsigned log_len = s.log_N;
    gl_t shift = GL_GENERATOR;
    gl_t* coef = c->fri_coef.as<gl_t>();
    gl_t* vals = c->fri_vals.as<gl_t>();
    for (size_t l = 0; l < s.L; l++) {
        HIPCHK(launch_fill_powers(c->scale_tab.as<gl_t>(), 1, shift, len, st));
        if (long_vector(log_len)) {
            LdeLongTables tb;
            if (int rc = ensure_long_tw(c, log_len, &tb)) return rc;
            HIPCHK(launch_ntt_long(coef, vals, vals, 2, len, log_len, false, c->scale_tab.as<gl_t>(), nullptr, tb, st));
        } else {
            HIPCHK(hipMemcpyAsync(vals, coef, len * 8, hipMemcpyDeviceToDevice, st));
            HIPCHK(hipMemcpyAsync(vals + len, coef + len, len * 8, hipMemcpyDeviceToDevice, st));
            HIPCHK(launch_ntt_global(vals, 2, len, log_len, c->tab->tw_fwd.as<gl_t>(), s.log_N, c->scale_tab.as<gl_t>(), nullptr, 1, st));
        }
        const unsigned ab = s.geo.arities[l];
        const size_t n_leaves = len >> ab, width = 2 << ab;
        HIPCHK(launch_fri_leaves(vals, log_len, ab, c->fri_rows[l].as<gl_t>(), st));
        HIPCHK(launch_leaf_hash_rows_by((int)c->opt_hasher, c->fri_rows[l].as<gl_t>(), width, n_leaves, c->fri_digests[l].as<gl_t>(), st));
        HIPCHK(launch_merkle_levels_by((int)c->opt_hasher, c->fri_digests[l].as<gl_t>(), log_len - ab, s.cap_h, st));
        gl_t* cap = fri_caps.data() + l * 4 * ncap;
        HIPCHK(read_back(c, cap, c->fri_digests[l].as<gl_t>() + 4 * level_off(n_leaves, log_len - ab - s.cap_h), 4 * ncap * 8, st));
        HIPCHK(stream_wait(c));
        fs.start();
        ch.observe_many(cap, 4 * ncap);
        const gl2_t beta = ch.get_ext();
        fs.stop();
        HIPCHK(launch_fri_fold(coef, len, ab, beta, vals, st));
        std::swap(coef, vals);
        len >>= ab;
        log_len -= ab;
        for (unsigned b = 0; b < ab; b++) shift = gl_sqr(shift);
    }
    std::vector<gl_t> fc(2 * len);
    HIPCHK(read_back(c, fc.data(), coef, len * 8, st));
    HIPCHK(read_back(c, fc.data() + len, coef + len, len * 8, st));
    HIPCHK(stream_wait(c));
    if ((len >> s.r) != s.geo.final_poly_len) return STARKHIP_ERR_BAD_SHAPE;
    for (size_t k = 0; k < len; k++) {
        if (k < s.geo.final_poly_len) final_poly[k] = gl2_make(fc[k], fc[len + k]);
        else if (fc[k] || fc[len + k]) return STARKHIP_ERR_QUOTIENT_NOT_DIVISIBLE;
    }
    fs.start();
    for (auto& e : final_poly) ch.observe_ext(e);
    fs.stop();
    return 0;
}

int ProveCall::pow() {
    if (pow_witness == STARKHIP_POW_SEARCH) {
        if (cfg.proof_of_work_bits == 0) {
            pow_witness = 0;
        } else {
            gl_t base[12];
            memcpy(base, ch.state, sizeof base);
            for (int i = 0; i < ch.n_in; i++) base[i] = ch.in[i];
            HIPCHK(hipMemcpyAsync(c->pow_state.p, base, sizeof base, hipMemcpyHostToDevice, st));
            unsigned long long best = ~0ULL;
            const uint64_t batch = 1ULL << 20;
            for (uint64_t start = 0; best == ~0ULL; start += batch) {
                if (start >= GL_P - batch) return STARKHIP_ERR_HIP;
                HIPCHK(hipMemcpyAsync(c->pow_best.p, &best, 8, hipMemcpyHostToDevice, st));
                if (c->opt_hasher == STARKHIP_HASHER_KECCAK)
                    HIPCHK(launch_pow_grind_keccak(c->pow_state.as<gl_t>(), ch.n_in, cfg.proof_of_work_bits, start, batch, c->pow_best.as<unsigned long long>(), st));
                else
                    HIPCHK(launch_pow_grind(c->pow_state.as<gl_t>(), ch.n_in, cfg.proof_of_work_bits, start, batch, c->pow_best.as<unsigned long long>(), st));
                HIPCHK(read_back(c, &best, c->pow_best.p, 8, st));
                HIPCHK(stream_wait(c));
            }
            pow_witness = best;
        }
    }
    ch.observe(pow_witness);
    (void)ch.get();
    return 0;
}

int ProveCall::queries() {
    const ProofLayout& pl = s.pl;
    const size_t N = s.N, C = s.C, Q = s.Q, L = s.L, ncap = s.ncap;
    if (!c->hs && !c->blob_airs.count(air.id)) {
        static const bool pinned = [] { const char* e = getenv("STARKHIP_PINNED_PROOFS"); return !(e && *e == '0'); }();
        if (pinned) (void)blob_arena_add(c, pl.total * 8, 2);
        c->blob_airs.insert(air.id);
    }
    out = blob_alloc(pl.total * 8);
    if (!out) return STARKHIP_ERR_OOM;
    const size_t nq = pl.n_queries;
    std::vector<uint32_t> xs(nq);
    for (size_t q = 0; q < nq; q++) xs[q] = (uint32_t)(ch.get() % N);
    const size_t stride = pl.query_words;
    const unsigned d0 = s.log_N - s.cap_h;
    int err = 0;
#define HIPCHK_FREE(expr) do { hipError_t _e = (expr); if (_e != hipSuccess) { fprintf(stderr, "starkhip: HIP error %s (%s)\n", hipGetErrorString(_e), #expr); err = 1; } } while (0)
    gl_t* dq = c->gather_t.as<gl_t>();
    if (nq) HIPCHK_FREE(hipMemcpyAsync(c->qidx.p, xs.data(), nq * 4, hipMemcpyHostToDevice, st));
    const uint32_t* dxs = c->qidx.as<uint32_t>();
    size_t off = 0;
    if (!err) {
        HIPCHK_FREE(launch_query_leaf_colmajor(c->lde.as<gl_t>(), C, s.log_n, s.r, dxs, nq, dq, stride, off, st)); off += C;
        HIPCHK_FREE(launch_query_path(c->digests.as<gl_t>(), N, d0, dxs, 0, nq, dq, stride, off, st)); off += 4 * d0;
        if (s.nZ) {
            HIPCHK_FREE(launch_query_leaf_colmajor(c->perm.zlde.as<gl_t>(), s.nZ, s.log_n, s.r, dxs, nq, dq, stride, off, st)); off += s.nZ;
// ... 141 lines not shown
```

Before: 9.032.

## Fuse Merkle tree levels into subtree kernels that keep nodes in LDS

Replaces the per-level Merkle hashing loop, which issued one kernel per tree level, with a subtree kernel that hashes up to seven levels per launch. Intermediate nodes stay in shared memory. For Poseidon, the narrow upper levels switch to a row form where 16 lanes cooperate on one permutation, keeping more threads busy when few parents remain. The aim is to cut launch overhead and the global re-reads of child digests, at the cost of shrinking per-block parallelism on upper levels and extra shared memory. The feature is on by default, can be toggled with a context option, and a test API exposes it.

```diff
diff --git a/bindings/rust/starkhip-sys/src/lib.rs b/bindings/rust/starkhip-sys/src/lib.rs
--- a/bindings/rust/starkhip-sys/src/lib.rs
+++ b/bindings/rust/starkhip-sys/src/lib.rs
@@ -337,6 +337,8 @@
     pub fn starkhip_keccak_permute_batch(ctx: *mut c_void, states: *mut u64, n: usize) -> c_int;
     pub fn starkhip_merkle_tree_hasher(ctx: *mut c_void, hasher: c_int, lde_colmajor: *const u64, n_cols: usize, log_n: c_uint, cap_height: c_uint,
                                        digests_out: *mut u64, cap_out: *mut u64) -> c_int;
+    pub fn starkhip_merkle_levels(ctx: *mut c_void, hasher: c_int, leaf_digests: *const u64, log_leaves: c_uint, cap_height: c_uint, fused: c_int,
+                                  out: *mut u64) -> c_int;
     pub fn starkhip_hash_rows_hasher(ctx: *mut c_void, hasher: c_int, rows: *const u64, width: usize, n_leaves: usize, digests_out: *mut u64) -> c_int;
     pub fn starkhip_fri_geometry(cfg: *const starkhip_config_t, log_n: c_uint, arities_out: *mut c_uint, cap: usize, n_layers: *mut usize,
                                  final_poly_len: *mut usize) -> c_int;
diff --git a/include/starkhip.h b/include/starkhip.h
--- a/include/starkhip.h
+++ b/include/starkhip.h
@@ -328,6 +328,7 @@
 int starkhip_keccak_permute_batch(void* ctx, uint64_t* states, size_t n);
 int starkhip_merkle_tree_hasher(void* ctx, int hasher, const uint64_t* lde_colmajor, size_t n_cols, unsigned log_N, unsigned cap_height,
                                 uint64_t* digests_out, uint64_t* cap_out);
+int starkhip_merkle_levels(void* ctx, int hasher, const uint64_t* leaf_digests, unsigned log_leaves, unsigned cap_height, int fused, uint64_t* out);
 int starkhip_hash_rows_hasher(void* ctx, int hasher, const uint64_t* rows, size_t width, size_t n_leaves, uint64_t* digests_out);
 void starkhip_poseidon_permute_host(uint64_t state[12]);
 void starkhip_poseidon_permute_host_many(uint64_t state[12], size_t n, int which);
diff --git a/starky_bls12_381_amd/api.py b/starky_bls12_381_amd/api.py
--- a/starky_bls12_381_amd/api.py
+++ b/starky_bls12_381_amd/api.py
@@ -130,6 +130,7 @@
 lib.starkhip_keccak_state_from_words.argtypes = [_u64p, C.c_size_t, _u64p]
 lib.starkhip_keccak_permute_batch.argtypes = [C.c_void_p, _u64p, C.c_size_t]
 lib.starkhip_merkle_tree_hasher.argtypes = [C.c_void_p, C.c_int, _u64p, C.c_size_t, C.c_uint, C.c_uint, _u64p, _u64p]
+lib.starkhip_merkle_levels.argtypes = [C.c_void_p, C.c_int, _u64p, C.c_uint, C.c_uint, C.c_int, _u64p]
 lib.starkhip_hash_rows_hasher.argtypes = [C.c_void_p, C.c_int, _u64p, C.c_size_t, C.c_size_t, _u64p]
 lib.starkhip_proof_hasher.argtypes = [_u64p, C.c_size_t]
 lib.starkhip_trace_ecc_aggregate.argtypes = [_u32p, _u8p, _u64p, C.c_size_t, _u64p]
@@ -1196,6 +1197,19 @@
         cap = np.zeros((1 << cap_height, 4), dtype=np.uint64)
         _chk(lib.starkhip_merkle_tree_hasher(self._ctx, hasher, _p64(v), ncols, N.bit_length() - 1, cap_height, _p64(digests), _p64(cap)))
         return digests, cap
+
+    def merkle_levels(self, leaf_digests, cap_height, hasher=HASHER_POSEIDON, fused=True):
+        d = np.ascontiguousarray(leaf_digests, dtype=np.uint64)
+        assert d.ndim == 2 and d.shape[1] == 4
+        log_leaves = d.shape[0].bit_length() - 1
+        assert d.shape[0] == 1 << log_leaves and log_leaves >= cap_height
+        out = np.zeros((2 * d.shape[0] - (1 << cap_height), 4), dtype=np.uint64)
+        _chk(lib.starkhip_merkle_levels(self._ctx, hasher, _p64(d), log_leaves, cap_height, 1 if fused else 0, _p64(out)))
+        levels, at = [], 0
+        for l in range(log_leaves, cap_height - 1, -1):
+            levels.append(out[at:at + (1 << l)])
+            at += 1 << l
+        return levels
 
     def hash_rows(self, rows, hasher=HASHER_POSEIDON):
         r = np.ascontiguousarray(rows, dtype=np.uint64)
diff --git a/starky_bls12_381_amd/csrc/capi.cpp b/starky_bls12_381_amd/csrc/capi.cpp
--- a/starky_bls12_381_amd/csrc/capi.cpp
+++ b/starky_bls12_381_amd/csrc/capi.cpp
@@ -1072,6 +1072,10 @@
     if (!ctx) return STARKHIP_ERR_NO_DEVICE;
     return merkle_tree_hasher((Ctx*)ctx, hasher, lde_colmajor, n_cols, log_N, cap_height, digests_out, cap_out);
 }
+int starkhip_merkle_levels(void* ctx, int hasher, const uint64_t* leaf_digests, unsigned log_leaves, unsigned cap_height, int fused, uint64_t* out) {
+    if (!ctx) return STARKHIP_ERR_NO_DEVICE;
+    return merkle_levels((Ctx*)ctx, hasher, leaf_digests, log_leaves, cap_height, fused, out);
+}
 int starkhip_hash_rows_hasher(void* ctx, int hasher, const uint64_t* rows, size_t width, size_t n_leaves, uint64_t* digests_out) {
     if (!ctx) return STARKHIP_ERR_NO_DEVICE;
     return hash_rows_hasher((Ctx*)ctx, hasher, rows, width, n_leaves, digests_out);
diff --git a/starky_bls12_381_amd/csrc/ctx.h b/starky_bls12_381_amd/csrc/ctx.h
--- a/starky_bls12_381_amd/csrc/ctx.h
+++ b/starky_bls12_381_amd/csrc/ctx.h
@@ -114,6 +114,7 @@
     long opt_lde_impl = 0;
     long opt_lde_closed_forms = 1;
     long opt_leaf_hash_prefix = 1;
+    long opt_merkle_fused = 1;
     long opt_host_commit_leaves = 64;
     long opt_verify_chunk_mb = 1024;
     double verify_timings[4] = {0};
diff --git a/starky_bls12_381_amd/csrc/ctx.hip b/starky_bls12_381_amd/csrc/ctx.hip
--- a/starky_bls12_381_amd/csrc/ctx.hip
+++ b/starky_bls12_381_amd/csrc/ctx.hip
@@ -367,6 +367,7 @@
     else if (k == "lde_closed_forms" && (value == 0 || value == 1)) c->opt_lde_closed_forms = value;
     else if (k == "lde_impl" && (value == 0 || value == 1)) c->opt_lde_impl = value;
     else if (k == "leaf_hash_prefix" && (value == 0 || value == 1)) c->opt_leaf_hash_prefix = value;
+    else if (k == "merkle_fused" && (value == 0 || value == 1)) c->opt_merkle_fused = value;
     else if (k == "host_commit_leaves" && value >= 0 && value <= 4096) c->opt_host_commit_leaves = value;
     else if (k == "leaf_hash_form" && value >= FORM_AUTO && value <= FORM_PAIR) c->opt_leaf_hash_form = value;
     else if (k == "quotient_cosets" && (value == 0 || value == 1)) c->opt_quotient_cosets = value;
diff --git a/starky_bls12_381_amd/csrc/host_only_stubs.cc b/starky_bls12_381_amd/csrc/host_only_stubs.cc
--- a/starky_bls12_381_amd/csrc/host_only_stubs.cc
+++ b/starky_bls12_381_amd/csrc/host_only_stubs.cc
@@ -111,6 +111,7 @@
 int permute_batch_form(Ctx*, int, int, uint64_t*, size_t) { return STARKHIP_ERR_NO_DEVICE; }
 int keccak_permute_batch(Ctx*, uint64_t*, size_t) { return STARKHIP_ERR_NO_DEVICE; }
 int merkle_tree_hasher(Ctx*, int, const uint64_t*, size_t, unsigned, unsigned, uint64_t*, uint64_t*) { return STARKHIP_ERR_NO_DEVICE; }
+int merkle_levels(Ctx*, int, const uint64_t*, unsigned, unsigned, int, uint64_t*) { return STARKHIP_ERR_NO_DEVICE; }
 int hash_rows_hasher(Ctx*, int, const uint64_t*, size_t, size_t, uint64_t*) { return STARKHIP_ERR_NO_DEVICE; }
 int leaf_hash_lane_group(Ctx*, const uint64_t*, size_t, size_t, unsigned, unsigned, int, int, unsigned, uint64_t*) { return STARKHIP_ERR_NO_DEVICE; }
 int leaf_prefix_table(Ctx*, unsigned, unsigned, uint64_t*) { return STARKHIP_ERR_NO_DEVICE; }
@@ -160,7 +161,8 @@
 }
 hipError_t launch_leaf_hash_keccak(const gl_t*, size_t, unsigned, unsigned, gl_t*, hipStream_t) { return hipErrorNoDevice; }
 hipError_t launch_leaf_hash_rows_keccak(const gl_t*, size_t, size_t, gl_t*, hipStream_t) { return hipErrorNoDevice; }
-hipError_t launch_merkle_levels_keccak(gl_t*, unsigned, unsigned, hipStream_t) { return hipErrorNoDevice; }
+hipError_t launch_merkle_levels(gl_t*, unsigned, unsigned, hipStream_t, bool) { return hipErrorNoDevice; }
+hipError_t launch_merkle_levels_keccak(gl_t*, unsigned, unsigned, hipStream_t, bool) { return hipErrorNoDevice; }
 hipError_t launch_permute_batch_keccak(gl_t*, size_t, hipStream_t) { return hipErrorNoDevice; }
 hipError_t launch_pow_grind_keccak(const gl_t*, int, unsigned, uint64_t, uint64_t, unsigned long long*, hipStream_t) { return hipErrorNoDevice; }
 hipError_t launch_verify_leaf_digests_keccak(const gl_t* words, const VQLeaf* leaves, size_t n, gl_t* digests, hipStream_t) {
diff --git a/starky_bls12_381_amd/csrc/kernel_entries.hip b/starky_bls12_381_amd/csrc/kernel_entries.hip
--- a/starky_bls12_381_amd/csrc/kernel_entries.hip
+++ b/starky_bls12_381_amd/csrc/kernel_entries.hip
@@ -166,7 +166,7 @@
     HIPCHK(hipMemcpyAsync(c->lde.p, lde_natural, n_cols * N * 8, hipMemcpyHostToDevice, c->st));
     int form;
     HIPCHK(launch_leaf_hash_lone(c, c->lde.as<gl_t>(), n_cols, log_N, 0, c->digests.as<gl_t>(), c->st, &form));
-    HIPCHK(launch_merkle_levels(c->digests.as<gl_t>(), log_N, cap_h, c->st));
+    HIPCHK(launch_merkle_levels(c->digests.as<gl_t>(), log_N, cap_h, c->st, c->opt_merkle_fused != 0));
     HIPCHK(hipMemcpyAsync(cap_out, c->digests.as<gl_t>() + 4 * level_off(N, log_N - cap_h), ((size_t)4 << cap_h) * 8, hipMemcpyDeviceToHost, c->st));
     HIPCHK(stream_wait(c));
     return STARKHIP_OK;
@@ -205,9 +205,26 @@
     int form;
     if (hasher == STARKHIP_HASHER_KECCAK) HIPCHK(launch_leaf_hash_keccak(c->lde.as<gl_t>(), n_cols, log_N, 0, c->digests.as<gl_t>(), c->st));
     else HIPCHK(launch_leaf_hash_lone(c, c->lde.as<gl_t>(), n_cols, log_N, 0, c->digests.as<gl_t>(), c->st, &form));
-    HIPCHK(launch_merkle_levels_by(hasher, c->digests.as<gl_t>(), log_N, cap_h, c->st));
+    HIPCHK(launch_merkle_levels_by(hasher, c->digests.as<gl_t>(), log_N, cap_h, c->st, c->opt_merkle_fused != 0));
     if (digests_out) HIPCHK(hipMemcpyAsync(digests_out, c->digests.p, 4 * N * 8, hipMemcpyDeviceToHost, c->st));
     HIPCHK(hipMemcpyAsync(cap_out, c->digests.as<gl_t>() + 4 * level_off(N, log_N - cap_h), ((size_t)4 << cap_h) * 8, hipMemcpyDeviceToHost, c->st));
+    HIPCHK(stream_wait(c));
+    return STARKHIP_OK;
+}
+
+int merkle_levels(Ctx* c, int hasher, const uint64_t* leaf_digests, unsigned log_leaves, unsigned cap_h, int fused, uint64_t* out) {
+    if (hasher < STARKHIP_HASHER_POSEIDON || hasher > STARKHIP_HASHER_KECCAK || !leaf_digests || !out || log_leaves < cap_h || log_leaves > 24 ||
+        (fused != 0 && fused != 1))
+        return STARKHIP_ERR_BAD_SHAPE;
+    HIPCHK(hipSetDevice(c->device));
+    const size_t N = (size_t)1 << log_leaves;
+    const size_t words = 4 * (2 * N - ((size_t)1 << cap_h));
+    HIPCHK(c->digests.ensure(digest_words(N) * 8));
+    gl_t* d = c->digests.as<gl_t>();
+    HIPCHK(hipMemcpyAsync(d, leaf_digests, 4 * N * 8, hipMemcpyHostToDevice, c->st));
+    if (words > 4 * N) HIPCHK(hipMemsetAsync(d + 4 * N, 0xEE, (words - 4 * N) * 8, c->st));
+    HIPCHK(launch_merkle_levels_by(hasher, d, log_leaves, cap_h, c->st, fused != 0));
+    HIPCHK(hipMemcpyAsync(out, d, words * 8, hipMemcpyDeviceToHost, c->st));
     HIPCHK(stream_wait(c));
     return STARKHIP_OK;
 }
diff --git a/starky_bls12_381_amd/csrc/kernels.h b/starky_bls12_381_amd/csrc/kernels.h
--- a/starky_bls12_381_amd/csrc/kernels.h
+++ b/starky_bls12_381_amd/csrc/kernels.h
@@ -94,7 +94,7 @@
                                  LeafPrefix prefix = LeafPrefix());
 hipError_t upload_table_once(const void* symbol, const void* image, size_t bytes, bool (&done)[64]);
 hipError_t launch_leaf_hash_rows(const gl_t* rows, size_t width, size_t n_leaves, gl_t* digests, hipStream_t st);
-hipError_t launch_merkle_levels(gl_t* digests, unsigned log_leaves, unsigned cap_h, hipStream_t st);
+hipError_t launch_merkle_levels(gl_t* digests, unsigned log_leaves, unsigned cap_h, hipStream_t st, bool fused);
 hipError_t launch_permute_batch(gl_t* states, size_t n, hipStream_t st);
 inline unsigned permute_form_variants(int form) {
     switch (form) {
@@ -109,15 +109,15 @@
                             hipStream_t st);
 hipError_t launch_leaf_hash_keccak(const gl_t* mat, size_t n_cols, unsigned log_n, unsigned rate_bits, gl_t* digests, hipStream_t st);
 hipError_t launch_leaf_hash_rows_keccak(const gl_t* rows, size_t width, size_t n_leaves, gl_t* digests, hipStream_t st);
-hipError_t launch_merkle_levels_keccak(gl_t* digests, unsigned log_leaves, unsigned cap_h, hipStream_t st);
+hipError_t launch_merkle_levels_keccak(gl_t* digests, unsigned log_leaves, unsigned cap_h, hipStream_t st, bool fused);
 hipError_t launch_permute_batch_keccak(gl_t* states, size_t n, hipStream_t st);
 hipError_t launch_pow_grind_keccak(const gl_t* base_state, int pos, unsigned pow_bits, uint64_t start, uint64_t count, unsigned long long* best,
                                    hipStream_t st);
 inline hipError_t launch_leaf_hash_rows_by(int hasher, const gl_t* rows, size_t width, size_t n_leaves, gl_t* digests, hipStream_t st) {
     return hasher ? launch_leaf_hash_rows_keccak(rows, width, n_leaves, digests, st) : launch_leaf_hash_rows(rows, width, n_leaves, digests, st);
 }
-inline hipError_t launch_merkle_levels_by(int hasher, gl_t* digests, unsigned log_leaves, unsigned cap_h, hipStream_t st) {
-    return hasher ? launch_merkle_levels_keccak(digests, log_leaves, cap_h, st) : launch_merkle_levels(digests, log_leaves, cap_h, st);
+inline hipError_t launch_merkle_levels_by(int hasher, gl_t* digests, unsigned log_leaves, unsigned cap_h, hipStream_t st, bool fused) {
+    return hasher ? launch_merkle_levels_keccak(digests, log_leaves, cap_h, st, fused) : launch_merkle_levels(digests, log_leaves, cap_h, st, fused);
 }
 hipError_t launch_field_ops(int op, const gl_t* a, const gl_t* b, gl_t* out, size_t n, hipStream_t st);
 
diff --git a/starky_bls12_381_amd/csrc/kernels_hash.hip b/starky_bls12_381_amd/csrc/kernels_hash.hip
--- a/starky_bls12_381_amd/csrc/kernels_hash.hip
+++ b/starky_bls12_381_amd/csrc/kernels_hash.hip
@@ -3,6 +3,7 @@
 #include <mutex>
 
 #include "kernels.h"
+#include "merkle_fused.h"
 #include "poseidon_dev.h"
 #include "verify_query.h"
 
@@ -617,7 +618,30 @@
     hipLaunchKernelGGL(leaf_hash_rows_kernel, dim3(nblocks(n_leaves, 64)), dim3(64), 0, st, rows, width, n_leaves, digests);
     return hipGetLastError();
 }
-hipError_t launch_merkle_levels(gl_t* digests, unsigned log_leaves, unsigned cap_h, hipStream_t st) {
+struct PoseidonTwoToOne {
+    static constexpr bool ROW_FORM = true;
+    static constexpr unsigned ROW_MAX_WIDTH = 64;
+    struct RowShared {
+        RcPair rcs[16][64];
+    };
+    struct RowLane {
+        RowConsts K;
+        const RcPair* rc;
+    };
+    static __device__ __forceinline__ void two_to_one(const gl_t* a, const gl_t* b, gl_t* out) { poseidon_two_to_one_dev(a, b, out); }
+    static __device__ __forceinline__ void row_init(RowShared& sh, RowLane& ln) {
+        row_rcs_fill(sh.rcs);
+        const unsigned e = threadIdx.x & 15u;
+        row_consts_init(ln.K, e, ROW_MERGED.coef[e]);
+        ln.rc = sh.rcs[e];
+    }
+    static __device__ __forceinline__ gl_t row_permute(gl_t s, const RowShared&, const RowLane& ln) {
+        return gl_canon(poseidon_permute_row_merged_asm(s, ln.rc, ln.K));
+    }
+    static hipError_t prepare() { return ensure_row_merged_tables(); }
+};
+hipError_t launch_merkle_levels(gl_t* digests, unsigned log_leaves, unsigned cap_h, hipStream_t st, bool fused) {
+    if (fused) return launch_merkle_fused<PoseidonTwoToOne>(digests, log_leaves, cap_h, st);
     gl_t* child = digests;
     for (unsigned lv = log_leaves; lv > cap_h; lv--) {
         size_t n_parent = (size_t)1 << (lv - 1);
diff --git a/starky_bls12_381_amd/csrc/kernels_keccak.hip b/starky_bls12_381_amd/csrc/kernels_keccak.hip
--- a/starky_bls12_381_amd/csrc/kernels_keccak.hip
+++ b/starky_bls12_381_amd/csrc/kernels_keccak.hip
@@ -2,6 +2,7 @@
 
 #include "keccak.h"
 #include "kernels.h"
+#include "merkle_fused.h"
 #include "verify_query.h"
 
 namespace starkhip {
@@ -116,7 +117,16 @@
     hipLaunchKernelGGL(leaf_hash_rows_keccak_kernel, dim3(nblocks(n_leaves, 64)), dim3(64), 0, st, rows, width, n_leaves, digests);
     return hipGetLastError();
 }
-hipError_t launch_merkle_levels_keccak(gl_t* digests, unsigned log_leaves, unsigned cap_h, hipStream_t st) {
+struct KeccakTwoToOne {
+    static constexpr bool ROW_FORM = false;
+    static constexpr unsigned ROW_MAX_WIDTH = 0;
+    struct RowShared {};
+    struct RowLane {};
+    static __device__ __forceinline__ void two_to_one(const gl_t* a, const gl_t* b, gl_t* out) { keccak_two_to_one(a, b, out); }
+    static hipError_t prepare() { return hipSuccess; }
+};
+hipError_t launch_merkle_levels_keccak(gl_t* digests, unsigned log_leaves, unsigned cap_h, hipStream_t st, bool fused) {
+    if (fused) return launch_merkle_fused<KeccakTwoToOne>(digests, log_leaves, cap_h, st);
     gl_t* child = digests;
     for (unsigned lv = log_leaves; lv > cap_h; lv--) {
         const size_t n_parent = (size_t)1 << (lv - 1);
diff --git a/starky_bls12_381_amd/csrc/merkle_fused.h b/starky_bls12_381_amd/csrc/merkle_fused.h
--- /dev/null
+++ b/starky_bls12_381_amd/csrc/merkle_fused.h
@@ -0,0 +1,105 @@
+#pragma once
+#include <hip/hip_runtime.h>
+
+#include "kernels.h"
+
+namespace starkhip {
+
+#ifndef STARKHIP_MERKLE_SUBTREE_LOG
+#define STARKHIP_MERKLE_SUBTREE_LOG 7
+#endif
+static const unsigned MERKLE_SUBTREE_LOG = STARKHIP_MERKLE_SUBTREE_LOG;
+static_assert(STARKHIP_MERKLE_SUBTREE_LOG >= 1 && STARKHIP_MERKLE_SUBTREE_LOG <= 9, "a workgroup is at most 256 threads: 256 parents of its first level");
+
+template <class H>
+constexpr unsigned merkle_subtree_threads(unsigned log_own) { return H::ROW_FORM ? 256u : 1u << (log_own - 1); }
+
+template <class H>
+__global__ __launch_bounds__(merkle_subtree_threads<H>(STARKHIP_MERKLE_SUBTREE_LOG)) void merkle_subtree_kernel(gl_t* level, unsigned log_nodes,
+                                                                                                                unsigned log_own,
+                                                                                                                unsigned levels) { STARKHIP_PRIO_ENTRY
+    __shared__ gl_t nodes[4u << STARKHIP_MERKLE_SUBTREE_LOG];
+    __shared__ typename H::RowShared row_shared;
+    typename H::RowLane row_lane;
+    if constexpr (H::ROW_FORM) {
+        H::row_init(row_shared, row_lane);
+        __syncthreads();
+    }
+    const unsigned t = threadIdx.x;
+    unsigned width = 1u << (log_own - 1);
+    size_t first = (size_t)blockIdx.x * width;
+    unsigned lv = log_nodes;
+    gl_t* out = level + ((size_t)4 << lv);
+    unsigned lds_in = 0, lds_out = 0;
+    for (unsigned k = 0; k < levels; k++) {
+        bool by_rows = false;
+        if constexpr (H::ROW_FORM) by_rows = width <= H::ROW_MAX_WIDTH;
+        if (!by_rows) {
+            if (t < width) {
+                gl_t a[4], b[4], d[4];
+                if (k == 0) {
+                    const gl_t* c = level + 8 * (first + t);
+#pragma unroll
+                    for (int e = 0; e < 4; e++) {
+                        a[e] = c[e];
+                        b[e] = c[4 + e];
+                    }
+                } else {
+                    const gl_t* c = nodes + 4 * (size_t)(lds_in + 2 * t);
+#pragma unroll
+                    for (int e = 0; e < 4; e++) {
+                        a[e] = c[e];
+                        b[e] = c[4 + e];
+                    }
+                }
+                H::two_to_one(a, b, d);
+                gl_t* g = out + 4 * (first + t);
+                gl_t* l = nodes + 4 * (size_t)(lds_out + t);
+#pragma unroll
+                for (int e = 0; e < 4; e++) {
+                    g[e] = d[e];
+                    l[e] = d[e];
+                }
+            }
+        } else if constexpr (H::ROW_FORM) {
+            const unsigned e = t & 15u, n_rows = blockDim.x >> 4;
+            for (unsigned i0 = 0; i0 < width; i0 += n_rows) {
+                const unsigned i = i0 + (t >> 4);
+                const bool live = i < width;
+                const unsigned ii = live ? i : width - 1;
+                gl_t s = 0;
+                if (e < 8) s = k == 0 ? level[8 * (first + ii) + e] : nodes[4 * (size_t)(lds_in + 2 * ii) + e];
+                s = H::row_permute(s, row_shared, row_lane);
+                if (live && e < 4) {
+                    out[4 * (first + ii) + e] = s;
+                    nodes[4 * (size_t)(lds_out + ii) + e] = s;
+                }
+            }
+        }
+        __syncthreads();
+        lds_in = lds_out;
+        lds_out += width;
+        lv--;
+        out += (size_t)4 << lv;
+        first >>= 1;
+        width >>= 1;
+    }
+}
+
+template <class H>
+hipError_t launch_merkle_fused(gl_t* digests, unsigned log_leaves, unsigned cap_h, hipStream_t st) {
+    if (log_leaves <= cap_h) return hipSuccess;
+    if (hipError_t e = H::prepare(); e != hipSuccess) return e;
+    gl_t* level = digests;
+    unsigned lv = log_leaves;
+    while (lv > cap_h) {
+        const unsigned own = lv < MERKLE_SUBTREE_LOG ? lv : MERKLE_SUBTREE_LOG;
+        const unsigned levels = lv - cap_h < own ? lv - cap_h : own;
+        hipLaunchKernelGGL(merkle_subtree_kernel<H>, dim3(1u << (lv - own)), dim3(merkle_subtree_threads<H>(own)), 0, st, level, lv, own, levels);
+        if (hipError_t e = hipGetLastError(); e != hipSuccess) return e;
+        for (unsigned k = 0; k < levels; k++, lv--) level += (size_t)4 << lv;
+    }
+    return hipSuccess;
+}
+
+}
diff --git a/starky_bls12_381_amd/csrc/prover.h b/starky_bls12_381_amd/csrc/prover.h
--- a/starky_bls12_381_amd/csrc/prover.h
+++ b/starky_bls12_381_amd/csrc/prover.h
@@ -88,6 +88,7 @@
 int permute_batch(Ctx* c, uint64_t* states, size_t n);
 int keccak_permute_batch(Ctx* c, uint64_t* states, size_t n);
 int merkle_tree_hasher(Ctx* c, int hasher, const uint64_t* lde_natural, size_t n_cols, unsigned log_N, unsigned cap_h, uint64_t* digests_out, uint64_t* cap_out);
+int merkle_levels(Ctx* c, int hasher, const uint64_t* leaf_digests, unsigned log_leaves, unsigned cap_h, int fused, uint64_t* out);
 int hash_rows_hasher(Ctx* c, int hasher, const uint64_t* rows, size_t width, size_t n_leaves, uint64_t* digests_out);
 int permute_batch_form(Ctx* c, int form, int variant, uint64_t* states, size_t n);
 int leaf_hash_lane_group(Ctx* c, const uint64_t* mats, size_t n_segments, size_t n_cols, unsigned log_n, unsigned rate_bits, int grouped, int form,
diff --git a/starky_bls12_381_amd/csrc/prover.hip b/starky_bls12_381_amd/csrc/prover.hip
--- a/starky_bls12_381_amd/csrc/prover.hip
+++ b/starky_bls12_381_amd/csrc/prover.hip
@@ -314,7 +314,7 @@
         HIPCHK(launch_leaf_hash_lone(c, c->lde.as<gl_t>(), s.C, s.log_n, s.r, c->digests.as<gl_t>(), st, &c->hash_timing.form, pf));
     }
     HIPCHK(hipEventRecord(c->kev[1], st));
-    HIPCHK(launch_merkle_levels_by((int)c->opt_hasher, c->digests.as<gl_t>(), s.log_N, s.cap_h, st));
+    HIPCHK(launch_merkle_levels_by((int)c->opt_hasher, c->digests.as<gl_t>(), s.log_N, s.cap_h, st, c->opt_merkle_fused != 0));
     trace_cap.resize(4 * s.ncap);
     HIPCHK(read_back(c, trace_cap.data(), c->digests.as<gl_t>() + 4 * level_off(s.N, s.log_N - s.cap_h), 4 * s.ncap * 8, st));
     return 0;
@@ -413,7 +413,7 @@
     HIPCHK(run_lde(c, pb.zvals.as<gl_t>(), lde_long_supported(s.log_n) ? pb.zcoef.as<gl_t>() : nullptr, pb.zlde.as<gl_t>(), nZ, s.log_n, s.r, 0));
     if (c->opt_hasher == STARKHIP_HASHER_KECCAK) HIPCHK(launch_leaf_hash_keccak(pb.zlde.as<gl_t>(), nZ, s.log_n, s.r, pb.zdigests.as<gl_t>(), st));
     else HIPCHK(launch_leaf_hash_form(FORM_QUAD, pb.zlde.as<gl_t>(), nZ, s.log_n, s.r, pb.zdigests.as<gl_t>(), st));
-    HIPCHK(launch_merkle_levels_by((int)c->opt_hasher, pb.zdigests.as<gl_t>(), s.log_N, s.cap_h, st));
+    HIPCHK(launch_merkle_levels_by((int)c->opt_hasher, pb.zdigests.as<gl_t>(), s.log_N, s.cap_h, st, c->opt_merkle_fused != 0));
     zs_cap.resize(4 * s.ncap);
     HIPCHK(read_back(c, zs_cap.data(), pb.zdigests.as<gl_t>() + 4 * level_off(s.N, s.log_N - s.cap_h), 4 * s.ncap * 8, st));
     HIPCHK(stream_wait(c));
@@ -467,7 +467,7 @@
     HIPCHK(run_lde(c, c->qcoef.as<gl_t>(), nullptr, c->qlde.as<gl_t>(), s.Q, s.log_n, s.r, 1));
     if (c->opt_hasher == STARKHIP_HASHER_KECCAK) HIPCHK(launch_leaf_hash_keccak(c->qlde.as<gl_t>(), s.Q, s.log_n, s.r, c->qdigests.as<gl_t>(), st));
     else HIPCHK(launch_leaf_hash_form(FORM_QUAD, c->qlde.as<gl_t>(), s.Q, s.log_n, s.r, c->qdigests.as<gl_t>(), st));
-    HIPCHK(launch_merkle_levels_by((int)c->opt_hasher, c->qdigests.as<gl_t>(), s.log_N, s.cap_h, st));
+    HIPCHK(launch_merkle_levels_by((int)c->opt_hasher, c->qdigests.as<gl_t>(), s.log_N, s.cap_h, st, c->opt_merkle_fused != 0));
     quot_cap.resize(4 * s.ncap);
     HIPCHK(read_back(c, quot_cap.data(), c->qdigests.as<gl_t>() + 4 * level_off(s.N, s.log_N - s.cap_h), 4 * s.ncap * 8, st));
     return 0;
@@ -576,7 +576,7 @@
         const size_t n_leaves = len >> ab, width = 2 << ab;
         HIPCHK(launch_fri_leaves(vals, log_len, ab, c->fri_rows[l].as<gl_t>(), st));
         HIPCHK(launch_leaf_hash_rows_by((int)c->opt_hasher, c->fri_rows[l].as<gl_t>(), width, n_leaves, c->fri_digests[l].as<gl_t>(), st));
-        HIPCHK(launch_merkle_levels_by((int)c->opt_hasher, c->fri_digests[l].as<gl_t>(), log_len - ab, s.cap_h, st));
+        HIPCHK(launch_merkle_levels_by((int)c->opt_hasher, c->fri_digests[l].as<gl_t>(), log_len - ab, s.cap_h, st, c->opt_merkle_fused != 0));
         gl_t* cap = fri_caps.data() + l * 4 * ncap;
         HIPCHK(read_back(c, cap, c->fri_digests[l].as<gl_t>() + 4 * level_off(n_leaves, log_len - ab - s.cap_h), 4 * ncap * 8, st));
         HIPCHK(stream_wait(c));
```

After: 8.988. Within noise of the previous version (-0.5%).
